# IrisRainbowNeko/HCP-Diffusion

Measured on AMD Instinct MI355X. Metric: training images/sec (whole node), SD1.5 LoRA 512px bs=4/GPU, higher is better.
Workload: dtype bf16; 1 GPU; SD1.5 UNet LoRA rank=8 bf16, bs=4/GPU, 512x512 (64x64 latents), 77-token context, random-init weights, cached latents, grad-ckpt off; global_batch=4, parallelism=dp1, rccl_ranks=1, comm=none, hip_graph=True, gradient_checkpointing=False

## Files before the change

hcp_diffusion_amd/_lib.py:

```python
import ctypes
import os
from ctypes import c_int, c_long, c_float, c_void_p, c_size_t, c_char_p
from pathlib import Path

LIB_PATH = Path(__file__).resolve().parent / "libhcp_mi355x.so"

P, I, L, F = c_void_p, c_int, c_long, c_float

_PROTOTYPES = {
    "hcp_last_error": (c_char_p, []),
    "hcp_is_emulated": (I, []),
    "hcp_abi_version": (I, []),
    "hcp_selfcheck_atomics": (I, [P, P, I, I, I, P]),
    "hcp_gemm_bf16": (I, [P, I, P, I, P, I, I, I, I, P, I, P, I, I, P, P, I, I, P, I, P, P, P, F, I, P, c_size_t, P]),
    "hcp_gemm_lora_bf16": (I, [P, I, P, I, P, P, P, I, P, I, I, I, I, P, P, I, P, P, P, P, c_size_t, P]),
    "hcp_gemm_geglu_bwd_bf16": (I, [P, I, P, I, P, P, P, I, P, P, I, I, I, P, c_size_t, P]),
    "hcp_gemm_workspace_bytes": (c_size_t, [I, I]),
    "hcp_conv3x3_bf16": (I, [P, I, P, I, I, I, I, I, I, I, I, I, I, P, I, P, I, P, P, I, P, I, I, P, P, P, c_size_t, P]),
    "hcp_attention_fwd": (I, [P, P, P, P, P, I, I, I, I, I, L, I, L, I, L, I, L, I, F, P, L, I, P]),
    "hcp_attention_bwd": (I, [P, P, P, P, P, P, P, P, P, P, I, I, I, I, I, L, I, L, I, L, I, L, I, F, P, L, I, P, c_size_t, P]),
    "hcp_groupnorm_workspace_bytes": (c_size_t, [I, I, I, I]),
    "hcp_groupnorm_silu_fwd": (I, [P, P, P, P, P, P, I, I, I, I, F, I, P]),
    "hcp_groupnorm_silu_bwd": (I, [P, P, P, P, P, P, P, P, I, I, I, I, I, P]),
    "hcp_layernorm_fwd": (I, [P, P, P, P, P, P, I, I, F, P]),
    "hcp_layernorm_bwd": (I, [P, P, P, P, P, P, P, P, P, I, I, P]),
    "hcp_geglu_fwd": (I, [P, P, L, I, P]),
    "hcp_geglu_bwd": (I, [P, P, P, L, I, P]),
    "hcp_add_bf16": (I, [P, P, P, L, P]),
    "hcp_copy2d_bf16": (I, [P, I, P, I, L, I, P]),
    "hcp_concat2_bf16": (I, [P, I, P, I, P, L, I, P]),
    "hcp_silu_fwd": (I, [P, P, L, P]),
    "hcp_silu_bwd": (I, [P, P, P, L, P]),
    "hcp_nchw_to_nhwc_bf16": (I, [P, I, P, I, I, I, I, P]),
    "hcp_nhwc_to_nchw_f32": (I, [P, P, I, I, I, I, P]),
    "hcp_upsample2x_bwd": (I, [P, P, I, I, I, I, P]),
    "hcp_timestep_embedding": (I, [P, P, I, I, F, P]),
    "hcp_timestep_embedding_f32": (I, [P, P, I, I, F, P]),
    "hcp_wgrad_linear_bf16": (I, [P, I, P, I, P, I, I, I, I, P, c_size_t, P]),
    "hcp_wgrad_conv3x3_bf16": (I, [P, I, P, I, P, I, P, I, I, I, I, I, I, I, I, I, P, c_size_t, P]),
    "hcp_colsum_bf16": (I, [P, I, P, I, I, I, I, P]),
    "hcp_ema_update": (I, [P, P, L, P, F, F, F, P]),
    "hcp_cast_f32_bf16": (I, [P, P, L, F, I, P]),
    "hcp_cast_bf16_f32": (I, [P, P, L, P]),
    "hcp_pack_piece_bytes": (I, []),
    "hcp_pack_weights": (I, [P, I, I, P]),
    "hcp_groupnorm_affine_grad": (I, [P, P, P, P, P, P, P, I, I, I, I, I, P]),
    "hcp_layernorm_affine_grad": (I, [P, P, P, P, P, I, I, P]),
    "hcp_add_noise": (I, [P, P, P, P, P, I, L, P]),
    "hcp_cfg_ddim_step": (I, [P, P, P, L, I, F, F, F, P]),
    "hcp_snr_loss_weight": (I, [P, P, P, I, I, F, P]),
    "hcp_quick_gelu": (I, [P, P, P, L, P]),
    "hcp_embedding_bf16": (I, [P, P, P, P, P, L, I, I, P]),
    "hcp_embedding_pt_fwd_bf16": (I, [P, I, I, I, I, P, I, P, P, I, P, I, P, I, P, P, I, P]),
    "hcp_embedding_pt_bwd_f32": (I, [P, P, L, I, P, I, I, P]),
    "hcp_transpose_bf16": (I, [P, P, I, I, I, P]),
    "hcp_softmax_rows": (I, [P, L, P, L, I, I, F, P]),
    "hcp_vae_latent_sample": (I, [P, P, P, P, P, I, I, L, F, P]),
    "hcp_mse_masked_mean": (I, [P, P, P, I, P, P, P, I, I, I, F, P]),
    "hcp_lora_wgrad": (I, [P, I, I, P, I, P, I, I, I, I, F, I, P, c_size_t, P]),
    "hcp_lora_wgrad_pair": (I, [P, I, P, I, I, P, P, I, P, I, I, P, I, I, F, P, c_size_t, P]),
    "hcp_split_hi_lo_bf16": (I, [P, P, c_long, I, P]),
    "hcp_lora_wgrad_group_geometry": (I, [I, I, I, I, I, P, P, P, P]),
    "hcp_lora_wgrad_group_desc_bytes": (I, []),
    "hcp_lora_wgrad_grouped": (I, [P, I, I, I, c_long, P, c_size_t, P]),
    "hcp_lora_pack": (I, [P, I, P]),
    "hcp_lora_pack_desc_bytes": (I, []),
    "hcp_sumsq_f32": (I, [P, L, P, P]),
    "hcp_adamw_clip_fused": (I, [P, P, P, P, L, P, F, F, F, F, P, F, F, P, P]),
    "hcp_comm_unique_id": (I, [P]),
    "hcp_comm_init": (I, [I, I, P, ctypes.POINTER(P)]),
    "hcp_comm_destroy": (I, [P]),
    "hcp_comm_rank": (I, [P]),
    "hcp_comm_world": (I, [P]),
    "hcp_allreduce_flat": (I, [P, P, c_size_t, I, P]),
    "hcp_reduce_scatter_flat": (I, [P, P, P, c_size_t, I, P]),
    "hcp_allgather_flat": (I, [P, P, P, c_size_t, I, P]),
}

_TOOLS_PROTOTYPES = {
    "hcp_debug_set_gemm_config": (I, [I]),
    "hcp_debug_set_gemm_glds": (I, [I]),
    "hcp_debug_set_gemm_loaders": (I, [I]),
    "hcp_debug_set_gemm_epilogue": (I, [I]),
    "hcp_debug_set_conv_patch": (I, [I]),
    "hcp_debug_set_gn_target": (I, [I]),
    "hcp_debug_set_gemm_ablation": (I, [I]),
    "hcp_debug_set_attention_config": (I, [I]),
    "hcp_debug_set_wgrad_tile": (I, [I]),
    "hcp_debug_gemm_table_stats": (I, [P, P]),
}

EXPORTED_SYMBOLS = tuple(_PROTOTYPES)
TOOLS_SYMBOLS = tuple(_TOOLS_PROTOTYPES)
TOOLS_LIB_PATH = Path(__file__).resolve().parent / "libhcp_mi355x_tools.so"


ABI_VERSION = 4


class HcpError(RuntimeError):
    pass


def bind(cdll):
    cdll.hcp_abi_version.restype = I
    cdll.hcp_abi_version.argtypes = []
    got = cdll.hcp_abi_version()
    if got != ABI_VERSION:
        raise HcpError(f"{getattr(cdll, '_name', 'library')}: hcp_abi_version() = {got}, these bindings are for ABI {ABI_VERSION} "
                       "(rebuild with `python -m hcp_diffusion_amd.build`)")
    for name, (res, args) in _PROTOTYPES.items():
        fn = getattr(cdll, name)
        fn.restype = res
        fn.argtypes = args
    for name, (res, args) in _TOOLS_PROTOTYPES.items():
        fn = getattr(cdll, name, None)
        if fn is not None:
            fn.restype = res
            fn.argtypes = args
    return cdll


_tools = None


def load_tools():
    global _tools
    if _tools is None:
        import torch
        if not TOOLS_LIB_PATH.exists():
            raise HcpError(f"{TOOLS_LIB_PATH} not found: build it with `python -m hcp_diffusion_amd.build`")
        _tools = ctypes.CDLL(str(TOOLS_LIB_PATH))
        for name in _TOOLS_PROTOTYPES:
            getattr(_tools, name)
    return _tools


_lib = None


def load():
    global _lib
    if _lib is None:
        import torch
        if not LIB_PATH.exists():
            raise HcpError(
                f"{LIB_PATH} not found: build it with `python -m hcp_diffusion_amd.build` "
                "(hipcc, gfx950). hcp_diffusion_amd has no CPU/PyTorch fallback path.")
        _lib = bind(ctypes.CDLL(str(LIB_PATH)))
    return _lib


def check(rc, what=""):
    if rc != 0:
        msg = load().hcp_last_error() if _lib is not None else b""
        raise HcpError(f"{what} failed: {msg.decode() if msg else rc}")
```

hcp_diffusion_amd/csrc/gemm.hip:

```cpp
#include "hcp_common.h"
#include "gemm_params.h"

extern "C" int hcp_geglu_fwd(const void* h, void* y, long M, int F, hipStream_t stream);

namespace {

using namespace hcp_gemm;

HCP_DEVICE void epilogue_store(const GemmParams& p, int m, int n, hcp_f32x4 v) {
    if (p.geglu_hg) { epilogue_geglu_bwd(p, m, n, v); return; }
    v = v * p.alpha;
    if (p.bias) v += *(const hcp_f32x4*)(p.bias + n);
    if (p.rowbias) v += *(const hcp_f32x4*)(p.rowbias + (size_t)(m / p.rows_per_group) * p.rowbias_ld + n);
    if (p.residual) {
        hcp_bf16x4 r = *(const hcp_bf16x4*)(p.residual + (size_t)m * p.ldr + n);
#pragma unroll
        for (int q = 0; q < 4; ++q) v[q] += hcp_bf2f((unsigned short)r[q]);
        add_residual_lo(p, m, n, v);
    }
    if (p.out_f32) *(hcp_f32x4*)((float*)p.D + (size_t)m * p.ldd + n) = v;
    else store_hi_lo(p, m, n, v);
}


// ... 469 lines not shown
            } else
#endif
            {
#pragma unroll
                for (int i = 0; i < TM; ++i) fa[i] = *(const hcp_bf16x8*)(st + a_rd + i * 16 * BK);
#pragma unroll
                for (int j = 0; j < TN; ++j) fb[j] = *(const hcp_bf16x8*)(st + b_rd + j * 16 * BK);
            }
#if defined(HCP_TOOLS)
            if (p.dbg & 16) {
#pragma unroll
                for (int i = 0; i < TM; ++i) asm volatile("" ::"v"(fa[i]));
#pragma unroll
                for (int j = 0; j < TN; ++j) asm volatile("" ::"v"(fb[j]));
                continue;
            }
#endif
#pragma unroll
            for (int i = 0; i < TM; ++i)
#pragma unroll
                for (int j = 0; j < TN; ++j) acc[i][j] = hcp_mfma16(fb[j], fa[i], acc[i][j]);
            if (LORA) {
                const hcp_bf16x8 fl = *(const hcp_bf16x8*)(st + (l_rd0 ^ (ks * 32)));
#pragma unroll
                for (int i = 0; i < TM; ++i) tacc[i] = hcp_mfma16(fl, fa[i], tacc[i]);
            }
        }
    };

    constexpr bool EARLY = NLD > 0;
    constexpr int ES = EARLY ? 32 : 40;
    hcp_bf16* const le_early = lds + NST * BUF_ELEMS;
    hcp_f32x4 bias_v[TN];
    hcp_bf16x4 res_v[TM][TN];
    auto load_epilogue_operands = [&]() {
#pragma unroll
        for (int j = 0; j < TN; ++j) {
            const int nl = n0 + wn * WTN + j * 16 + 4 * fg, n = geglu_col(p, BN, nl);
            hcp_f32x4 z = {0.f, 0.f, 0.f, 0.f};
            bias_v[j] = (p.bias && nl < p.N) ? *(const hcp_f32x4*)(p.bias + n) : z;
        }
        if (p.residual && !p.epi_tile) {
#pragma unroll
            for (int i = 0; i < TM; ++i) {
                const int m = m0 + wm * WTM + i * 16 + fr;
#pragma unroll
                for (int j = 0; j < TN; ++j) {
                    const int n = n0 + wn * WTN + j * 16 + 4 * fg;
                    hcp_bf16x4 z = {0, 0, 0, 0};
                    res_v[i][j] = (m < p.M && n < p.N) ? *(const hcp_bf16x4*)(p.residual + (size_t)m * p.ldr + n) : z;
                }
            }
        }
    };
    if (EARLY && !is_loader && p.nsplit == 1) load_epilogue_operands();

    if (NLD > 0 && is_loader) {
        if (LORA) {
            const hcp_rsrc re = hcp_make_rsrc(p.E);
            for (int g = wave; g < BN / 16; g += NLD) {
                const int nl = n0 + g * 16 + (lane >> 2), n = geglu_col(p, BN, nl);
                hcp_buf_glds16(re, nl < p.N ? (unsigned)(((size_t)n * 32 + (lane & 3) * 8) * 2) : HCP_BUF_OOB, le_early + g * 16 * 32);
            }
        }
        static_assert(NLD == 0 || (BM % RPP == 0 && BN % RPP == 0), "loader waves: whole row groups");
        constexpr int IPT = A_IT + B_IT + (LORA ? 1 : 0);
        int issued = 0, wbuf = 0;
        auto issue_next = [&]() {
            if (issued < nprim) issue(wbuf); else issue_ext(wbuf);
            ++issued; wbuf = wbuf + 1 == NST ? 0 : wbuf + 1;
        };
        auto wait_newer = [&](int newer) {
            if (NST > 3 && newer >= 2) hcp_wait_vmcnt_c<2 * IPT>();
            else if (NST > 2 && newer >= 1) hcp_wait_vmcnt_c<IPT>();
            else hcp_wait_vmcnt_c<0>();
        };
        for (int i = 0; i < NST - 1 && issued < nk; ++i) issue_next();
        wait_newer(issued - 1);
        hcp_barrier_keep_dma();
        for (int t = 0; t < nk; ++t) {
#if defined(HCP_TOOLS)
            if (p.dbg & 8) issued = nk;
#endif
            if (issued < nk) issue_next();
            wait_newer(issued - (t + 2));
            hcp_barrier_keep_dma();
        }
        if (LORA) HCP_SYNC();
        if ((p.geglu_hg || p.geglu_out || p.epi_tile) && p.nsplit == 1) { if (LORA) HCP_SYNC(); HCP_SYNC(); }
        return;
    }
    if (NLD == 0) { if (nprim > 0) issue(0); else if (has_ext) issue_ext(0); }
    HCP_SYNC();
    for (int t = 0, cur = 0; t < nk; ++t) {
        if (NLD == 0) {
            if (t + 1 < nprim) issue(cur ^ 1);
            else if (t + 1 == nprim && has_ext) issue_ext(cur ^ 1);
        }
        compute(cur);
        HCP_SYNC();
        cur = cur + 1 == NST ? 0 : cur + 1;
    }

    if (LORA) {
        constexpr int TS2 = 40;
        hcp_bf16* lt = lds;
        hcp_bf16* le = EARLY ? le_early : lds + BM * TS2;
        hcp_bf16* lt2 = lds + BM * TS2 + (EARLY ? 0 : BN * TS2);
        const bool split = p.ldt == 64;
        const int ldt = split ? 64 : 32;
#pragma unroll
        for (int i = 0; i < TM; ++i) {
            hcp_bf16x4 o, o2;
            lora_t_split(tacc[i], o, o2);
            const int ml = wm * WTM + i * 16 + fr;
            *(hcp_bf16x4*)(lt + ml * TS2 + wn * 16 + 4 * fg) = o;
            if (split) *(hcp_bf16x4*)(lt2 + ml * TS2 + wn * 16 + 4 * fg) = o2;
            if (tile_n == 0 && p.Tout && m0 + ml < p.M) {
                *(hcp_bf16x4*)(p.Tout + (size_t)(m0 + ml) * ldt + wn * 16 + 4 * fg) = o;
                if (split) *(hcp_bf16x4*)(p.Tout + (size_t)(m0 + ml) * ldt + 32 + wn * 16 + 4 * fg) = o2;
            }
        }
        if (!EARLY) {
            for (int c = tid_all; c < BN * 4; c += NTC) {
                const int r = c >> 2, q = c & 3;
                hcp_bf16x8 v = hcp_zero8();
                if (n0 + r < p.N) v = *(const hcp_bf16x8*)(p.E + (size_t)geglu_col(p, BN, n0 + r) * 32 + q * 8);
                *(hcp_bf16x8*)(le + r * TS2 + q * 8) = v;
            }
        }
        HCP_SYNC();
        hcp_bf16x8 ft[TM], fe[TN];
#pragma unroll
        for (int i = 0; i < TM; ++i) ft[i] = *(const hcp_bf16x8*)(lt + (wm * WTM + i * 16 + fr) * TS2 + fg * 8);
#pragma unroll
        for (int j = 0; j < TN; ++j) fe[j] = *(const hcp_bf16x8*)(le + (wn * WTN + j * 16 + fr) * ES + fg * 8);
#pragma unroll
        for (int i = 0; i < TM; ++i)
#pragma unroll
            for (int j = 0; j < TN; ++j) acc[i][j] = hcp_mfma16(fe[j], ft[i], acc[i][j]);
        if (split) {
#pragma unroll
            for (int i = 0; i < TM; ++i) ft[i] = *(const hcp_bf16x8*)(lt2 + (wm * WTM + i * 16 + fr) * TS2 + fg * 8);
#pragma unroll
            for (int i = 0; i < TM; ++i)
#pragma unroll
                for (int j = 0; j < TN; ++j) acc[i][j] = hcp_mfma16(fe[j], ft[i], acc[i][j]);
        }
    }

    if (p.nsplit > 1) {
#pragma unroll
        for (int i = 0; i < TM; ++i) {
            const int m = m0 + wm * WTM + i * 16 + fr;
            if (m >= p.M) continue;
#pragma unroll
            for (int j = 0; j < TN; ++j) {
                const int n = n0 + wn * WTN + j * 16 + 4 * fg;
                if (n < p.N) *(hcp_f32x4*)(p.slabs + ((size_t)split * p.M + m) * p.N + n) = acc[i][j];
            }
        }
        return;
    }
    if (p.geglu_hg) {
        static_assert((size_t)BM * geglu_tile_ld(BN) <= (size_t)2 * BUF_ELEMS, "the product tile fits the ring");
        if (LORA) HCP_SYNC();
#pragma unroll
        for (int i = 0; i < TM; ++i)
#pragma unroll
            for (int j = 0; j < TN; ++j) geglu_tile_put(lds, geglu_tile_ld(BN), wm * WTM + i * 16 + fr, wn * WTN + j * 16 + 4 * fg, acc[i][j], p.alpha);
        HCP_SYNC();
        geglu_tile_apply<BM, BN, NTC>(p, lds, m0, n0, tid_all);
        return;
    }
    if (p.geglu_out) {
        static_assert((size_t)BM * BN * 2 <= (size_t)2 * BUF_ELEMS * sizeof(hcp_bf16), "the gelu(g) tile fits the ring");
        if (!EARLY) load_epilogue_operands();
        if (LORA) HCP_SYNC();
        hcp_f32x4 v[TM][TN];
        int rows[TM], cols[TN];
        constexpr int HW = WGN / 2;
        const bool is_g = wn >= HW;
#pragma unroll
        for (int j = 0; j < TN; ++j) cols[j] = tile_n * (BN / 2) + (wn - (is_g ? HW : 0)) * WTN + j * 16 + 4 * fg;
#pragma unroll
        for (int i = 0; i < TM; ++i) {
            const int m = m0 + wm * WTM + i * 16 + fr;
            rows[i] = m;
#pragma unroll
            for (int j = 0; j < TN; ++j) {
                v[i][j] = acc[i][j] * p.alpha + bias_v[j];
                if (m < p.M) store_hi_lo(p, m, cols[j] + (is_g ? (p.N >> 1) : 0), v[i][j]);
            }
        }
        geglu_fwd_pair<TM, TN>(v, is_g, wm * HW + (wn - (is_g ? HW : 0)), lane, (hcp_f32x4*)lds, [] { HCP_SYNC(); }, p.geglu_out, p.N >> 1, rows, p.M, cols);
        return;
    }
    if (p.epi_tile) {
        if (!EARLY) load_epilogue_operands();
        if (LORA) HCP_SYNC();
        float* const tile = (float*)lds;
#pragma unroll
        for (int i = 0; i < TM; ++i) {
            const int ml = wm * WTM + i * 16 + fr, m = m0 + ml;
            const float* rbp = (p.rowbias && m < p.M) ? p.rowbias + (size_t)(m / p.rows_per_group) * p.rowbias_ld : nullptr;
#pragma unroll
            for (int j = 0; j < TN; ++j) {
                const int nl = wn * WTN + j * 16 + 4 * fg;
                hcp_f32x4 v = acc[i][j] * p.alpha + bias_v[j];
                if (rbp && n0 + nl < p.N) v += *(const hcp_f32x4*)(rbp + n0 + nl);
                *(hcp_f32x4*)(tile + ml * epi_tile_ld(BN) + nl) = v;
            }
        }
        HCP_SYNC();
        epi_tile_store<BM, BN, NTC>(p, tile, m0, n0, tid_all);
        return;
    }
    if (!EARLY) load_epilogue_operands();
#pragma unroll
    for (int i = 0; i < TM; ++i) {
        const int m = m0 + wm * WTM + i * 16 + fr;
        if (m >= p.M) continue;
        hcp_f32x4 rb_v[TN];
        if (p.rowbias) {
            const float* rbp = p.rowbias + (size_t)(m / p.rows_per_group) * p.rowbias_ld;
#pragma unroll
            for (int j = 0; j < TN; ++j) {
                const int n = n0 + wn * WTN + j * 16 + 4 * fg;
                hcp_f32x4 z = {0.f, 0.f, 0.f, 0.f};
                rb_v[j] = n < p.N ? *(const hcp_f32x4*)(rbp + n) : z;
            }
        }
#pragma unroll
        for (int j = 0; j < TN; ++j) {
            const int n = n0 + wn * WTN + j * 16 + 4 * fg;
            if (n >= p.N) continue;
            hcp_f32x4 v = acc[i][j] * p.alpha + bias_v[j];
            if (p.rowbias) v += rb_v[j];
            if (p.residual) {
#pragma unroll
                for (int q = 0; q < 4; ++q) v[q] += hcp_bf2f((unsigned short)res_v[i][j][q]);
                add_residual_lo(p, m, n, v);
            }
#if defined(HCP_TOOLS)
            if ((p.dbg & 64) && v[0] != 12345.678f) continue;
#endif
            if (p.out_f32) *(hcp_f32x4*)((float*)p.D + (size_t)m * p.ldd + n) = v;
            else store_hi_lo(p, m, n, v);
        }
    }
}

HCP_KERNEL(256) splitk_reduce_kernel(GemmParams p) {
    const unsigned nv = (unsigned)p.N / 4;
    const unsigned total = (unsigned)p.M * nv;
    const size_t slab = (size_t)p.M * p.N;
    const int ns = p.nsplit;
    const bool plain = !p.geglu_hg;
    for (unsigned i = blockIdx.x * 256u + threadIdx.x; i < total; i += gridDim.x * 256u) {
        const int m = (int)(i / nv), n = (int)(i - (unsigned)m * nv) * 4;
        const float* src = p.slabs + (size_t)i * 4;
        hcp_f32x4 v = *(const hcp_f32x4*)src;
        const void* const zp = g_zero_page;
        const hcp_f32x4 bias = *(const hcp_f32x4*)(plain && p.bias ? (const void*)(p.bias + n) : zp);
        const hcp_f32x4 rowb = *(const hcp_f32x4*)(plain && p.rowbias ? (const void*)(p.rowbias + (size_t)(m / p.rows_per_group) * p.rowbias_ld + n) : zp);
        const hcp_bf16x4 res = *(const hcp_bf16x4*)(plain && p.residual ? (const void*)(p.residual + (size_t)m * p.ldr + n) : zp);
        const hcp_bf16x4 res_lo = *(const hcp_bf16x4*)(plain && p.residual && p.residual_lo ? (const void*)(p.residual_lo + (size_t)m * p.ldr + n) : zp);
        int s = 1;
        for (; s + 4 <= ns; s += 4) {
            const hcp_f32x4 a = *(const hcp_f32x4*)(src + (size_t)s * slab), b = *(const hcp_f32x4*)(src + (size_t)(s + 1) * slab);
            const hcp_f32x4 c = *(const hcp_f32x4*)(src + (size_t)(s + 2) * slab), d = *(const hcp_f32x4*)(src + (size_t)(s + 3) * slab);
            v += a; v += b; v += c; v += d;
        }
        if (s + 2 <= ns) {
            const hcp_f32x4 a = *(const hcp_f32x4*)(src + (size_t)s * slab), b = *(const hcp_f32x4*)(src + (size_t)(s + 1) * slab);
            v += a; v += b;
            s += 2;
        }
        if (s < ns) v += *(const hcp_f32x4*)(src + (size_t)s * slab);
        if (!plain) { epilogue_geglu_bwd(p, m, n, v); continue; }
        v = v * p.alpha;
        if (p.bias) v += bias;
        if (p.rowbias) v += rowb;
        if (p.residual) {
#pragma unroll
            for (int q = 0; q < 4; ++q) v[q] += hcp_bf2f((unsigned short)res[q]);
            if (p.residual_lo) {
#pragma unroll
                for (int q = 0; q < 4; ++q) v[q] += hcp_bf2f((unsigned short)res_lo[q]);
            }
        }
        if (p.out_f32) *(hcp_f32x4*)((float*)p.D + (size_t)m * p.ldd + n) = v;
        else store_hi_lo(p, m, n, v);
    }
}

HCP_TUNABLE(int, g_force_cfg, -1);
inline int forced_id(int v) { return v >= 1024 ? (v - 1024) % 64 : v % 16; }
inline int forced_split(int v) { const int s = v >= 1024 ? (v - 1024) / 64 : v / 16; return s > 0 ? s : 1; }
HCP_TUNABLE(int, g_dbg_ablate, 0);
HCP_TUNABLE(int, g_use_v2, 1);

HCP_TUNABLE(int, g_conv_patch, 1);
HCP_TUNABLE(int, g_epi_tile, -1);
HCP_TUNABLE(int, g_force_loaders, -1);

bool want_epi_tile(const GemmParams& p, int mode) {
    if (p.nsplit != 1 || p.out_f32 || p.geglu_hg || p.geglu_out || p.N % 8 || p.ldd % 8 || (p.residual && p.ldr % 8)) return false;
    if ((((size_t)p.D) | ((size_t)p.D_lo) | ((size_t)p.residual) | ((size_t)p.residual_lo)) & 15) return false;
    if (g_epi_tile >= 0) return g_epi_tile == 1;
    return mode == 0 && p.residual != nullptr;
}

int launch_splitk_reduce(const GemmParams& p, hipStream_t stream, const char* name = "splitk_reduce_kernel") {
    if (p.nsplit > 1) {
        const long nv = (long)p.M * (p.N / 4);
        int g = (int)((nv + 255) / 256); if (g > 2048) g = 2048;
        HCP_LAUNCH(splitk_reduce_kernel, dim3(g), dim3(256), 0, stream, p);
    }
    HCP_LAUNCH_CHECK(name);
}
bool buffer_loops_take(const GemmParams& p) {
    return g_use_v2 && !(g_dbg_ablate & 7) && p.K % BK == 0 && (p.K2 == 0 || p.K2 == 32) &&
           (size_t)p.M * p.lda * 2 < (1ul << 31) && (size_t)p.N * p.ldb * 2 < (1ul << 31);
}
void pair_geglu_or_clear(GemmParams& p, int mode, int bn, int wgn) {
    if (p.geglu_out && mode == 0 && wgn % 2 == 0 && p.nsplit == 1 && (p.N / 2) % (bn / 2) == 0) p.geglu_fused = 1;
    else p.geglu_out = nullptr;
}
template <int BM, int BN, int WGM, int WGN, int MODE, bool FAST, bool LORA = false, int NSTAGE = 2, int NLD = 0>
int launch_cfg(GemmParams& p, hipStream_t stream) {
    p.tiles_m = hcp_cdiv(p.M, BM);
    const int tiles_n = hcp_cdiv(p.N, BN);
    p.dbg = g_dbg_ablate;
    constexpr size_t tail = (size_t)(2 * BM + BN) * 40 * sizeof(hcp_bf16);
    if constexpr (NSTAGE == 2 && (MODE == 0 || FAST)) {
        if (buffer_loops_take(p)) {
            constexpr size_t stage = (size_t)(BM + BN + (LORA ? 32 : 0)) * BK * sizeof(hcp_bf16);
            constexpr size_t eimg = (LORA && NLD > 0) ? (size_t)BN * 32 * sizeof(hcp_bf16) : 0;
            pair_geglu_or_clear(p, MODE, BN, WGN);
            constexpr size_t tile_bytes = (size_t)BM * epi_tile_ld(BN) * sizeof(float);
            p.epi_tile = want_epi_tile(p, MODE) && tile_bytes <= 160 * 1024 - eimg ? 1 : 0;
            size_t smem = 2 * stage;
            if (LORA && smem < tail) smem = tail;
            if (p.epi_tile && smem < tile_bytes) smem = tile_bytes;
            [[maybe_unused]] const dim3 grid(p.tiles_m * tiles_n, p.nsplit);
            if constexpr (NLD > 0) {
                const size_t tb = p.epi_tile ? tile_bytes : 0;
                if (p.loaders == 4 && 4 * stage + eimg <= 160 * 1024) {
                    HCP_LAUNCH((gemm_v2_kernel<BM, BN, WGM, WGN, MODE, LORA, NLD, (4 * stage + eimg <= 160 * 1024 ? 4 : 2)>), grid, dim3(64 * (WGM * WGN + NLD)), (4 * stage > tb ? 4 * stage : tb) + eimg, stream, p);
                } else if (p.loaders >= 3 && 3 * stage + eimg <= 160 * 1024) {
                    HCP_LAUNCH((gemm_v2_kernel<BM, BN, WGM, WGN, MODE, LORA, NLD, (3 * stage + eimg <= 160 * 1024 ? 3 : 2)>), grid, dim3(64 * (WGM * WGN + NLD)), (3 * stage > tb ? 3 * stage : tb) + eimg, stream, p);
                } else if (p.loaders) {
                    HCP_LAUNCH((gemm_v2_kernel<BM, BN, WGM, WGN, MODE, LORA, NLD>), grid, dim3(64 * (WGM * WGN + NLD)), smem + eimg, stream, p);
                } else {
                    HCP_LAUNCH((gemm_v2_kernel<BM, BN, WGM, WGN, MODE, LORA>), grid, dim3(64 * WGM * WGN), smem, stream, p);
                }
            } else {
                HCP_LAUNCH((gemm_v2_kernel<BM, BN, WGM, WGN, MODE, LORA>), dim3(p.tiles_m * tiles_n, p.nsplit), dim3(64 * WGM * WGN), smem, stream, p);
            }
            return launch_splitk_reduce(p, stream, "gemm_v2_kernel");
        }
    }
    {
        p.epi_tile = 0;
        p.geglu_out = nullptr;
        size_t smem = (size_t)NSTAGE * (BM + BN + (LORA ? 32 : 0)) * BK * sizeof(hcp_bf16);
        if (LORA && smem < tail) smem = tail;
        HCP_LAUNCH((gemm_glds_kernel<BM, BN, WGM, WGN, MODE, FAST, LORA, NSTAGE>), dim3(p.tiles_m * tiles_n, p.nsplit),
                   dim3(64 * WGM * WGN), smem, stream, p);
    }
    return launch_splitk_reduce(p, stream, "gemm_kernel");
}

struct TileCfg { int bm, bn; };
constexpr TileCfg kCfgs[] = {{128, 128}, {128, 64}, {64, 64}, {128, 160}, {64, 160}, {256, 128}, {256, 160}, {128, 320},
                             {128, 160}, {128, 160}, {256, 160},
                             {128, 320}, {256, 160}, {128, 160}, {64, 160}, {128, 128},
                             {32, 160}};
constexpr int kNumCfgs = sizeof(kCfgs) / sizeof(kCfgs[0]);

int try_pp(int id, int mode, bool fast_or_plain, bool lora, GemmParams& p, hipStream_t stream) {
    if (p.loaders < 8 || !fast_or_plain || !buffer_loops_take(p)) return -2;
    const int bm = kCfgs[id].bm, bn = kCfgs[id].bn;
    p.tiles_m = hcp_cdiv(p.M, bm);
    p.dbg = g_dbg_ablate;
    p.epi_tile = want_epi_tile(p, mode) ? 1 : 0;
    hcp_bf16* const gout = p.geglu_out;
    pair_geglu_or_clear(p, mode, bn, 2);
    int r = -2;
    if (mode != 0 && !lora && (g_conv_patch == 2 || (g_conv_patch == 1 && (mode == 2 || p.nsplit > 1))))
        r = conv_patch_launch(p, bm, bn, mode, p.loaders - 8, stream);
    if (r == -2) r = gemm_pp_launch(p, bm, bn, mode, lora, p.loaders - 8, stream);
    if (r == -2) { p.geglu_out = gout; p.geglu_fused = 0; }
    if (r != 0 || p.nsplit <= 1) return r;
    return launch_splitk_reduce(p, stream);
}

template <int MODE, bool FAST>
int launch_by_id(int id, GemmParams& p, hipStream_t stream) {
    if (id >= 0 && id < kNumCfgs) { const int r = try_pp(id, MODE, MODE == 0 || FAST, false, p, stream); if (r != -2) return r; }
    switch (id) {
        case 0: return launch_cfg<128, 128, 2, 2, MODE, FAST>(p, stream);
        case 1: return launch_cfg<128, 64, 2, 2, MODE, FAST>(p, stream);
        case 2: return launch_cfg<64, 64, 2, 2, MODE, FAST>(p, stream);
        case 3: return launch_cfg<128, 160, 2, 2, MODE, FAST>(p, stream);
        case 4: return launch_cfg<64, 160, 2, 2, MODE, FAST>(p, stream);
        case 5: return launch_cfg<256, 128, 4, 2, MODE, FAST>(p, stream);
        case 6: return launch_cfg<256, 160, 4, 2, MODE, FAST>(p, stream);
        case 8: return launch_cfg<128, 160, 4, 2, MODE, FAST, false, 3>(p, stream);
        case 9: return launch_cfg<128, 160, 2, 2, MODE, FAST, false, 3>(p, stream);
        case 10: return launch_cfg<256, 160, 4, 2, MODE, FAST, false, 3>(p, stream);
        case 11: return launch_cfg<128, 320, 4, 4, MODE, FAST>(p, stream);
        case 12: return launch_cfg<256, 160, 8, 2, MODE, FAST>(p, stream);
        case 13: return launch_cfg<128, 160, 4, 2, MODE, FAST, false, 2, 4>(p, stream);
        case 14: return launch_cfg<64, 160, 4, 2, MODE, FAST, false, 2, 4>(p, stream);
        case 15: return launch_cfg<128, 128, 4, 2, MODE, FAST, false, 2, 4>(p, stream);
        case 16: return launch_cfg<64, 160, 4, 2, MODE, FAST, false, 2, 4>(p, stream);
        default: return launch_cfg<128, 320, 2, 4, MODE, FAST>(p, stream);
    }
}

int launch_lora_by_id(int id, GemmParams& p, hipStream_t stream) {
    if (id >= 0 && id < kNumCfgs) { const int r = try_pp(id, 0, true, true, p, stream); if (r != -2) return r; }
    switch (id) {
        case 0: return launch_cfg<128, 128, 2, 2, 0, false, true>(p, stream);
        case 1: return launch_cfg<128, 64, 2, 2, 0, false, true>(p, stream);
        case 2: return launch_cfg<64, 64, 2, 2, 0, false, true>(p, stream);
        case 3: return launch_cfg<128, 160, 2, 2, 0, false, true>(p, stream);
        case 5: return launch_cfg<256, 128, 4, 2, 0, false, true>(p, stream);
        case 6: return launch_cfg<256, 160, 4, 2, 0, false, true>(p, stream);
        case 8: return launch_cfg<128, 160, 4, 2, 0, false, true, 3>(p, stream);
        case 9: return launch_cfg<128, 160, 2, 2, 0, false, true, 3>(p, stream);
        case 12: return launch_cfg<256, 160, 8, 2, 0, false, true>(p, stream);
        case 13: return launch_cfg<128, 160, 4, 2, 0, false, true, 2, 4>(p, stream);
        case 14: return launch_cfg<64, 160, 4, 2, 0, false, true, 2, 4>(p, stream);
        case 15: return launch_cfg<128, 128, 4, 2, 0, false, true, 2, 4>(p, stream);
        case 16: return launch_cfg<64, 160, 4, 2, 0, false, true, 2, 4>(p, stream);
        default: return launch_cfg<64, 160, 2, 2, 0, false, true>(p, stream);
    }
}

int choose_cfg(const GemmParams& p, int* nsplit_out) {
    const int nk1 = hcp_cdiv(p.K, BK);
    int id;
    if (p.N <= 64) id = 2;
    else if (p.N % 160 == 0) id = ((long)p.M * p.N >= (long)4096 * 2560) ? 6 : 4;
    else id = ((long)p.M * p.N >= (long)4096 * 2048) ? 0 : 2;
    const long tiles = (long)hcp_cdiv(p.M, kCfgs[id].bm) * hcp_cdiv(p.N, kCfgs[id].bn);
    int s = 1;
    while (s < 16 && tiles * s < 1024 && nk1 / (s * 2) >= 4) s *= 2;
    *nsplit_out = s;
    return id;
}

struct TunedEntry { int mode, M, N, K, has_k2, stride, up, cfg, split, loaders; };
const TunedEntry kTuned[] = {
#include "gemm_tuned_loaders.inc"
#include "gemm_tuned.inc"
};

#if defined(HCP_TOOLS)
long g_table_hits = 0, g_table_misses = 0;
#endif

bool lookup_tuned(const GemmParams& p, int mode, int* cfg, int* split, int* loaders = nullptr) {
    bool hit = false;
    for (const TunedEntry& e : kTuned) {
        if (g_force_loaders == 0 && e.loaders) continue;
        if (e.mode == mode && e.M == p.M && e.N == p.N && e.K == p.K && e.has_k2 == (p.K2 > 0) &&
            (mode == 0 || mode == 3 || (e.stride == p.cv.stride && e.up == p.cv.up))) {
            *cfg = e.cfg; *split = e.split; if (loaders) *loaders = e.loaders; hit = true; break;
        }
    }
#if defined(HCP_TOOLS)
    (hit ? g_table_hits : g_table_misses) += 1;
#endif
    return hit;
}

inline int deepest_ring(int ld) { return ld == 3 ? 4 : ld; }

template <int MODE, bool FAST>
int dispatch_gemm(GemmParams& p, float* ws, size_t ws_bytes, hipStream_t stream) {
    int nsplit = 1;
    int id = 0, ld = 0;
    if (!lookup_tuned(p, MODE, &id, &nsplit, &ld)) id = choose_cfg(p, &nsplit);
    if (g_force_cfg >= 0) { id = forced_id(g_force_cfg); nsplit = forced_split(g_force_cfg); }
    p.loaders = g_force_loaders >= 0 ? g_force_loaders : deepest_ring(ld);
    if (nsplit > 1 && (size_t)nsplit * p.M * p.N * sizeof(float) > ws_bytes) nsplit = 1;
    if (p.geglu_out) nsplit = 1;
    const int nk1 = hcp_cdiv(p.K, BK);
    p.nsplit = nsplit;
    p.kt_per_split = hcp_cdiv(nk1, nsplit);
    p.nsplit = hcp_cdiv(nk1, p.kt_per_split);
    p.slabs = ws;
    return launch_by_id<MODE, FAST>(id, p, stream);
}

int check_common(const GemmParams& p) {
    HCP_REQUIRE(p.M > 0 && p.N > 0 && p.K > 0, "gemm: empty problem M=%d N=%d K=%d", p.M, p.N, p.K);
    HCP_REQUIRE(p.K % 8 == 0 && p.K2 % 8 == 0, "gemm: K (%d) and K2 (%d) must be multiples of 8", p.K, p.K2);
    HCP_REQUIRE(p.N % 4 == 0 && p.ldd % 4 == 0, "gemm: N (%d) and ldd (%d) must be multiples of 4", p.N, p.ldd);
    HCP_REQUIRE(p.ldb % 8 == 0, "gemm: ldb (%d) must be a multiple of 8", p.ldb);
    HCP_REQUIRE(p.K2 == 0 || (p.A2 && p.B2 && p.lda2 % 8 == 0 && p.ldb2 % 8 == 0), "gemm: bad K-extension operands");
    HCP_REQUIRE(!p.residual || p.ldr % 4 == 0, "gemm: ldr must be a multiple of 4");
    HCP_REQUIRE(!p.rowbias || p.rows_per_group > 0, "gemm: rows_per_group must be > 0");
    return 0;
}

int check_gact(GemmParams& p, void* gact, const char* who) {
    if (!gact) return 0;
    HCP_REQUIRE(!p.out_f32 && !p.residual && !p.rowbias && !p.D_lo && p.alpha == 1.0f && p.N % 16 == 0 && p.ldd == p.N,
                "%s: the GEGLU output needs a contiguous bf16 (h | g) [M, N] (N %% 16 == 0) with no residual / row bias / alpha", who);
    p.geglu_out = (hcp_bf16*)gact; p.geglu_fused = 0;
    return 0;
}
int finish_gact(const GemmParams& p, void* gact, hipStream_t stream) {
    if (!gact || p.geglu_fused) return 0;
    return hcp_geglu_fwd(p.D, gact, p.M, p.N / 2, stream);
}

int launch_lora_dispatched(GemmParams& p, void* workspace, size_t workspace_bytes, hipStream_t stream) {
    int id = 4, nsplit = 1, ld = 0;
    GemmParams q = p; q.K2 = 32;
    if (!lookup_tuned(q, 3, &id, &nsplit, &ld)) {
        if (p.K >= 4096 && p.M <= 4096) id = -1;
        else if ((long)p.M * p.N >= (long)4096 * 2560 && p.N % 160 == 0) id = 6;
        else if (p.N % 160 == 0 && (long)p.M * p.N >= (long)4096 * 640) id = 4;
        else id = 2;
    }
    if (g_force_cfg >= 0) id = forced_id(g_force_cfg);
    p.loaders = g_force_loaders >= 0 ? g_force_loaders : deepest_ring(ld);
    if (id == 7 || id == 10 || id == 11) id = 6;
    if (id < 0) {
        HCP_REQUIRE(p.Tout, "hcp_gemm_lora_bf16: this shape runs as two launches and needs the T buffer");
        const int ldt = p.ldt == 64 ? 64 : 32;
        if (ldt == 64 && hcp_memset_async(p.Tout, 0, (size_t)p.M * 64 * sizeof(hcp_bf16), stream)) return hcp_set_error("hcp_gemm_lora_bf16: memset failed");
        GemmParams t = {};
        t.A = p.A; t.lda = p.lda; t.B = p.L; t.ldb = p.K; t.M = p.M; t.N = 32; t.K = p.K; t.D = p.Tout; t.ldd = ldt; t.alpha = 1.0f;
        if (int e2 = dispatch_gemm<0, false>(t, (float*)workspace, workspace ? workspace_bytes : 0, stream)) return e2;
        p.A2 = (const hcp_bf16*)p.Tout; p.lda2 = ldt; p.B2 = p.E; p.ldb2 = 32; p.K2 = 32;
        p.L = nullptr; p.E = nullptr; p.Tout = nullptr; p.ldt = 0;
        return dispatch_gemm<0, false>(p, (float*)workspace, workspace ? workspace_bytes : 0, stream);
    }
    p.nsplit = 1; p.kt_per_split = hcp_cdiv(p.K, BK); p.slabs = nullptr;
    return launch_lora_by_id(id, p, stream);
}

}

#if defined(HCP_TOOLS)
HCP_API int hcp_debug_gemm_table_stats(long* hits, long* misses) {
    if (hits) *hits = g_table_hits;
    if (misses) *misses = g_table_misses;
    g_table_hits = 0; g_table_misses = 0;
    return 0;
}
HCP_API int hcp_debug_set_gemm_config(int cfg) { g_force_cfg = cfg; return 0; }
HCP_API int hcp_debug_set_gemm_glds(int on) { g_use_v2 = on == 1; return 0; }
HCP_API int hcp_debug_set_gemm_ablation(int flags) { g_dbg_ablate = flags; return 0; }
HCP_API int hcp_debug_set_gemm_loaders(int mode) { g_force_loaders = mode; return 0; }
HCP_API int hcp_debug_set_gemm_epilogue(int mode) { g_epi_tile = mode; return 0; }
HCP_API int hcp_debug_set_conv_patch(int on) { g_conv_patch = on; return 0; }
#endif

HCP_API size_t hcp_gemm_workspace_bytes(int M, int N) { return (size_t)16 * M * N * sizeof(float); }

HCP_API int hcp_gemm_bf16(const void* A, int lda, const void* B, int ldb, void* D, int ldd, int M, int N, int K,
                          const void* A2, int lda2, const void* B2, int ldb2, int K2, const float* bias,
                          const float* rowbias, int rowbias_ld, int rows_per_group, const void* residual, int ldr,
                          const void* residual_lo, void* D_lo, void* gact, float alpha, int out_f32, void* workspace,
                          size_t workspace_bytes, hipStream_t stream) {
    GemmParams p = {};
    p.A = (const hcp_bf16*)A; p.lda = lda; p.B = (const hcp_bf16*)B; p.ldb = ldb;
    p.A2 = (const hcp_bf16*)A2; p.lda2 = lda2; p.B2 = (const hcp_bf16*)B2; p.ldb2 = ldb2; p.K2 = K2;
    p.M = M; p.N = N; p.K = K; p.D = D; p.ldd = ldd; p.out_f32 = out_f32;
    p.bias = bias; p.rowbias = rowbias; p.rowbias_ld = rowbias_ld; p.rows_per_group = rows_per_group;
    p.residual = (const hcp_bf16*)residual; p.ldr = ldr; p.alpha = alpha;
    p.residual_lo = (const hcp_bf16*)residual_lo; p.D_lo = (hcp_bf16*)D_lo;
    HCP_REQUIRE(A && B && D, "hcp_gemm_bf16: null operand");
    HCP_REQUIRE((!residual_lo || residual) && (!D_lo || !out_f32), "hcp_gemm_bf16: residual_lo needs residual; D_lo needs a bf16 output");
    HCP_REQUIRE(lda % 8 == 0, "hcp_gemm_bf16: lda (%d) must be a multiple of 8", lda);
    if (int e = check_common(p)) return e;
    if (int e = check_gact(p, gact, "hcp_gemm_bf16")) return e;
    if (int e = dispatch_gemm<0, false>(p, (float*)workspace, workspace ? workspace_bytes : 0, stream)) return e;
    return finish_gact(p, gact, stream);
}

HCP_API int hcp_conv3x3_bf16(const void* X1, int C1, const void* X2, int C2, int Bn, int Hs, int Ws, int Ho, int Wo,
                             int mode, int stride, int upsample, int pad, const void* Wp, int Cout, void* D, int ldd,
                             const float* bias, const float* rowbias, int rowbias_ld, const void* residual, int ldr,
                             int out_f32, const void* A2, const void* B2, void* workspace, size_t workspace_bytes,
                             hipStream_t stream) {
    GemmParams p = {};
    HCP_REQUIRE(X1 && Wp && D, "hcp_conv3x3_bf16: null operand");
    HCP_REQUIRE((A2 == nullptr) == (B2 == nullptr), "hcp_conv3x3_bf16: the rank-32 K-extension needs both A2 and B2");
    if (A2) { p.A2 = (const hcp_bf16*)A2; p.lda2 = 32; p.B2 = (const hcp_bf16*)B2; p.ldb2 = 32; p.K2 = 32; }
    HCP_REQUIRE(C1 % 8 == 0 && C2 % 8 == 0 && (C2 == 0 || X2), "hcp_conv3x3_bf16: channels must be multiples of 8");
    HCP_REQUIRE(stride == 1 || stride == 2, "hcp_conv3x3_bf16: stride must be 1 or 2");
    HCP_REQUIRE(mode == 0 || (mode == 1 && upsample == 0 && C2 == 0), "hcp_conv3x3_bf16: bad mode/options");
    HCP_REQUIRE(pad == 1 || (pad == 0 && mode == 0 && !upsample), "hcp_conv3x3_bf16: pad must be 1 (or 0 for a forward conv without upsampling)");
    HCP_REQUIRE(Ho <= 1024 && Wo <= 1024 && Bn < 2048, "hcp_conv3x3_bf16: dims too large for packed pixel ids (10 bits per output axis)");
    HCP_REQUIRE((long)Bn * Hs * Ws * (C1 > C2 ? C1 : C2) < (1L << 31), "hcp_conv3x3_bf16: source tensor too large for 32-bit offsets");
    p.cv.X1 = (const hcp_bf16*)X1; p.cv.C1 = C1; p.cv.X2 = (const hcp_bf16*)X2; p.cv.C2 = C2;
    p.cv.Hs = Hs; p.cv.Ws = Ws; p.cv.Ho = Ho; p.cv.Wo = Wo; p.cv.stride = stride; p.cv.up = upsample ? 1 : 0; p.cv.pad = pad;
    p.M = Bn * Ho * Wo; p.N = Cout; p.K = 9 * (C1 + C2);
    p.B = (const hcp_bf16*)Wp; p.ldb = p.K;
    p.D = D; p.ldd = ldd; p.out_f32 = out_f32; p.bias = bias;
    p.rowbias = rowbias; p.rowbias_ld = rowbias_ld; p.rows_per_group = Ho * Wo;
    p.residual = (const hcp_bf16*)residual; p.ldr = ldr; p.alpha = 1.0f;
    if (int e = check_common(p)) return e;
    float* ws = (float*)workspace; size_t wb = workspace ? workspace_bytes : 0;
    const bool fast = (C1 % 64 == 0) && (C2 % 64 == 0) && !upsample && !(mode == 1 && stride == 2);
    if (mode == 0) return fast ? dispatch_gemm<1, true>(p, ws, wb, stream) : dispatch_gemm<1, false>(p, ws, wb, stream);
    return fast ? dispatch_gemm<2, true>(p, ws, wb, stream) : dispatch_gemm<2, false>(p, ws, wb, stream);
}

HCP_API int hcp_gemm_geglu_bwd_bf16(const void* A, int lda, const void* B, int ldb, const void* L, const void* E, void* Tout, int ldt,
                                    const void* HG, void* DHG, int M, int F, int K, void* workspace, size_t workspace_bytes,
                                    hipStream_t stream) {
    GemmParams p = {};
    p.A = (const hcp_bf16*)A; p.lda = lda; p.B = (const hcp_bf16*)B; p.ldb = ldb;
    p.M = M; p.N = F; p.K = K; p.D = DHG; p.ldd = 2 * F; p.out_f32 = 0; p.alpha = 1.0f;
    p.geglu_hg = (const hcp_bf16*)HG; p.geglu_ld = 2 * F;
    HCP_REQUIRE(A && B && HG && DHG, "hcp_gemm_geglu_bwd_bf16: null operand");
    HCP_REQUIRE((L == nullptr) == (E == nullptr), "hcp_gemm_geglu_bwd_bf16: L and E come together");
    HCP_REQUIRE(lda % 8 == 0 && F % 8 == 0, "hcp_gemm_geglu_bwd_bf16: lda (%d) and F (%d) must be multiples of 8", lda, F);
    if (int e = check_common(p)) return e;
    if (!L) return dispatch_gemm<0, false>(p, (float*)workspace, workspace ? workspace_bytes : 0, stream);
    HCP_REQUIRE(ldt == 32 || ldt == 64, "hcp_gemm_geglu_bwd_bf16: ldt (%d) is 32 (bf16 U) or 64 (split U: hi | lo)", ldt);
    p.L = (const hcp_bf16*)L; p.E = (const hcp_bf16*)E; p.Tout = (hcp_bf16*)Tout; p.ldt = ldt;
    return launch_lora_dispatched(p, workspace, workspace_bytes, stream);
}

HCP_API int hcp_gemm_lora_bf16(const void* A, int lda, const void* B, int ldb, const void* L, const void* E, void* Tout, int ldt, void* D,
                               int ldd, int M, int N, int K, const float* bias, const void* residual, int ldr, const void* residual_lo,
                               void* D_lo, void* gact, void* workspace, size_t workspace_bytes, hipStream_t stream) {
    GemmParams p = {};
    p.A = (const hcp_bf16*)A; p.lda = lda; p.B = (const hcp_bf16*)B; p.ldb = ldb;
    p.M = M; p.N = N; p.K = K; p.D = D; p.ldd = ldd; p.out_f32 = 0;
    p.bias = bias; p.residual = (const hcp_bf16*)residual; p.ldr = ldr; p.alpha = 1.0f;
    p.L = (const hcp_bf16*)L; p.E = (const hcp_bf16*)E; p.Tout = (hcp_bf16*)Tout; p.ldt = ldt;
    p.residual_lo = (const hcp_bf16*)residual_lo; p.D_lo = (hcp_bf16*)D_lo;
    HCP_REQUIRE(A && B && D && L && E, "hcp_gemm_lora_bf16: null operand");
    HCP_REQUIRE(!residual_lo || residual, "hcp_gemm_lora_bf16: residual_lo needs residual");
    HCP_REQUIRE(ldt == 32 || ldt == 64, "hcp_gemm_lora_bf16: ldt (%d) is 32 (bf16 T) or 64 (split T: hi | lo)", ldt);
    HCP_REQUIRE(lda % 8 == 0, "hcp_gemm_lora_bf16: lda (%d) must be a multiple of 8", lda);
    if (int e = check_common(p)) return e;
    if (int e = check_gact(p, gact, "hcp_gemm_lora_bf16")) return e;
    if (int e = launch_lora_dispatched(p, workspace, workspace_bytes, stream)) return e;
    return finish_gact(p, gact, stream);
}
```

hcp_diffusion_amd/csrc/gemm_params.h:

```cpp
#pragma once
#include "hcp_common.h"

namespace hcp_gemm {

struct ConvDesc {
    const hcp_bf16* X1; int C1;
    const hcp_bf16* X2; int C2;
    int Hs, Ws;
    int Ho, Wo;
    int stride;
    int up;
    int pad;
};

struct GemmParams {
    const hcp_bf16* A; int lda;
    const hcp_bf16* A2; int lda2; int K2;
    const hcp_bf16* B; int ldb;
    const hcp_bf16* B2; int ldb2;
    int M, N, K;
    void* D; int ldd; int out_f32;
    const float* bias;
    const float* rowbias; int rowbias_ld; int rows_per_group;
    const hcp_bf16* residual; int ldr;
    const hcp_bf16* residual_lo; hcp_bf16* D_lo;
    float alpha;
    int tiles_m;
    int nsplit; int kt_per_split;
    float* slabs;
    const hcp_bf16* L; const hcp_bf16* E; hcp_bf16* Tout; int ldt;
    const hcp_bf16* geglu_hg; int geglu_ld;
    hcp_bf16* geglu_out; int geglu_fused;
    int epi_tile;
    int loaders;
    int dbg;
    ConvDesc cv;
};

constexpr int BK = 64;

HCP_DEVICE void lora_t_split(const hcp_f32x4& t, hcp_bf16x4& hi, hcp_bf16x4& lo) {
#pragma unroll
    for (int q = 0; q < 4; ++q) {
        const unsigned short h = hcp_f2bf(t[q]);
        hi[q] = (short)h;
        lo[q] = (short)hcp_f2bf(t[q] - hcp_bf2f(h));
    }
}

HCP_DEVICE void store_hi_lo(const GemmParams& p, int m, int n, const hcp_f32x4& v) {
    hcp_bf16x4 o;
#pragma unroll
    for (int q = 0; q < 4; ++q) o[q] = (short)hcp_f2bf(v[q]);
    *(hcp_bf16x4*)((hcp_bf16*)p.D + (size_t)m * p.ldd + n) = o;
    if (p.D_lo) {
        hcp_bf16x4 l;
#pragma unroll
        for (int q = 0; q < 4; ++q) l[q] = (short)hcp_f2bf(v[q] - hcp_bf2f((unsigned short)o[q]));
        *(hcp_bf16x4*)(p.D_lo + (size_t)m * p.ldd + n) = l;
    }
}
HCP_DEVICE void add_residual_lo(const GemmParams& p, int m, int n, hcp_f32x4& v) {
    if (!p.residual_lo) return;
    const hcp_bf16x4 r = *(const hcp_bf16x4*)(p.residual_lo + (size_t)m * p.ldr + n);
#pragma unroll
    for (int q = 0; q < 4; ++q) v[q] += hcp_bf2f((unsigned short)r[q]);
}

constexpr int epi_tile_ld(int BN) { return BN + 4; }
template <int BM, int BN, int NTHREADS>
HCP_DEVICE void epi_tile_store(const GemmParams& p, const float* tile, int m0, int n0, int tid) {
    constexpr int LD = epi_tile_ld(BN), PIECES = BN / 8;
    for (int idx = tid; idx < BM * PIECES; idx += NTHREADS) {
        const int row = idx / PIECES, c8 = (idx - row * PIECES) * 8;
        const int m = m0 + row, n = n0 + c8;
        if (m >= p.M || n >= p.N) continue;
        const hcp_f32x4 a = *(const hcp_f32x4*)(tile + row * LD + c8), b = *(const hcp_f32x4*)(tile + row * LD + c8 + 4);
        float v[8] = {a[0], a[1], a[2], a[3], b[0], b[1], b[2], b[3]};
        if (p.residual) {
            const hcp_bf16x8 r = *(const hcp_bf16x8*)(p.residual + (size_t)m * p.ldr + n);
#pragma unroll
            for (int q = 0; q < 8; ++q) v[q] += hcp_bf2f((unsigned short)r[q]);
            if (p.residual_lo) {
                const hcp_bf16x8 rl = *(const hcp_bf16x8*)(p.residual_lo + (size_t)m * p.ldr + n);
#pragma unroll
                for (int q = 0; q < 8; ++q) v[q] += hcp_bf2f((unsigned short)rl[q]);
            }
        }
        hcp_bf16x8 o;
#pragma unroll
        for (int q = 0; q < 8; ++q) o[q] = (short)hcp_f2bf(v[q]);
        *(hcp_bf16x8*)((hcp_bf16*)p.D + (size_t)m * p.ldd + n) = o;
        if (p.D_lo) {
            hcp_bf16x8 l;
#pragma unroll
            for (int q = 0; q < 8; ++q) l[q] = (short)hcp_f2bf(v[q] - hcp_bf2f((unsigned short)o[q]));
            *(hcp_bf16x8*)(p.D_lo + (size_t)m * p.ldd + n) = l;
        }
    }
}

HCP_DEVICE int geglu_col(const GemmParams& p, int BN, int nl) {
    if (!p.geglu_out) return nl;
    const int half = BN >> 1, j = nl / BN, c = nl - j * BN;
    return c < half ? j * half + c : (p.N >> 1) + j * half + (c - half);
}
template <int TI, int TJ, typename SYNC>
HCP_DEVICE void geglu_fwd_pair(hcp_f32x4 (&v)[TI][TJ], bool is_g, int slot, int lane, hcp_f32x4* xg, SYNC&& sync,
                               hcp_bf16* out, int F, const int (&rows)[TI], int M, const int (&cols)[TJ]) {
    hcp_f32x4* mine = xg + (size_t)slot * TI * TJ * 64 + lane;
    if (is_g) {
#pragma unroll
        for (int i = 0; i < TI; ++i)
#pragma unroll
            for (int j = 0; j < TJ; ++j) {
                hcp_f32x4 ge;
#pragma unroll
                for (int q = 0; q < 4; ++q) ge[q] = hcp_gelu_erf(v[i][j][q]);
                mine[(i * TJ + j) * 64] = ge;
            }
    }
    sync();
    if (!is_g) {
#pragma unroll
        for (int i = 0; i < TI; ++i) {
            if (rows[i] >= M) continue;
#pragma unroll
            for (int j = 0; j < TJ; ++j) {
                const hcp_f32x4 ge = mine[(i * TJ + j) * 64];
                hcp_bf16x4 o;
#pragma unroll
                for (int q = 0; q < 4; ++q) o[q] = (short)hcp_f2bf(v[i][j][q] * ge[q]);
                *(hcp_bf16x4*)(out + (size_t)rows[i] * F + cols[j]) = o;
            }
        }
    }
}

HCP_DEVICE void epilogue_geglu_bwd(const GemmParams& p, int m, int n, hcp_f32x4 v) {
    const hcp_bf16* hp = p.geglu_hg + (size_t)m * p.geglu_ld + n;
    const hcp_bf16x4 h = *(const hcp_bf16x4*)hp, g = *(const hcp_bf16x4*)(hp + p.N);
    hcp_bf16x4 dh, dg;
#pragma unroll
    for (int q = 0; q < 4; ++q) {
        const float hf = hcp_bf2f((unsigned short)h[q]), gf = hcp_bf2f((unsigned short)g[q]);
        const float d = hcp_bf2f(hcp_f2bf(v[q] * p.alpha));
        dh[q] = (short)hcp_f2bf(d * hcp_gelu_erf(gf));
        dg[q] = (short)hcp_f2bf(d * hf * hcp_gelu_erf_grad(gf));
    }
    hcp_bf16* dp = (hcp_bf16*)p.D + (size_t)m * p.ldd + n;
    *(hcp_bf16x4*)dp = dh;
    *(hcp_bf16x4*)(dp + p.N) = dg;
}

constexpr int geglu_tile_ld(int BN) { return BN + 8; }
HCP_DEVICE void geglu_tile_put(hcp_bf16* tile, int ld, int row, int col, hcp_f32x4 v, float alpha) {
    hcp_bf16x4 o;
#pragma unroll
    for (int q = 0; q < 4; ++q) o[q] = (short)hcp_f2bf(v[q] * alpha);
    *(hcp_bf16x4*)(tile + row * ld + col) = o;
}
template <int BM, int BN, int NTHREADS>
HCP_DEVICE void geglu_tile_apply(const GemmParams& p, const hcp_bf16* tile, int m0, int n0, int tid) {
    constexpr int LD = geglu_tile_ld(BN), PIECES = BN / 8;
    for (int idx = tid; idx < BM * PIECES; idx += NTHREADS) {
        const int row = idx / PIECES, c8 = (idx - row * PIECES) * 8;
        const int m = m0 + row, n = n0 + c8;
        if (m >= p.M || n >= p.N) continue;
        const hcp_bf16x8 d = *(const hcp_bf16x8*)(tile + row * LD + c8);
        const hcp_bf16* hp = p.geglu_hg + (size_t)m * p.geglu_ld + n;
        const hcp_bf16x8 h = *(const hcp_bf16x8*)hp, g = *(const hcp_bf16x8*)(hp + p.N);
        hcp_bf16x8 dh, dg;
#pragma unroll
        for (int q = 0; q < 8; ++q) {
            const float df = hcp_bf2f((unsigned short)d[q]), hf = hcp_bf2f((unsigned short)h[q]), gf = hcp_bf2f((unsigned short)g[q]);
            dh[q] = (short)hcp_f2bf(df * hcp_gelu_erf(gf));
            dg[q] = (short)hcp_f2bf(df * hf * hcp_gelu_erf_grad(gf));
        }
        hcp_bf16* dp = (hcp_bf16*)p.D + (size_t)m * p.ldd + n;
        *(hcp_bf16x8*)dp = dh;
        *(hcp_bf16x8*)(dp + p.N) = dg;
    }
}

int gemm_pp_launch(GemmParams& p, int bm, int bn, int mode, bool lora, int ring, hipStream_t stream);
int conv_patch_launch(GemmParams& p, int bm, int bn, int mode, int ring, hipStream_t stream);

}
```

hcp_diffusion_amd/csrc/gemm_pp.hip:

```cpp
#include "gemm_params.h"
#include <type_traits>

namespace hcp_gemm {
namespace {

template <int BM, int BN, int MODE, bool LORA, int NST>
HCP_KERNEL(768) gemm_pp_kernel(GemmParams p) {
    constexpr int NC = 8, NLD = 4;
    constexpr int NTC = 64 * NC, NTL = 64 * NLD;
    constexpr int WTM = BM / 2, WTN = BN / 2;
    constexpr int TM = WTM / 16, TN = WTN / 16;
    constexpr int UPT = 1;
    constexpr bool FIN_N = TM == 1;
    constexpr int TMF = FIN_N ? 1 : TM / 2;
    constexpr int TNF0 = FIN_N ? (TN + 1) / 2 : TN, TNF1 = FIN_N ? TN / 2 : TN;
    constexpr int TNF = TNF0;
    constexpr int RPP = NTL / 8;
    constexpr int A_IT = BM / RPP, B_IT = BN / RPP;
    static_assert(WTM % 16 == 0 && WTN % 16 == 0 && BM % RPP == 0 && BN % RPP == 0 && (TM % 2 == 0 || FIN_N), "tile shape");
    static_assert(NST >= 2 && NST <= 4, "ring depth");
    constexpr int A_ELEMS = BM * BK, B_ELEMS = BN * BK, L_ELEMS = LORA ? 32 * BK : 0, BUF_ELEMS = A_ELEMS + B_ELEMS + L_ELEMS;
    constexpr int E_ELEMS = LORA ? BN * 32 : 0;
    HCP_DYN_SMEM(smem);
    hcp_bf16* const lds_e = (hcp_bf16*)smem;
    hcp_bf16* const ring = lds_e + E_ELEMS;

    const int tid_all = threadIdx.x;
    const int lane = tid_all & 63;
    const int wave_all = hcp_uniform(tid_all >> 6);
    const int tile_m = blockIdx.x % p.tiles_m, tile_n = blockIdx.x / p.tiles_m;
    const int m0 = tile_m * BM, n0 = tile_n * BN;
    const int split = blockIdx.y;

    const int nk1 = p.K / BK;
    const int kt_begin = split * p.kt_per_split;
    int kt_end = kt_begin + p.kt_per_split; if (kt_end > nk1) kt_end = nk1;
    const int nprim = kt_end - kt_begin;
    const bool has_ext = (split == p.nsplit - 1) && p.K2 > 0;
    const int nk = nprim + (has_ext ? 1 : 0);

    if (wave_all >= NC) {
        const int wave = wave_all - NC, tid = tid_all - NTC;
        const int kc = tid & 7, lrow = tid >> 3;
#if defined(HCP_TOOLS)
        if (p.dbg & 0x2000) hcp_setprio<3>();
#endif
        const int Ctot = p.cv.C1 + p.cv.C2;
        unsigned va[A_IT], vb[B_IT];
        unsigned a_msk[(A_IT + 2) / 3];
#pragma unroll
        for (int i = 0; i < (A_IT + 2) / 3; ++i) a_msk[i] = 0;
        const unsigned a_chunk = (unsigned)(((kc ^ ((lrow >> 1) & 7)) << 3) * 2);
#pragma unroll
        for (int i = 0; i < B_IT; ++i) {
            const int r = lrow + RPP * i, nl = n0 + r, n = geglu_col(p, BN, nl);
            vb[i] = nl < p.N ? (unsigned)(((size_t)n * p.ldb + ((kc ^ ((r >> 1) & 7)) << 3)) * 2) : HCP_BUF_OOB;
        }
#pragma unroll
        for (int i = 0; i < A_IT; ++i) {
            const int r = lrow + RPP * i, m = m0 + r;
            va[i] = HCP_BUF_OOB;
            if (m < p.M) {
                if (MODE == 0) {
                    va[i] = (unsigned)(((size_t)m * p.lda + ((kc ^ ((r >> 1) & 7)) << 3)) * 2);
                } else {
                    const int hw = p.cv.Ho * p.cv.Wo;
                    const int b = m / hw; const int rem = m - b * hw;
                    const int py = rem / p.cv.Wo, px = rem - py * p.cv.Wo;
                    const int s = MODE == 1 ? p.cv.stride : 1;
                    va[i] = (unsigned)((b * p.cv.Hs + py * s) * p.cv.Ws + px * s);
                    unsigned msk = 0;
#pragma unroll
                    for (int ky = 0; ky < 3; ++ky)
#pragma unroll
                        for (int kx = 0; kx < 3; ++kx) {
                            const int sy = MODE == 1 ? py * s + ky - p.cv.pad : py + 1 - ky;
                            const int sx = MODE == 1 ? px * s + kx - p.cv.pad : px + 1 - kx;
                            if (sy >= 0 && sy < p.cv.Hs && sx >= 0 && sx < p.cv.Ws) msk |= 1u << (ky * 3 + kx);
                        }
                    a_msk[i / 3] |= msk << (9 * (i % 3));
                }
            }
        }
        int tap = 0, cb = 0;
        if (MODE != 0) { const int k0 = kt_begin * BK; tap = k0 / Ctot; cb = k0 - tap * Ctot; }
        unsigned vo1[MODE != 0 ? A_IT : 1], vo2[MODE != 0 ? A_IT : 1], a_nmsk[(A_IT + 2) / 3];
        if (MODE != 0) {
#pragma unroll
            for (int i = 0; i < A_IT; ++i) {
                const bool live = va[i] != HCP_BUF_OOB;
                vo1[i] = live ? va[i] * (unsigned)(2 * p.cv.C1) + a_chunk : HCP_BUF_OOB;
                vo2[i] = live ? va[i] * (unsigned)(2 * p.cv.C2) + a_chunk : HCP_BUF_OOB;
            }
#pragma unroll
            for (int i = 0; i < (A_IT + 2) / 3; ++i) a_nmsk[i] = ~a_msk[i];
        }
        const hcp_bf16* Ab = p.A + (size_t)kt_begin * BK;
        const hcp_bf16* Bb = p.B + (size_t)kt_begin * BK;
        const hcp_bf16* Lb = LORA ? p.L + (size_t)kt_begin * BK : nullptr;
        const unsigned vl = (unsigned)(((size_t)lrow * p.K + ((kc ^ ((lrow >> 1) & 7)) << 3)) * 2);

        constexpr int IPT = A_IT + B_IT + (LORA ? 1 : 0);
        static_assert(IPT * (NST - 1) < 64, "vmcnt immediate");
        auto issue_part = [&](auto Q0, auto Q1, int buf, bool ext) {
            constexpr int q0 = decltype(Q0)::value, q1 = decltype(Q1)::value;
            hcp_bf16* la = ring + buf * BUF_ELEMS;
            hcp_bf16* lb = la + A_ELEMS;
            if (!ext) {
                const hcp_rsrc rb = hcp_make_rsrc(Bb);
#pragma unroll
                for (int i = 0; i < B_IT; ++i)
                    if (i >= q0 && i < q1) hcp_buf_glds16(rb, vb[i], lb + (wave * 8 + RPP * i) * BK);
                if (LORA && B_IT >= q0 && B_IT < q1) {
                    const hcp_rsrc rl = hcp_make_rsrc(Lb);
                    hcp_buf_glds16(rl, vl, lb + B_ELEMS + (wave * 8) * BK);
                }
                constexpr int qa = B_IT + (LORA ? 1 : 0);
                if (qa + A_IT > q0 && qa < q1) {
                    if (MODE == 0) {
                        const hcp_rsrc ra = hcp_make_rsrc(Ab);
#pragma unroll
                        for (int i = 0; i < A_IT; ++i)
                            if (qa + i >= q0 && qa + i < q1) hcp_buf_glds16(ra, va[i], la + (wave * 8 + RPP * i) * BK);
                    } else {
                        const int ky = tap / 3, kx = tap - ky * 3;
                        const int doff = MODE == 1 ? (ky - p.cv.pad) * p.cv.Ws + (kx - p.cv.pad) : (1 - ky) * p.cv.Ws + (1 - kx);
                        const bool first = cb < p.cv.C1;
                        const hcp_bf16* base = first ? p.cv.X1 + (long)doff * p.cv.C1 + cb : p.cv.X2 + (long)doff * p.cv.C2 + (cb - p.cv.C1);
                        const hcp_rsrc ra = hcp_make_rsrc(base);
                        if (first) {
#pragma unroll
                            for (int i = 0; i < A_IT; ++i)
                                if (qa + i >= q0 && qa + i < q1)
                                    hcp_buf_glds16(ra, vo1[i] | (((a_nmsk[i / 3] >> (9 * (i % 3) + tap)) & 1u) << 31), la + (wave * 8 + RPP * i) * BK);
                        } else {
#pragma unroll
                            for (int i = 0; i < A_IT; ++i)
                                if (qa + i >= q0 && qa + i < q1)
                                    hcp_buf_glds16(ra, vo2[i] | (((a_nmsk[i / 3] >> (9 * (i % 3) + tap)) & 1u) << 31), la + (wave * 8 + RPP * i) * BK);
                        }
                    }
                }
            } else {
                const hcp_rsrc rb = hcp_make_rsrc(p.B2), ra = hcp_make_rsrc(p.A2);
#pragma unroll
                for (int i = 0; i < B_IT; ++i)
                    if (i >= q0 && i < q1) {
                        const int r = lrow + RPP * i, nl = n0 + r, n = geglu_col(p, BN, nl), k = (kc ^ ((r >> 1) & 7)) << 3;
                        hcp_buf_glds16(rb, (nl < p.N && k < p.K2) ? (unsigned)(((size_t)n * p.ldb2 + k) * 2) : HCP_BUF_OOB, lb + (wave * 8 + RPP * i) * BK);
                    }
                if (LORA && B_IT >= q0 && B_IT < q1) hcp_buf_glds16(rb, HCP_BUF_OOB, lb + B_ELEMS + (wave * 8) * BK);
                constexpr int qa = B_IT + (LORA ? 1 : 0);
#pragma unroll
                for (int i = 0; i < A_IT; ++i)
                    if (qa + i >= q0 && qa + i < q1) {
                        const int r = lrow + RPP * i, m = m0 + r, k = (kc ^ ((r >> 1) & 7)) << 3;
                        hcp_buf_glds16(ra, (m < p.M && k < p.K2) ? (unsigned)(((size_t)m * p.lda2 + k) * 2) : HCP_BUF_OOB, la + (wave * 8 + RPP * i) * BK);
                    }
            }
        };
        int issued = 0, wbuf = 0;
        auto tile_done = [&]() {
            if (issued < nprim) {
                Bb += BK;
                if (LORA) Lb += BK;
                if (MODE == 0) Ab += BK;
                else { cb += BK; if (cb >= Ctot) { cb -= Ctot; ++tap; } }
            }
            ++issued; wbuf = wbuf + 1 == NST ? 0 : wbuf + 1;
        };
        using I0 = std::integral_constant<int, 0>;
        using IALL = std::integral_constant<int, IPT>;
        if (LORA) {
            const hcp_rsrc re = hcp_make_rsrc(p.E);
            for (int gq = wave; gq < BN / 16; gq += NLD) {
                const int nl = n0 + gq * 16 + (lane >> 2), n = geglu_col(p, BN, nl);
                hcp_buf_glds16(re, nl < p.N ? (unsigned)(((size_t)n * 32 + (lane & 3) * 8) * 2) : HCP_BUF_OOB, lds_e + gq * 16 * 32);
            }
        }
        auto wait_tiles = [&](int rem) {
            if (NST >= 4 && rem >= 3) hcp_wait_vmcnt_c<(NST >= 4 ? 3 : 0) * IPT>();
            else if (NST >= 4 && rem == 2) hcp_wait_vmcnt_c<(NST >= 4 ? 2 : 0) * IPT>();
            else if (NST >= 3 && rem >= 1) hcp_wait_vmcnt_c<(NST >= 3 ? 1 : 0) * IPT>();
            else hcp_wait_vmcnt_c<0>();
        };
        auto quiet_iter = [&](int t) {
            hcp_barrier_only();
#pragma unroll
            for (int e = 0; e < 2 * UPT - 2; ++e) hcp_barrier_only();
            wait_tiles(issued - (t + 2));
            hcp_barrier_only();
        };
        for (int i = 0; i < NST && issued < nk; ++i) { issue_part(I0{}, IALL{}, wbuf, issued >= nprim); tile_done(); }
        wait_tiles(issued - 1);
        hcp_barrier_only();
        quiet_iter(0);
        int t = 1;
        constexpr int NPART = NST >= 3 ? 2 * UPT : 1;
        constexpr int LASTQ = IPT * (NPART - 1) / NPART;
        for (; t + NST - 1 < nk; ++t) {
            const bool ext = issued >= nprim;
            hcp_barrier_only();
#if defined(HCP_TOOLS)
            if (p.dbg & 0x300) {
                const hcp_rsrc rz = hcp_make_rsrc(p.B);
                hcp_bf16* la = ring + wbuf * BUF_ELEMS;
                if (!(p.dbg & 0x100)) for (int i = 0; i < A_IT; ++i) hcp_buf_glds16(rz, MODE == 0 ? (va[i] & 0xfffff) : (unsigned)(lane * 16 + i * 1024 + wave * 8192), la + (wave * 8 + RPP * i) * BK);
                if (!(p.dbg & 0x200)) for (int i = 0; i < B_IT; ++i) hcp_buf_glds16(rz, vb[i], la + A_ELEMS + (wave * 8 + RPP * i) * BK);
                ++issued; wbuf = wbuf + 1 == NST ? 0 : wbuf + 1;
                for (int e = 0; e < 2 * UPT - 2; ++e) hcp_barrier_only();
                hcp_wait_vmcnt_c<0>();
                hcp_barrier_only();
                continue;
            }
#endif
            if constexpr (NPART == 1) {
                issue_part(I0{}, IALL{}, wbuf, ext); tile_done();
#pragma unroll
                for (int e = 0; e < 2 * UPT - 2; ++e) hcp_barrier_only();
                hcp_wait_vmcnt_c<0>();
                hcp_barrier_only();
            } else {
                if constexpr (NPART == 2) {
                    issue_part(I0{}, std::integral_constant<int, LASTQ>{}, wbuf, ext);
                } else {
                    issue_part(I0{}, std::integral_constant<int, IPT / 4>{}, wbuf, ext);
                    hcp_barrier_only();
                    issue_part(std::integral_constant<int, IPT / 4>{}, std::integral_constant<int, IPT / 2>{}, wbuf, ext);
                    hcp_barrier_only();
                    issue_part(std::integral_constant<int, IPT / 2>{}, std::integral_constant<int, LASTQ>{}, wbuf, ext);
                }
                hcp_wait_vmcnt_c<(NST - 3) * IPT + LASTQ>();
                hcp_barrier_only();
                issue_part(std::integral_constant<int, LASTQ>{}, IALL{}, wbuf, ext); tile_done();
            }
        }
        for (; t < nk; ++t) quiet_iter(t);
        hcp_barrier_only();
        hcp_barrier_only(); hcp_barrier_only();
        if (LORA) HCP_SYNC();
        if ((p.geglu_hg || p.geglu_out || p.epi_tile) && p.nsplit == 1) { if (LORA) HCP_SYNC(); HCP_SYNC(); }
        return;
    }

    const int g = wave_all >> 2, gm = (wave_all >> 1) & 1, gn = wave_all & 1;
    const int fr = lane & 15, fg = lane >> 4;
    const int row0 = gm * WTM;
    const int frow0 = FIN_N ? row0 : gm * WTM + g * (WTM / 2);
    const int col0 = gn * WTN;
    const int fcol0 = col0 + (FIN_N ? g * TNF0 * 16 : 0);
    const int nfin = FIN_N && g == 1 ? TNF1 : TNF0;
    const int sw0 = ((fg ^ ((fr >> 1) & 7)) << 3) ^ (g * 32);
    const int a_rd0 = (row0 + fr) * BK + sw0;
    const int b_rd0 = A_ELEMS + (col0 + fr) * BK + sw0;
    const int l_rd0 = A_ELEMS + B_ELEMS + (gn * 16 + fr) * BK + sw0;

    hcp_f32x4 acc[TM][TN];
    hcp_f32x4 tacc[LORA ? TM : 1];
#pragma unroll
    for (int i = 0; i < TM; ++i)
#pragma unroll
        for (int j = 0; j < TN; ++j) { hcp_f32x4 z = {0.f, 0.f, 0.f, 0.f}; acc[i][j] = z; }
#pragma unroll
    for (int i = 0; i < (LORA ? TM : 1); ++i) { hcp_f32x4 z = {0.f, 0.f, 0.f, 0.f}; tacc[i] = z; }

    constexpr bool EARLY = !(LORA && TM * TN >= 20);
    hcp_f32x4 bias_v[TNF];
    hcp_bf16x4 res_v[TMF][TNF];
    auto load_bias = [&]() {
        const hcp_rsrc rbias = hcp_make_rsrc_n(p.bias, p.bias ? (unsigned)p.N * 4u : 0u);
#pragma unroll
        for (int j = 0; j < TNF; ++j) bias_v[j] = hcp_buf_load16f(rbias, (unsigned)geglu_col(p, BN, n0 + fcol0 + j * 16 + 4 * fg) * 4u);
    };
    auto load_residual = [&]() {
        const hcp_rsrc rres = hcp_make_rsrc_n(p.residual, p.residual ? (unsigned)(((size_t)(p.M - 1) * p.ldr + p.N) * 2) : 0u);
#pragma unroll
        for (int i = 0; i < TMF; ++i) {
            const int m = m0 + frow0 + i * 16 + fr;
#pragma unroll
            for (int j = 0; j < TNF; ++j)
                res_v[i][j] = hcp_buf_load8(rres, ((unsigned)m * (unsigned)p.ldr + (unsigned)(n0 + fcol0 + j * 16 + 4 * fg)) * 2u);
        }
    };

    if (EARLY && p.nsplit == 1 && !p.epi_tile) load_residual();
    hcp_barrier_only();
    if (g == 1) hcp_barrier_only();
    for (int t = 0, st = 0; t < nk; ++t) {
        const hcp_bf16* sp = ring + st * BUF_ELEMS;
#pragma unroll
        for (int u = 0; u < UPT; ++u) {
#if defined(HCP_TOOLS)
            if (p.dbg & 0x800) { hcp_barrier_only(); hcp_barrier_only(); continue; }
#endif
            hcp_bf16x8 fa[TM], fb[TN], fl;
#pragma unroll
            for (int i = 0; i < TM; ++i) fa[i] = *(const hcp_bf16x8*)(sp + a_rd0 + i * 16 * BK);
#pragma unroll
            for (int j = 0; j < TN; ++j) fb[j] = *(const hcp_bf16x8*)(sp + b_rd0 + j * 16 * BK);
            if (LORA) fl = *(const hcp_bf16x8*)(sp + l_rd0);
            hcp_barrier_only();
#if defined(HCP_TOOLS)
            if (p.dbg & 0x400) {
#pragma unroll
                for (int i = 0; i < TM; ++i) asm volatile("" ::"v"(fa[i]));
#pragma unroll
                for (int j = 0; j < TN; ++j) asm volatile("" ::"v"(fb[j]));
                hcp_barrier_only();
                continue;
            }
#endif
#if defined(HCP_TOOLS)
            if (!(p.dbg & 0x1000))
#endif
            hcp_setprio<1>();
#pragma unroll
            for (int i = 0; i < TM; ++i)
#pragma unroll
                for (int j = 0; j < TN; ++j) acc[i][j] = hcp_mfma16(fb[j], fa[i], acc[i][j]);
            if (LORA) {
#pragma unroll
                for (int i = 0; i < TM; ++i) tacc[i] = hcp_mfma16(fl, fa[i], tacc[i]);
            }
            hcp_setprio<0>();
            hcp_barrier_only();
        }
        st = st + 1 == NST ? 0 : st + 1;
    }
    if (g == 0) hcp_barrier_only();

    hcp_f32x4* const xb = (hcp_f32x4*)ring;
    hcp_f32x4* const xt = xb + NC * TMF * (FIN_N ? TNF0 : TN) * 64;
    const int pw = wave_all ^ 4;
    if constexpr (FIN_N) {
        if (g == 1) {
            hcp_f32x4 tmp[TN];
#pragma unroll
            for (int j = 0; j < TN; ++j) tmp[j] = acc[0][j];
#pragma unroll
            for (int j = 0; j < TN; ++j) acc[0][j] = tmp[(j + TNF0) % TN];
        }
        if (g == 0) {
#pragma unroll
            for (int k = 0; k < TNF1; ++k) xb[(wave_all * TNF0 + k) * 64 + lane] = acc[0][TNF0 + k];
        } else {
#pragma unroll
            for (int k = 0; k < TNF0; ++k) xb[(wave_all * TNF0 + k) * 64 + lane] = acc[0][TNF1 + k];
            if (LORA) xt[wave_all * 64 + lane] = tacc[0];
        }
        if (p.nsplit == 1) load_bias();
        hcp_barrier_keep_dma();
        if (g == 0) {
#pragma unroll
            for (int k = 0; k < TNF0; ++k) acc[0][k] += xb[(pw * TNF0 + k) * 64 + lane];
            if (LORA) tacc[0] += xt[pw * 64 + lane];
        } else {
#pragma unroll
            for (int k = 0; k < TNF1; ++k) acc[0][k] += xb[(pw * TNF0 + k) * 64 + lane];
        }
    } else {
        if (g == 1) {
#pragma unroll
            for (int i = 0; i < TMF; ++i) {
#pragma unroll
                for (int j = 0; j < TN; ++j) { const hcp_f32x4 tmp = acc[i][j]; acc[i][j] = acc[TMF + i][j]; acc[TMF + i][j] = tmp; }
                if (LORA) { const hcp_f32x4 tmp = tacc[i]; tacc[i] = tacc[TMF + i]; tacc[TMF + i] = tmp; }
            }
        }
#pragma unroll
        for (int i = 0; i < TMF; ++i) {
#pragma unroll
            for (int j = 0; j < TN; ++j) xb[((wave_all * TMF + i) * TN + j) * 64 + lane] = acc[TMF + i][j];
            if (LORA) xt[(wave_all * TMF + i) * 64 + lane] = tacc[TMF + i];
        }
        if (p.nsplit == 1) load_bias();
        hcp_barrier_keep_dma();
#pragma unroll
        for (int i = 0; i < TMF; ++i) {
#pragma unroll
            for (int j = 0; j < TN; ++j) acc[i][j] += xb[((pw * TMF + i) * TN + j) * 64 + lane];
            if (LORA) tacc[i] += xt[(pw * TMF + i) * 64 + lane];
        }
    }
    hcp_barrier_keep_dma();

    if (LORA) {
        constexpr int TS2 = 40;
        hcp_bf16* lt = ring;
        hcp_bf16* lt2 = ring + BM * TS2;
        const bool split = p.ldt == 64;
        const int ldt = split ? 64 : 32;
#pragma unroll
        for (int i = 0; i < TMF; ++i) {
            if (FIN_N && g == 1) break;
            hcp_bf16x4 o, o2;
            lora_t_split(tacc[i], o, o2);
            const int ml = frow0 + i * 16 + fr;
            *(hcp_bf16x4*)(lt + ml * TS2 + gn * 16 + 4 * fg) = o;
            if (split) *(hcp_bf16x4*)(lt2 + ml * TS2 + gn * 16 + 4 * fg) = o2;
            if (tile_n == 0 && p.Tout && m0 + ml < p.M) {
                *(hcp_bf16x4*)(p.Tout + (size_t)(m0 + ml) * ldt + gn * 16 + 4 * fg) = o;
                if (split) *(hcp_bf16x4*)(p.Tout + (size_t)(m0 + ml) * ldt + 32 + gn * 16 + 4 * fg) = o2;
            }
        }
        if (!EARLY && p.nsplit == 1 && !p.epi_tile) load_residual();
        HCP_SYNC();
        hcp_bf16x8 ft[TMF], fe[TNF];
#pragma unroll
        for (int i = 0; i < TMF; ++i) ft[i] = *(const hcp_bf16x8*)(lt + (frow0 + i * 16 + fr) * TS2 + fg * 8);
#pragma unroll
        for (int j = 0; j < TNF; ++j) fe[j] = *(const hcp_bf16x8*)(lds_e + (fcol0 + j * 16 + fr) * 32 + fg * 8);
#pragma unroll
        for (int i = 0; i < TMF; ++i)
#pragma unroll
            for (int j = 0; j < TNF; ++j) acc[i][j] = hcp_mfma16(fe[j], ft[i], acc[i][j]);
        if (split) {
#pragma unroll
            for (int i = 0; i < TMF; ++i) ft[i] = *(const hcp_bf16x8*)(lt2 + (frow0 + i * 16 + fr) * TS2 + fg * 8);
#pragma unroll
            for (int i = 0; i < TMF; ++i)
#pragma unroll
                for (int j = 0; j < TNF; ++j) acc[i][j] = hcp_mfma16(fe[j], ft[i], acc[i][j]);
        }
    }

    if (p.nsplit > 1) {
#pragma unroll
        for (int i = 0; i < TMF; ++i) {
            const int m = m0 + frow0 + i * 16 + fr;
            if (m >= p.M) continue;
#pragma unroll
            for (int j = 0; j < TNF; ++j) {
                const int n = n0 + fcol0 + j * 16 + 4 * fg;
                if (j < nfin && n < p.N) *(hcp_f32x4*)(p.slabs + ((size_t)split * p.M + m) * p.N + n) = acc[i][j];
            }
        }
        return;
    }
    if (p.geglu_hg) {
        if (LORA) HCP_SYNC();
#pragma unroll
        for (int i = 0; i < TMF; ++i)
#pragma unroll
            for (int j = 0; j < TNF; ++j)
                if (j < nfin) geglu_tile_put(ring, geglu_tile_ld(BN), frow0 + i * 16 + fr, fcol0 + j * 16 + 4 * fg, acc[i][j], p.alpha);
        HCP_SYNC();
        geglu_tile_apply<BM, BN, NTC>(p, ring, m0, n0, tid_all);
        return;
    }
    if constexpr (!FIN_N) if (p.geglu_out) {
        static_assert((size_t)BM * BN * 2 <= (size_t)NST * BUF_ELEMS * sizeof(hcp_bf16), "the gelu(g) tile fits the ring");
        if (LORA) HCP_SYNC();
        hcp_f32x4 v[TMF][TN];
        int rows[TMF], cols[TN];
        const bool is_g = gn == 1;
#pragma unroll
        for (int j = 0; j < TN; ++j) cols[j] = tile_n * (BN / 2) + j * 16 + 4 * fg;
#pragma unroll
        for (int i = 0; i < TMF; ++i) {
            const int m = m0 + frow0 + i * 16 + fr;
            rows[i] = m;
#pragma unroll
            for (int j = 0; j < TN; ++j) {
                v[i][j] = acc[i][j] * p.alpha + bias_v[j];
                if (m < p.M) store_hi_lo(p, m, cols[j] + (is_g ? (p.N >> 1) : 0), v[i][j]);
            }
        }
        geglu_fwd_pair<TMF, TN>(v, is_g, wave_all >> 1, lane, (hcp_f32x4*)ring, [] { HCP_SYNC(); }, p.geglu_out, p.N >> 1, rows, p.M, cols);
        return;
    }
    if (p.epi_tile) {
        if (LORA) HCP_SYNC();
        float* const tile = (float*)ring;
#pragma unroll
        for (int i = 0; i < TMF; ++i) {
            const int ml = frow0 + i * 16 + fr, m = m0 + ml;
            const float* rbp = (p.rowbias && m < p.M) ? p.rowbias + (size_t)(m / p.rows_per_group) * p.rowbias_ld : nullptr;
#pragma unroll
            for (int j = 0; j < TNF; ++j) {
                if (j >= nfin) continue;
                const int nl = fcol0 + j * 16 + 4 * fg;
                hcp_f32x4 v = acc[i][j] * p.alpha + bias_v[j];
                if (rbp && n0 + nl < p.N) v += *(const hcp_f32x4*)(rbp + n0 + nl);
                *(hcp_f32x4*)(tile + ml * epi_tile_ld(BN) + nl) = v;
            }
        }
        HCP_SYNC();
        epi_tile_store<BM, BN, NTC>(p, tile, m0, n0, tid_all);
        return;
    }
#pragma unroll
    for (int i = 0; i < TMF; ++i) {
        const int m = m0 + frow0 + i * 16 + fr;
        if (m >= p.M) continue;
        hcp_f32x4 rb_v[TNF];
        if (p.rowbias) {
            const float* rbp = p.rowbias + (size_t)(m / p.rows_per_group) * p.rowbias_ld;
#pragma unroll
            for (int j = 0; j < TNF; ++j) {
                const int n = n0 + fcol0 + j * 16 + 4 * fg;
                hcp_f32x4 z = {0.f, 0.f, 0.f, 0.f};
                rb_v[j] = n < p.N ? *(const hcp_f32x4*)(rbp + n) : z;
            }
        }
#pragma unroll
        for (int j = 0; j < TNF; ++j) {
            const int n = n0 + fcol0 + j * 16 + 4 * fg;
            if (j >= nfin || n >= p.N) continue;
            hcp_f32x4 v = acc[i][j] * p.alpha + bias_v[j];
            if (p.rowbias) v += rb_v[j];
            if (p.residual) {
#pragma unroll
                for (int q = 0; q < 4; ++q) v[q] += hcp_bf2f((unsigned short)res_v[i][j][q]);
                add_residual_lo(p, m, n, v);
            }
            if (p.out_f32) *(hcp_f32x4*)((float*)p.D + (size_t)m * p.ldd + n) = v;
            else store_hi_lo(p, m, n, v);
        }
    }
}

template <int BM, int BN, int MODE, bool LORA>
int launch_pp(GemmParams& p, int ring, hipStream_t stream) {
    constexpr size_t stage = (size_t)(BM + BN + (LORA ? 32 : 0)) * BK * sizeof(hcp_bf16);
    constexpr size_t eimg = LORA ? (size_t)BN * 32 * sizeof(hcp_bf16) : 0;
    constexpr int TM = BM / 32, TN = BN / 32;
    constexpr int TMF = TM == 1 ? 1 : TM / 2, TNX = TM == 1 ? (TN + 1) / 2 : TN;
    constexpr size_t xchg = (size_t)8 * TMF * TNX * 64 * 16 + (LORA ? (size_t)8 * TMF * 64 * 16 : 0);
    constexpr size_t tail = LORA ? (size_t)2 * BM * 40 * sizeof(hcp_bf16) : 0;
    constexpr size_t tile_bytes = (size_t)BM * epi_tile_ld(BN) * sizeof(float);
    if (p.epi_tile && tile_bytes + eimg > 160 * 1024) p.epi_tile = 0;
    const size_t floor_ = (xchg > tail ? xchg : tail) > (p.epi_tile ? tile_bytes : 0) ? (xchg > tail ? xchg : tail) : tile_bytes;
    constexpr size_t cap = 160 * 1024;
    const dim3 grid(p.tiles_m * hcp_cdiv(p.N, BN), p.nsplit);
    if (ring >= 4 && 4 * stage + eimg <= cap) {
        constexpr int R = 4 * stage + eimg <= cap ? 4 : 2;
        const size_t sm = (R * stage > floor_ ? R * stage : floor_) + eimg;
        HCP_LAUNCH((gemm_pp_kernel<BM, BN, MODE, LORA, R>), grid, dim3(768), sm, stream, p);
    } else if (ring >= 3 && 3 * stage + eimg <= cap) {
        constexpr int R = 3 * stage + eimg <= cap ? 3 : 2;
        const size_t sm = (R * stage > floor_ ? R * stage : floor_) + eimg;
        HCP_LAUNCH((gemm_pp_kernel<BM, BN, MODE, LORA, R>), grid, dim3(768), sm, stream, p);
    } else {
        const size_t sm = (2 * stage > floor_ ? 2 * stage : floor_) + eimg;
        HCP_LAUNCH((gemm_pp_kernel<BM, BN, MODE, LORA, 2>), grid, dim3(768), sm, stream, p);
    }
    HCP_LAUNCH_CHECK("gemm_pp_kernel");
}

template <int BM, int BN>
int launch_pp_mode(GemmParams& p, int mode, bool lora, int ring, hipStream_t stream) {
    if (lora) return launch_pp<BM, BN, 0, true>(p, ring, stream);
    if (mode == 0) return launch_pp<BM, BN, 0, false>(p, ring, stream);
    if (mode == 1) return launch_pp<BM, BN, 1, false>(p, ring, stream);
    return launch_pp<BM, BN, 2, false>(p, ring, stream);
}

}

int gemm_pp_launch(GemmParams& p, int bm, int bn, int mode, bool lora, int ring, hipStream_t stream) {
    if (p.residual && (size_t)p.M * p.ldr * 2 >= (1ul << 31)) return -2;
    if (bm == 128 && bn == 160) return launch_pp_mode<128, 160>(p, mode, lora, ring, stream);
    if (bm == 64 && bn == 160) return launch_pp_mode<64, 160>(p, mode, lora, ring, stream);
    if (bm == 32 && bn == 160) {
        if (mode != 0 || p.geglu_out) return -2;
        return lora ? launch_pp<32, 160, 0, true>(p, ring, stream) : launch_pp<32, 160, 0, false>(p, ring, stream);
    }
    if (bm == 128 && bn == 128) return launch_pp_mode<128, 128>(p, mode, lora, ring, stream);
    return -2;
}

}
```

hcp_diffusion_amd/csrc/pack.hip:

```cpp
#include "hcp_common.h"

namespace {

struct PackPiece {
    const float* src;
    hcp_bf16* dst_rm;
    hcp_bf16* dst_tr;
    int rows, cols, src_ld, rm_ld, tr_ld;
    int tile0;
    int tiles_c;
    float scale;
};
static_assert(sizeof(PackPiece) == 56, "descriptor layout is part of the ABI");

HCP_KERNEL(256) pack_weights_kernel(const PackPiece* pieces, int count) {
    HCP_DYN_SMEM(smem);
    hcp_bf16* tile = (hcp_bf16*)smem;
    constexpr int TS = 66;
    int lo = 0, hi = count - 1;
    const int b = blockIdx.x;
    while (lo < hi) {
        const int mid = (lo + hi + 1) >> 1;
        if (pieces[mid].tile0 <= b) lo = mid; else hi = mid - 1;
    }
    const PackPiece pc = pieces[lo];
    const int t = b - pc.tile0;
    const int r0 = (t / pc.tiles_c) * 64, c0 = (t % pc.tiles_c) * 64;
    const int tid = threadIdx.x;
    const int cc = tid & 63, rg = tid >> 6;
#pragma unroll 4
    for (int i = 0; i < 16; ++i) {
        const int rr = rg + 4 * i;
        const int r = r0 + rr, c = c0 + cc;
        hcp_bf16 v = 0;
        if (r < pc.rows && c < pc.cols) {
            v = hcp_f2bf(pc.src[(size_t)r * pc.src_ld + c] * pc.scale);
            if (pc.dst_rm) pc.dst_rm[(size_t)r * pc.rm_ld + c] = v;
        }
        tile[rr * TS + cc] = v;
    }
    if (!pc.dst_tr) return;
    HCP_SYNC();
#pragma unroll 4
    for (int i = 0; i < 16; ++i) {
        const int ci = rg + 4 * i;
        const int c = c0 + ci, r = r0 + cc;
        if (c < pc.cols && r < pc.rows) pc.dst_tr[(size_t)c * pc.tr_ld + r] = tile[cc * TS + ci];
    }
}

}

HCP_API int hcp_pack_piece_bytes(void) { return (int)sizeof(PackPiece); }

HCP_API int hcp_pack_weights(const void* pieces, int count, int total_tiles, hipStream_t stream) {
    HCP_REQUIRE(pieces && count > 0 && total_tiles > 0, "hcp_pack_weights: bad arguments");
    HCP_LAUNCH(pack_weights_kernel, dim3(total_tiles), dim3(256), 64 * 66 * sizeof(hcp_bf16), stream, (const PackPiece*)pieces, count);
    HCP_LAUNCH_CHECK("pack_weights");
}
```

hcp_diffusion_amd/csrc/runtime.hip:

```cpp
#include "hcp_common.h"

static thread_local char g_err[512] = "";

extern "C" int hcp_set_error(const char* fmt, ...) {
    va_list ap;
    va_start(ap, fmt);
    vsnprintf(g_err, sizeof(g_err), fmt, ap);
    va_end(ap);
    return -1;
}

HCP_API const char* hcp_last_error(void) { return g_err; }

HCP_API int hcp_is_emulated(void) { return HCP_IS_EMULATED; }

HCP_API int hcp_abi_version(void) { return 4; }

namespace {
HCP_KERNEL(256) atomics_selfcheck_kernel(float* line, float* bucket, int nb, int stride) {
    const int tid = threadIdx.x;
    const float v = (float)((tid & 3) + 1);
    hcp_atomic_add(line + (tid & 15), v);
    const int idx = (int)(((long)blockIdx.x * 37 + (long)tid * 101) % nb);
    hcp_atomic_add(bucket + (size_t)idx * stride, v);
}
}

HCP_API int hcp_selfcheck_atomics(float* line, float* bucket, int nb, int stride, int workgroups, hipStream_t stream) {
    HCP_REQUIRE(line && bucket && nb > 0 && stride > 0 && workgroups > 0 && workgroups <= 4096, "hcp_selfcheck_atomics: bad arguments");
    if (hcp_memset_async(line, 0, 16 * sizeof(float), stream) != 0 || hcp_memset_async(bucket, 0, (size_t)nb * stride * sizeof(float), stream) != 0)
        return hcp_set_error("hcp_selfcheck_atomics: clearing the targets failed");
    HCP_LAUNCH(atomics_selfcheck_kernel, dim3(workgroups), dim3(256), 0, stream, line, bucket, nb, stride);
    HCP_LAUNCH_CHECK("atomics_selfcheck");
}
```

hcp_diffusion_amd/kernels.py:

```python
import ctypes
import math
import os
import torch

from . import _lib

_backend = None


def lib():
    global _backend
    if _backend is None:
        _backend = _lib.load()
    return _backend


def _set_backend_for_tests(cdll):
    global _backend
    _backend = _lib.bind(cdll) if cdll is not None else None


def _chk(rc, name):
    if rc != 0:
        raise _lib.HcpError(f"{name}: {lib().hcp_last_error().decode()}")


def _p(t):
    return None if t is None else t.data_ptr()


def _stream(t):
    if t.is_cuda:
        return torch.cuda.current_stream(t.device).cuda_stream
    if not lib().hcp_is_emulated():
        raise _lib.HcpError("hcp_diffusion_amd kernels need tensors on the HIP device (no CPU path)")
    return None


def _bf16_2d(t, name):
    assert t.dtype == torch.bfloat16 and t.dim() == 2 and t.stride(1) == 1, f"{name}: need 2-D bf16, unit inner stride"
    return t


BF16 = torch.bfloat16

_WS = {}
_WGTAB = {}
_WS_BYTES = 256 << 20
WGRAD_GRID_BLOCKS = 16384


def _workspace(t):
    key = (t.device.type, t.device.index)
    ws = _WS.get(key)
    if ws is None:
        ws = torch.empty(_WS_BYTES if t.is_cuda else (16 << 20), dtype=torch.uint8, device=t.device)
        _WS[key] = ws
    return ws


def atomics_selfcheck(device, workgroups=2048, nb=4099, stride=37):
    dev = torch.device(device)
    line = torch.empty(16, dtype=torch.float32, device=dev)
    bucket = torch.empty(nb * stride, dtype=torch.float32, device=dev)
    _chk(lib().hcp_selfcheck_atomics(_p(line), _p(bucket), nb, stride, workgroups, _stream(line)), "hcp_selfcheck_atomics")
    w = torch.arange(workgroups, dtype=torch.int64).view(-1, 1)
    t = torch.arange(256, dtype=torch.int64).view(1, -1)
    want_b = torch.zeros(nb, dtype=torch.int64).index_add_(0, ((37 * w + 101 * t) % nb).flatten(), ((t & 3) + 1).expand(workgroups, 256).flatten())
    want_l = workgroups * 16 * ((torch.arange(16) & 3) + 1)
    got_l, got_b = line.cpu().double(), bucket.cpu()[::stride].double()
    bad_l = int((got_l != want_l.double()).sum()); bad_b = int((got_b != want_b.double()).sum())
    if bad_l or bad_b:
        worst = float(((got_b - want_b.double()).abs() / want_b.double().clamp(min=1)).max())
        raise _lib.HcpError(f"fp32 atomics self-check FAILED on {dev}: {bad_l}/16 words of the shared line and {bad_b}/{nb} strided words differ "
                            f"from the exact integer sums (worst relative error {worst:.3g}); no result of this device can be trusted")
    return True


TRACE = None
LAUNCHES = None


def _launch(kind, **d):
    d["kind"] = kind
    LAUNCHES.append(d)


def _lo_pair(residual, residual_lo, want_lo, M, N, dev):
    if residual_lo is not None:
        assert residual is not None and residual_lo.dtype == BF16 and residual_lo.shape == (M, N) and residual_lo.stride() == residual.stride()
    return torch.empty((M, N), dtype=BF16, device=dev) if want_lo else None


def gemm(a, b, *, a2=None, b2=None, bias=None, rowbias=None, rows_per_group=1, residual=None, alpha=1.0,
         out_f32=False, out=None, residual_lo=None, want_lo=False, want_gact=False):
    _bf16_2d(a, "a"); _bf16_2d(b, "b")
    M, K = a.shape
    N = b.shape[0]
    assert b.shape[1] == K
    K2 = 0
    if a2 is not None:
        _bf16_2d(a2, "a2"); _bf16_2d(b2, "b2")
        K2 = a2.shape[1]
        assert a2.shape[0] == M and b2.shape == (N, K2)
    if TRACE is not None:
        TRACE.append(("gemm", M, N, K, 1 if K2 else 0))
    if out is None:
        out = torch.empty((M, N), dtype=torch.float32 if out_f32 else BF16, device=a.device)
    assert out.stride(1) == 1
    if LAUNCHES is not None:
        _launch("gemm", M=M, N=N, K=K, K2=K2, lda=a.stride(0), ldb=b.stride(0), ldd=out.stride(0),
                lda2=a2.stride(0) if K2 else 0, ldb2=b2.stride(0) if K2 else 0, ldr=residual.stride(0) if residual is not None else 0,
                bias=bias is not None, rowbias=rowbias is not None, rows_per_group=rows_per_group if rowbias is not None else 0,
                residual=residual is not None, residual_lo=residual_lo is not None, want_lo=bool(want_lo), gact=bool(want_gact),
                alpha=float(alpha), out_f32=out.dtype == torch.float32)
    if bias is not None:
        assert bias.dtype == torch.float32 and bias.numel() == N and bias.is_contiguous()
    if rowbias is not None:
        assert rowbias.dtype == torch.float32 and rowbias.shape[1] == N and rowbias.stride(1) == 1
    if residual is not None:
        _bf16_2d(residual, "residual"); assert residual.shape == (M, N)
    ws = _workspace(a)
    assert not want_lo or (out.dtype == BF16 and out.is_contiguous())
    out_lo = _lo_pair(residual, residual_lo, want_lo, M, N, a.device)
    gact = torch.empty((M, N // 2), dtype=BF16, device=a.device) if want_gact else None
    _chk(lib().hcp_gemm_bf16(_p(a), a.stride(0), _p(b), b.stride(0), _p(out), out.stride(0), M, N, K,
                             _p(a2), a2.stride(0) if a2 is not None else 0, _p(b2), b2.stride(0) if b2 is not None else 0,
                             K2, _p(bias), _p(rowbias), rowbias.stride(0) if rowbias is not None else 0, rows_per_group,
                             _p(residual), residual.stride(0) if residual is not None else 0, _p(residual_lo), _p(out_lo), _p(gact), float(alpha),
                             1 if out.dtype == torch.float32 else 0, _p(ws), ws.numel(), _stream(a)), "hcp_gemm_bf16")
    if want_gact:
        return out, gact
    return (out, out_lo) if want_lo else out


T_SPLIT = os.environ.get("HCP_T_SPLIT") == "1"


def t_lo(t):
    return 32 if (t is not None and T_SPLIT and t.shape[1] == 64 and t.stride(0) == 64) else 0


def gemm_lora(a, b, l, e, *, bias=None, residual=None, want_t=True, residual_lo=None, want_lo=False, want_gact=False):
    _bf16_2d(a, "a"); _bf16_2d(b, "b"); _bf16_2d(l, "l"); _bf16_2d(e, "e")
    M, Kd = a.shape
    N = b.shape[0]
    assert b.shape[1] == Kd and l.shape == (32, Kd) and e.shape == (N, 32) and l.is_contiguous() and e.is_contiguous()
    if TRACE is not None:
        TRACE.append(("lora", M, N, Kd))
    out = torch.empty((M, N), dtype=BF16, device=a.device)
    ldt = 64 if T_SPLIT else 32
    if LAUNCHES is not None:
        _launch("gemm_lora", M=M, N=N, K=Kd, lda=a.stride(0), ldb=b.stride(0), ldd=N, ldt=ldt, want_t=bool(want_t),
                ldr=residual.stride(0) if residual is not None else 0, bias=bias is not None, residual=residual is not None,
                residual_lo=residual_lo is not None, want_lo=bool(want_lo), gact=bool(want_gact))
    t = torch.empty((M, ldt), dtype=BF16, device=a.device) if want_t else None
    if bias is not None:
        assert bias.dtype == torch.float32 and bias.numel() == N and bias.is_contiguous()
    if residual is not None:
        _bf16_2d(residual, "residual"); assert residual.shape == (M, N)
    ws = _workspace(a)
    out_lo = _lo_pair(residual, residual_lo, want_lo, M, N, a.device)
    gact = torch.empty((M, N // 2), dtype=BF16, device=a.device) if want_gact else None
    _chk(lib().hcp_gemm_lora_bf16(_p(a), a.stride(0), _p(b), b.stride(0), _p(l), _p(e), _p(t), ldt, _p(out), N, M, N, Kd, _p(bias),
                                  _p(residual), residual.stride(0) if residual is not None else 0, _p(residual_lo), _p(out_lo), _p(gact),
                                  _p(ws), ws.numel(), _stream(a)),
         "hcp_gemm_lora_bf16")
    if want_gact:
        return (out, gact), t
    return ((out, out_lo) if want_lo else out), t


def gemm_geglu_bwd(dy, wt, hg, *, l=None, e=None, want_t=True):
    _bf16_2d(dy, "dy"); _bf16_2d(wt, "wt"); _bf16_2d(hg, "hg")
    M, C = dy.shape
    Fd = wt.shape[0]
    assert wt.shape[1] == C and hg.shape == (M, 2 * Fd) and hg.is_contiguous()
    if TRACE is not None:
        TRACE.append(("lora", M, Fd, C) if l is not None else ("gemm", M, Fd, C, 0))
    if LAUNCHES is not None:
        _launch("gemm_geglu_bwd", M=M, N=Fd, K=C, lda=dy.stride(0), ldb=wt.stride(0), ldd=2 * Fd, lora=l is not None,
                ldt=(64 if T_SPLIT else 32) if l is not None else 0, want_t=bool(want_t) and l is not None)
    dhg = torch.empty((M, 2 * Fd), dtype=BF16, device=dy.device)
    u = None
    if l is not None:
        _bf16_2d(l, "l"); _bf16_2d(e, "e")
        assert l.shape == (32, C) and e.shape == (Fd, 32) and l.is_contiguous() and e.is_contiguous()
        u = torch.empty((M, 64 if T_SPLIT else 32), dtype=BF16, device=dy.device) if want_t else None
    ws = _workspace(dy)
    _chk(lib().hcp_gemm_geglu_bwd_bf16(_p(dy), dy.stride(0), _p(wt), wt.stride(0), _p(l), _p(e), _p(u), 64 if T_SPLIT else 32, _p(hg), _p(dhg), M, Fd, C,
                                       _p(ws), ws.numel(), _stream(dy)), "hcp_gemm_geglu_bwd_bf16")
    return dhg, u


def conv3x3(x1, wp, cout, *, x2=None, stride=1, upsample=False, mode=0, out_hw=None, bias=None, rowbias=None,
            residual=None, out_f32=False, a2=None, b2=None, pad=1, out=None):
    assert x1.dtype == BF16 and x1.dim() == 4 and x1.is_contiguous()
    B, Hs, Ws, C1 = x1.shape
    C2 = 0
    if x2 is not None:
        assert x2.dtype == BF16 and x2.is_contiguous() and x2.shape[:3] == x1.shape[:3]
        C2 = x2.shape[3]
    assert wp.dtype == BF16 and wp.is_contiguous() and wp.numel() == cout * 9 * (C1 + C2)
    if mode == 0:
        up = 2 if upsample else 1
        Ho = (Hs * up + (2 if pad else 1) - 3) // stride + 1
        Wo = (Ws * up + (2 if pad else 1) - 3) // stride + 1
    else:
        Ho, Wo = out_hw
    if TRACE is not None:
        TRACE.append(("conv", mode, B, Hs, Ws, C1, C2, cout, stride, 1 if upsample else 0, Ho, Wo, 1 if a2 is not None else 0))
    if LAUNCHES is not None:
        _launch("conv3x3", M=B * Ho * Wo, N=cout, K=9 * (C1 + C2), K2=32 if a2 is not None else 0, mode=mode, B=B, Hs=Hs, Ws=Ws, C1=C1, C2=C2,
                Cout=cout, stride=stride, upsample=1 if upsample else 0, pad=pad, Ho=Ho, Wo=Wo, ldd=cout, ldr=cout if residual is not None else 0,
                bias=bias is not None, rowbias=rowbias is not None, rows_per_group=Ho * Wo if rowbias is not None else 0,
                residual=residual is not None, out_f32=bool(out_f32))
    if out is None:
        out = torch.empty((B, Ho, Wo, cout), dtype=torch.float32 if out_f32 else BF16, device=x1.device)
    assert out.dtype == (torch.float32 if out_f32 else BF16) and out.is_contiguous() and tuple(out.shape) == (B, Ho, Wo, cout)
    if residual is not None:
        assert residual.dtype == BF16 and residual.is_contiguous() and residual.numel() == out.numel()
    if rowbias is not None:
        assert rowbias.dtype == torch.float32 and rowbias.shape == (B, cout) and rowbias.stride(1) == 1
    if bias is not None:
        assert bias.dtype == torch.float32 and bias.numel() == cout and bias.is_contiguous()
    if a2 is not None:
        assert a2.dtype == BF16 and b2.dtype == BF16 and a2.is_contiguous() and b2.is_contiguous()
        assert a2.numel() == B * Ho * Wo * 32 and tuple(b2.shape) == (cout, 32)
    ws = _workspace(x1)
    _chk(lib().hcp_conv3x3_bf16(_p(x1), C1, _p(x2), C2, B, Hs, Ws, Ho, Wo, mode, stride, 1 if upsample else 0, pad, _p(wp),
                                cout, _p(out), cout, _p(bias), _p(rowbias), rowbias.stride(0) if rowbias is not None else 0,
                                _p(residual), cout, 1 if out_f32 else 0, _p(a2), _p(b2), _p(ws), ws.numel(), _stream(x1)),
         "hcp_conv3x3_bf16")
    return out


def wgrad_linear(dy, x, dw):
    assert dy.dtype == BF16 and x.dtype == BF16 and dw.dtype == torch.float32 and dy.dim() == 2 and x.dim() == 2
    assert dy.stride(1) == 1 and x.stride(1) == 1 and dw.stride(1) == 1 and dy.shape[0] == x.shape[0]
    M, N = dy.shape
    K = x.shape[1]
    assert tuple(dw.shape) == (N, K)
    if LAUNCHES is not None:
        _launch("wgrad_linear", M=M, N=N, K=K, ldy=dy.stride(0), ldx=x.stride(0), ldw=dw.stride(0))
    ws = _workspace(x)
    _chk(lib().hcp_wgrad_linear_bf16(_p(dy), dy.stride(0), _p(x), x.stride(0), _p(dw), dw.stride(0), M, N, K, _p(ws), ws.numel(),
                                     _stream(x)), "hcp_wgrad_linear_bf16")


def wgrad_conv3x3(dy, x1, dw, *, x2=None, stride=1, upsample=False, cout=None, col0=0):
    assert dy.dtype == BF16 and x1.dtype == BF16 and dw.dtype == torch.float32 and dy.is_contiguous() and x1.is_contiguous()
    B, Hs, Ws, C1 = x1.shape
    C2 = 0
    if x2 is not None:
        assert x2.dtype == BF16 and x2.is_contiguous() and x2.shape[:3] == x1.shape[:3]
        C2 = x2.shape[3]
    _, Ho, Wo, ldy = dy.shape
    cout = cout or ldy
    cw = dw.numel() // (cout * 9)
    assert dw.numel() == cout * 9 * cw and cw <= C1 + C2
    ws = _workspace(x1)
    assert col0 % 8 == 0 and col0 + (cout + 7) // 8 * 8 <= ldy
    if LAUNCHES is not None:
        _launch("wgrad_conv3x3", M=B * Ho * Wo, N=cout, K=9 * (C1 + C2), B=B, Hs=Hs, Ws=Ws, C1=C1, C2=C2, Cout=cout, Cw=cw, stride=stride,
                upsample=1 if upsample else 0, Ho=Ho, Wo=Wo, ldy=ldy, col0=col0)
    dyp = ctypes.c_void_p(dy.data_ptr() + 2 * col0)
    _chk(lib().hcp_wgrad_conv3x3_bf16(dyp, ldy, _p(x1), C1, _p(x2), C2, _p(dw), cw, B, Hs, Ws, Ho, Wo, cout, stride,
                                      1 if upsample else 0, _p(ws), ws.numel(), _stream(x1)), "hcp_wgrad_conv3x3_bf16")


def colsum(y, out, rows_per_group=None):
    assert y.dtype == BF16 and y.dim() == 2 and y.stride(1) == 1 and out.dtype == torch.float32
    M, N = y.shape
    rpg = rows_per_group or M
    ldo = out.stride(0) if out.dim() == 2 else N
    _chk(lib().hcp_colsum_bf16(_p(y), y.stride(0), _p(out), ldo, M, N, rpg, _stream(y)), "hcp_colsum_bf16")


def _attn_strides(t):
    assert t.dtype == BF16 and t.dim() == 3 and t.stride(2) == 1
    return t.stride(0), t.stride(1)


def _key_bias(key_bias, B, Nk):
    if key_bias is None:
        return None, 0
    assert key_bias.dtype == torch.float32 and tuple(key_bias.shape) == (B, Nk) and key_bias.stride(1) == 1
    return key_bias, key_bias.stride(0)


def _attn_desc(q, k, v, B, H, Nq, Nk, D, scale, kbt, kbs, causal, pre):
    C = H * D
    e = q.element_size()
    kv = k.stride() == v.stride() and v.data_ptr() - k.data_ptr() == C * e and k.stride(1) >= 2 * C
    qkv = kv and q.stride() == k.stride() and k.data_ptr() - q.data_ptr() == C * e and q.stride(1) >= 3 * C
    return dict(B=B, H=H, Nq=Nq, Nk=Nk, D=D, q_bs=q.stride(0), q_rs=q.stride(1), k_bs=k.stride(0), k_rs=k.stride(1), v_bs=v.stride(0),
                v_rs=v.stride(1), layout="qkv" if qkv else "q+kv" if kv else "separate", key_bias=kbt is not None, kb_bs=kbs,
                causal=bool(causal), prescaled=bool(pre), scale=0.0 if abs(scale * math.sqrt(D) - 1.0) < 1e-6 else float(scale))


def attention_fwd(q, k, v, heads, scale=None, key_bias=None, causal=False, q_prescaled=False):
    B, Nq, C = q.shape
    Nk = k.shape[1]
    D = C // heads
    scale = scale if scale is not None else 1.0 / math.sqrt(D)
    o = torch.empty((B, Nq, C), dtype=BF16, device=q.device)
    lse = torch.empty((B, heads, Nq), dtype=torch.float32, device=q.device)
    qb, qr = _attn_strides(q); kb, kr = _attn_strides(k); vb, vr = _attn_strides(v); ob, orr = _attn_strides(o)
    kbt, kbs = _key_bias(key_bias, B, Nk)
    if LAUNCHES is not None:
        _launch("attn_fwd", **_attn_desc(q, k, v, B, heads, Nq, Nk, D, scale, kbt, kbs, causal, q_prescaled))
    _chk(lib().hcp_attention_fwd(_p(q), _p(k), _p(v), _p(o), _p(lse), B, heads, Nq, Nk, D, qb, qr, kb, kr, vb, vr, ob, orr,
                                 float(scale), _p(kbt), kbs, (1 if causal else 0) | (2 if q_prescaled else 0), _stream(q)), "hcp_attention_fwd")
    return o, lse


def attention_bwd(q, k, v, o, do, lse, heads, scale=None, out=None, key_bias=None, causal=False, q_prescaled=False):
    B, Nq, C = q.shape
    Nk = k.shape[1]
    D = C // heads
    scale = scale if scale is not None else 1.0 / math.sqrt(D)
    assert o.is_contiguous() and do.is_contiguous()
    if out is None:
        assert q.is_contiguous() and k.is_contiguous() and v.is_contiguous(), "strided q/k/v need matching `out` buffers"
        dq = torch.empty_like(q); dk = torch.empty_like(k); dv = torch.empty_like(v)
    else:
        dq, dk, dv = out
        assert dq.stride() == q.stride() and dk.stride() == k.stride() and dv.stride() == v.stride()
    delta = torch.empty((B, heads, Nq), dtype=torch.float32, device=q.device)
    qb, qr = _attn_strides(q); kb, kr = _attn_strides(k); vb, vr = _attn_strides(v); ob, orr = _attn_strides(o)
    ws = _workspace(q)
    kbt, kbs = _key_bias(key_bias, B, Nk)
    if LAUNCHES is not None:
        _launch("attn_bwd", **_attn_desc(q, k, v, B, heads, Nq, Nk, D, scale, kbt, kbs, causal, q_prescaled))
    _chk(lib().hcp_attention_bwd(_p(q), _p(k), _p(v), _p(o), _p(do), _p(lse), _p(delta), _p(dq), _p(dk), _p(dv), B, heads,
                                 Nq, Nk, D, qb, qr, kb, kr, vb, vr, ob, orr, float(scale), _p(kbt), kbs,
                                 (1 if causal else 0) | (2 if q_prescaled else 0), _p(ws),
                                 ws.numel(), _stream(q)), "hcp_attention_bwd")
    return dq, dk, dv


def _gn_ws(x, B, HW, C, G):
    n = lib().hcp_groupnorm_workspace_bytes(B, HW, C, G)
    return torch.empty((max(n, 4) // 4,), dtype=torch.float32, device=x.device)


def groupnorm_fwd(x, gamma, beta, groups, eps, silu):
    assert x.dtype == BF16 and x.is_contiguous()
    B, C = x.shape[0], x.shape[-1]
    HW = x.numel() // (B * C)
    y = torch.empty_like(x)
    stats = torch.empty((B, groups, 2), dtype=torch.float32, device=x.device)
    ws = _gn_ws(x, B, HW, C, groups)
    _chk(lib().hcp_groupnorm_silu_fwd(_p(x), _p(gamma), _p(beta), _p(y), _p(stats), _p(ws), B, HW, C, groups, float(eps),
                                      1 if silu else 0, _stream(x)), "hcp_groupnorm_silu_fwd")
    return y, stats


def groupnorm_bwd(x, dy, gamma, beta, stats, groups, silu, addend=None):
    assert x.dtype == BF16 and x.is_contiguous() and dy.dtype == BF16 and dy.is_contiguous()
    assert addend is None or (addend.dtype == BF16 and addend.is_contiguous() and addend.numel() == x.numel())
    B, C = x.shape[0], x.shape[-1]
    HW = x.numel() // (B * C)
    dx = torch.empty_like(x)
    ws = _gn_ws(x, B, HW, C, groups)
    _chk(lib().hcp_groupnorm_silu_bwd(_p(x), _p(dy), _p(gamma), _p(beta), _p(stats), _p(addend), _p(dx), _p(ws), B, HW, C, groups,
                                      1 if silu else 0, _stream(x)), "hcp_groupnorm_silu_bwd")
    return dx


def groupnorm_affine_grad(x, dy, gamma, beta, stats, groups, silu, dgamma, dbeta):
    B, C = x.shape[0], x.shape[-1]
    HW = x.numel() // (B * C)
    assert x.is_contiguous() and dy.is_contiguous() and dgamma.dtype == torch.float32 and dbeta.dtype == torch.float32
    _chk(lib().hcp_groupnorm_affine_grad(_p(x), _p(dy), _p(gamma), _p(beta), _p(stats), _p(dgamma), _p(dbeta), B, HW, C, groups,
                                         1 if silu else 0, _stream(x)), "hcp_groupnorm_affine_grad")


def layernorm_affine_grad(x, dy, stats, dgamma, dbeta):
    C = x.shape[-1]
    M = x.numel() // C
    assert x.is_contiguous() and dy.is_contiguous() and dgamma.dtype == torch.float32 and dbeta.dtype == torch.float32
    _chk(lib().hcp_layernorm_affine_grad(_p(x), _p(dy), _p(stats), _p(dgamma), _p(dbeta), M, C, _stream(x)),
         "hcp_layernorm_affine_grad")


def _lo_like(t, ref):
    assert t is None or (t.dtype == BF16 and t.is_contiguous() and t.numel() == ref.numel())
    return t


def layernorm_fwd(x, gamma, beta, eps, x_lo=None):
    assert x.dtype == BF16 and x.is_contiguous()
    C = x.shape[-1]; M = x.numel() // C
    y = torch.empty_like(x)
    stats = torch.empty((M, 2), dtype=torch.float32, device=x.device)
    _chk(lib().hcp_layernorm_fwd(_p(x), _p(_lo_like(x_lo, x)), _p(gamma), _p(beta), _p(y), _p(stats), M, C, float(eps), _stream(x)), "hcp_layernorm_fwd")
    return y, stats


def layernorm_bwd(x, dy, gamma, stats, addend=None, x_lo=None, addend_lo=None, want_lo=False):
    assert x.is_contiguous() and dy.is_contiguous() and dy.dtype == BF16
    assert addend is None or (addend.dtype == BF16 and addend.is_contiguous() and addend.numel() == x.numel())
    C = x.shape[-1]; M = x.numel() // C
    dx = torch.empty_like(x)
    dx_lo = torch.empty_like(x) if want_lo else None
    _chk(lib().hcp_layernorm_bwd(_p(x), _p(_lo_like(x_lo, x)), _p(dy), _p(gamma), _p(stats), _p(addend), _p(_lo_like(addend_lo, x)), _p(dx),
                                 _p(dx_lo), M, C, _stream(x)), "hcp_layernorm_bwd")
    return (dx, dx_lo) if want_lo else dx


def geglu_fwd(h):
    assert h.dtype == BF16 and h.is_contiguous()
    F2 = h.shape[-1]; F = F2 // 2; M = h.numel() // F2
    y = torch.empty(h.shape[:-1] + (F,), dtype=BF16, device=h.device)
    _chk(lib().hcp_geglu_fwd(_p(h), _p(y), M, F, _stream(h)), "hcp_geglu_fwd")
    return y


def geglu_bwd(h, dy):
    assert h.is_contiguous() and dy.is_contiguous() and dy.dtype == BF16
    F2 = h.shape[-1]; F = F2 // 2; M = h.numel() // F2
    dh = torch.empty_like(h)
    _chk(lib().hcp_geglu_bwd(_p(h), _p(dy), _p(dh), M, F, _stream(h)), "hcp_geglu_bwd")
    return dh


def add(a, b):
    assert a.dtype == BF16 and b.dtype == BF16 and a.is_contiguous() and b.is_contiguous() and a.numel() == b.numel()
    o = torch.empty_like(a)
    _chk(lib().hcp_add_bf16(_p(a), _p(b), _p(o), a.numel(), _stream(a)), "hcp_add_bf16")
    return o


def concat_channels(a, b):
    assert a.dtype == BF16 and b.dtype == BF16 and a.is_contiguous() and b.is_contiguous() and a.shape[:-1] == b.shape[:-1]
    c1, c2 = a.shape[-1], b.shape[-1]
    M = a.numel() // c1
    out = torch.empty(a.shape[:-1] + (c1 + c2,), dtype=BF16, device=a.device)
    o2 = out.view(M, c1 + c2)
    _chk(lib().hcp_concat2_bf16(_p(a), c1, _p(b), c2, _p(o2), M, 0, _stream(a)), "hcp_concat2_bf16")
    return out


def split_channels(d, c1):
    assert d.dtype == BF16 and d.is_contiguous()
    c = d.shape[-1]; c2 = c - c1
    M = d.numel() // c
    d2 = d.view(M, c)
    a = torch.empty(d.shape[:-1] + (c1,), dtype=BF16, device=d.device)
    b = torch.empty(d.shape[:-1] + (c2,), dtype=BF16, device=d.device)
    _chk(lib().hcp_concat2_bf16(_p(a), c1, _p(b), c2, _p(d2), M, 1, _stream(d)), "hcp_concat2_bf16")
    return a, b


def silu_fwd(x):
    assert x.dtype == BF16 and x.is_contiguous()
    y = torch.empty_like(x)
    _chk(lib().hcp_silu_fwd(_p(x), _p(y), x.numel(), _stream(x)), "hcp_silu_fwd")
    return y


def silu_bwd(x, dy):
    dx = torch.empty_like(x)
    _chk(lib().hcp_silu_bwd(_p(x), _p(dy), _p(dx), x.numel(), _stream(x)), "hcp_silu_bwd")
    return dx


def nchw_to_nhwc(x, cpad=None):
    assert x.dim() == 4 and x.is_contiguous() and x.dtype in (torch.float32, BF16)
    B, C, H, W = x.shape
    cp = cpad or C
    y = torch.empty((B, H, W, cp), dtype=BF16, device=x.device)
    _chk(lib().hcp_nchw_to_nhwc_bf16(_p(x), 1 if x.dtype == torch.float32 else 0, _p(y), B, C, H * W, cp, _stream(x)),
         "hcp_nchw_to_nhwc_bf16")
    return y


def nhwc_to_nchw_f32(x, c):
    assert x.dim() == 4 and x.is_contiguous() and x.dtype == torch.float32
    B, H, W, Cs = x.shape
    y = torch.empty((B, c, H, W), dtype=torch.float32, device=x.device)
    _chk(lib().hcp_nhwc_to_nchw_f32(_p(x), _p(y), B, c, H * W, Cs, _stream(x)), "hcp_nhwc_to_nchw_f32")
    return y


def upsample2x_bwd(dup):
    assert dup.dtype == BF16 and dup.is_contiguous()
    B, H2, W2, C = dup.shape
    dx = torch.empty((B, H2 // 2, W2 // 2, C), dtype=BF16, device=dup.device)
    _chk(lib().hcp_upsample2x_bwd(_p(dup), _p(dx), B, H2 // 2, W2 // 2, C, _stream(dup)), "hcp_upsample2x_bwd")
    return dx


def timestep_embedding(t, dim, max_period=10000.0):
    assert t.dtype in (torch.int64, torch.float32) and t.is_contiguous()
    emb = torch.empty((t.numel(), dim), dtype=BF16, device=t.device)
    if t.dtype == torch.int64:
        _chk(lib().hcp_timestep_embedding(_p(t), _p(emb), t.numel(), dim, float(max_period), _stream(t)), "hcp_timestep_embedding")
    else:
        _chk(lib().hcp_timestep_embedding_f32(_p(t), _p(emb), t.numel(), dim, float(max_period), _stream(t)),
             "hcp_timestep_embedding_f32")
    return emb


def add_noise(x0, noise, t, alphas_cumprod):
    assert x0.dtype == torch.float32 and noise.dtype == torch.float32 and x0.is_contiguous() and noise.is_contiguous()
    assert t.dtype == torch.int64 and alphas_cumprod.dtype == torch.float32
    xt = torch.empty_like(x0)
    B = x0.shape[0]
    _chk(lib().hcp_add_noise(_p(x0), _p(noise), _p(t), _p(alphas_cumprod), _p(xt), B, x0.numel() // B, _stream(x0)), "hcp_add_noise")
    return xt


def cfg_ddim_step(x, eps2, a_t, a_prev, guidance_scale=1.0, out=None):
    assert x.dtype == torch.float32 and eps2.dtype == torch.float32 and x.is_contiguous() and eps2.is_contiguous()
    guided = eps2.numel() == 2 * x.numel()
    assert guided or eps2.numel() == x.numel()
    out = torch.empty_like(x) if out is None else out
    _chk(lib().hcp_cfg_ddim_step(_p(x), _p(eps2), _p(out), x.numel(), 1 if guided else 0, float(guidance_scale), float(a_t), float(a_prev),
                                 _stream(x)), "hcp_cfg_ddim_step")
    return out


def quick_gelu(x, dy=None):
    assert x.dtype == BF16 and x.is_contiguous() and (dy is None or (dy.dtype == BF16 and dy.is_contiguous() and dy.shape == x.shape))
    out = torch.empty_like(x)
    _chk(lib().hcp_quick_gelu(_p(x), _p(dy), _p(out), x.numel(), _stream(x)), "hcp_quick_gelu")
    return out


def embedding(token_table, ids, position_table, position_ids=None):
    assert token_table.dtype == torch.float32 and position_table.dtype == torch.float32 and token_table.is_contiguous() and position_table.is_contiguous()
    assert ids.dtype == torch.int64 and ids.is_contiguous() and (position_ids is None or (position_ids.dtype == torch.int64 and position_ids.shape == ids.shape))
    C, L = token_table.shape[1], ids.shape[-1]
    out = torch.empty(tuple(ids.shape) + (C,), dtype=BF16, device=ids.device)
    _chk(lib().hcp_embedding_bf16(_p(token_table), _p(ids), _p(position_table), _p(position_ids.contiguous() if position_ids is not None else None),
# ... 238 lines not shown
```

hcp_diffusion_amd/layers.py:

```python
import torch
from torch import nn

from . import ops

BF16 = torch.bfloat16


class _Packed:
    pass


def _key(*ts):
    return tuple((t._version, t.data_ptr(), t.device) if t is not None else None for t in ts)


def _same_storage(k_old, k_new):
    return len(k_old) == len(k_new) and all((a is None) == (b is None) and (a is None or a[1:] == b[1:]) for a, b in zip(k_old, k_new))


def _pad_last(t, mult):
    c = t.shape[-1]
    cp = (c + mult - 1) // mult * mult
    if cp == c:
        return t
    out = t.new_zeros(t.shape[:-1] + (cp,))
    out[..., :c] = t
    return out


class HipLinear(nn.Linear):
    supports_fused_residual = True
    _pk = None

    def packed(self):
        k = _key(self.weight, self.bias)
        if self._pk is None or self._pk.key != k:
            w = self.weight.detach()
            if self._pk is not None and _same_storage(self._pk.key, k):
                pk = self._pk
                pk.w.copy_(w); pk.wt.copy_(w.t())
                if pk.bias is not None and pk.bias.data_ptr() != self.bias.data_ptr():
                    pk.bias.copy_(self.bias.detach())
                pk.key = k
                return pk
            pk = _Packed(); pk.key = k
            pk.w = w.to(BF16).contiguous()
            pk.wt = w.t().to(BF16).contiguous()
            pk.bias = self.bias.detach().float().contiguous() if self.bias is not None else None
            self._pk = pk
        return self._pk

    def forward(self, x, residual=None, out_f32=False):
        return ops.linear(x, self, None, residual, out_f32)


class HipConv2d(nn.Conv2d):
    supports_fused_residual = True
    _pk = None

    def __init__(self, *args, **kwargs):
        super().__init__(*args, **kwargs)
        if self.kernel_size == (3, 3):
            self.weight.data = self.weight.data.contiguous(memory_format=torch.channels_last)

    def packed(self):
        k = _key(self.weight, self.bias)
        if self._pk is None or self._pk.key != k:
            w = self.weight.detach()
            if self._pk is not None and _same_storage(self._pk.key, k):
                pk = self._pk
                if self.kernel_size == (1, 1):
                    w2 = w.reshape(pk.cout, pk.cin)
                    pk.w.copy_(w2); pk.wt.copy_(w2.t())
                else:
                    pk.w[..., :pk.cin].copy_(w.permute(0, 2, 3, 1)); pk.wd[..., :pk.cout].copy_(w.permute(1, 2, 3, 0))
                if pk.bias is not None and pk.bias.data_ptr() != self.bias.data_ptr():
                    pk.bias.copy_(self.bias.detach())
                pk.key = k
                return pk
            pk = _Packed(); pk.key = k
            cout, cin = w.shape[0], w.shape[1]
            pk.cout, pk.cin = cout, cin
            pk.bias = self.bias.detach().float().contiguous() if self.bias is not None else None
            if self.kernel_size == (1, 1):
                w2 = w.reshape(cout, cin)
                pk.w = w2.to(BF16).contiguous(); pk.wt = w2.t().to(BF16).contiguous()
            else:
                assert self.kernel_size == (3, 3) and (self.padding == (1, 1) or (self.padding == (0, 0) and self.stride == (2, 2))), \
                    "only 3x3 (padding 1, or the VAE's padding-0 stride-2 downsample) and 1x1 convolutions exist in SD models"
                pk.cin_pad = (cin + 7) // 8 * 8
                pk.cout_pad = (cout + 7) // 8 * 8
                pk.w = _pad_last(w.permute(0, 2, 3, 1), 8).to(BF16).contiguous()
                pk.wd = _pad_last(w.permute(1, 2, 3, 0), 8).to(BF16).contiguous()
            self._pk = pk
        return self._pk

    def forward(self, x, residual=None, x2=None, rowbias=None, upsample=False):
        if self.kernel_size == (1, 1):
            assert x2 is None and rowbias is None and not upsample
            return ops.linear(x, self, None, residual)
        return ops.conv3x3(x, self, x2=x2, rowbias=rowbias, residual=residual, stride=self.stride[0], upsample=upsample)


class HipConvIn(HipConv2d):

    def forward(self, sample):
        return ops.conv_in(sample, self)


class HipConvOut(HipConv2d):

    def forward(self, x):
        return ops.conv_out(x, self)


class _F32Affine:
    _af = None

    def f32_params(self):
        k = _key(self.weight, self.bias)
        if self._af is None or self._af[0] != k:
            if self._af is not None and _same_storage(self._af[0], k):
                for dst, src in ((self._af[1], self.weight), (self._af[2], self.bias)):
                    if dst.data_ptr() != src.data_ptr():
                        dst.copy_(src.detach())
                self._af = (k, self._af[1], self._af[2])
            else:
                self._af = (k, self.weight.detach().float().contiguous(), self.bias.detach().float().contiguous())
        return self._af[1], self._af[2]


class HipGroupNorm(_F32Affine, nn.GroupNorm):
    def forward(self, x, silu=False, fork=False):
        return ops.groupnorm_fork(x, self, silu) if fork else ops.groupnorm(x, self, silu)


class HipLayerNorm(_F32Affine, nn.LayerNorm):
    def forward(self, x, fork=False):
        return ops.layernorm_fork(x, self) if fork else ops.layernorm(x, self)
```

hcp_diffusion_amd/ops.py:

```python
import os
import threading
from contextlib import contextmanager

import torch

from . import kernels as K

BF16 = torch.bfloat16



class WgradContext:
    def __init__(self, grouped=False, side_stream=False):
        self.grouped, self.side = bool(grouped), bool(side_stream)
        self.items, self.keep = [], []
        self.stream, self.side_keep = None, []

    def add(self, U, x2, gd, T, dy2, gu, rank, alpha, slot0=0, ulo=0, tlo=0):
        if self.grouped:
            self.items.append((U, x2, gd, T, dy2, gu, rank, alpha, slot0, ulo, tlo))
            return
        if slot0 != 0 or not dy2.is_contiguous() or (ulo != 0) != (U.shape[1] == 64) or (tlo != 0) != (T.shape[1] == 64):
            self.keep = [K.lora_wgrad_grouped([(U, x2, gd, T, dy2, gu, rank, alpha, slot0, ulo, tlo)])]
            return
        if not (self.side and x2.is_cuda):
            K.lora_wgrad_pair(U, x2, gd, T, dy2, gu, rank, alpha)
            return
        if self.stream is None:
            self.stream = torch.cuda.Stream(device=x2.device)
        ev = torch.cuda.Event()
        ev.record()
        self.stream.wait_event(ev)
        with torch.cuda.stream(self.stream):
            K.lora_wgrad_pair(U, x2, gd, T, dy2, gu, rank, alpha)
        self.side_keep.append((U, x2, T, dy2))

    def flush(self):
        if self.items:
            keep = K.lora_wgrad_grouped(self.items)
            self.keep = [keep, self.items]
            self.items = []

    def join(self):
        if self.stream is not None and self.side_keep:
            torch.cuda.current_stream().wait_stream(self.stream)
        self.side_keep.clear()


_IMMEDIATE = WgradContext()
_tls = threading.local()


def current_wgrad():
    return getattr(_tls, "ctx", None) or _IMMEDIATE


@contextmanager
def wgrad_context(ctx):
    prev = getattr(_tls, "ctx", None)
    _tls.ctx = ctx
    try:
        yield ctx
    finally:
        _tls.ctx = prev


def _tr(p):
    return p if (p is not None and p.requires_grad and torch.is_grad_enabled()) else None


def grad_buffer(p, conv3x3=False):
    g = p.grad
    if g is None:
        if conv3x3:
            g = torch.zeros((p.shape[0], 3, 3, p.shape[1]), dtype=torch.float32, device=p.device).permute(0, 3, 1, 2)
        else:
            g = torch.zeros(p.shape, dtype=torch.float32, device=p.device)
        p.grad = g
    if g.dtype != torch.float32:
        raise TypeError("hcp_diffusion_amd: host gradients accumulate in fp32 (fp32 master parameters expected)")
    if conv3x3:
        g = g.permute(0, 2, 3, 1)
    if not g.is_contiguous():
        raise RuntimeError("hcp_diffusion_amd: .grad of a trainable host parameter must be dense (3x3 conv weights: channels_last)")
    return g


class _LinearFn(torch.autograd.Function):

    @staticmethod
    def forward(ctx, x, residual, w_down, w_up, host, lora, out_f32=False, hw=None, hb=None, residual_lo=None, stream=False, geglu=False):
        shp = x.shape
        x2 = x.reshape(-1, shp[-1])
        res2 = residual.reshape(-1, residual.shape[-1]) if residual is not None else None
        lo2 = residual_lo.reshape(-1, residual_lo.shape[-1]) if residual_lo is not None else None
        pk = host.packed()
        T = None
        if lora is not None and getattr(lora, "wide", False):
            lp = lora.packed()
            T = K.gemm(x2, lp.ad)
            y = K.gemm(x2, pk.w, a2=T, b2=lp.bu, bias=pk.bias, residual=res2, residual_lo=lo2, want_lo=stream, want_gact=geglu)
        elif lora is not None:
            lp = lora.packed()
            y, T = K.gemm_lora(x2, pk.w, lp.ad, lp.bu, bias=pk.bias, residual=res2, residual_lo=lo2, want_lo=stream, want_gact=geglu)
        else:
            y = K.gemm(x2, pk.w, bias=pk.bias, residual=res2, out_f32=out_f32, residual_lo=lo2, want_lo=stream, want_gact=geglu)
        ctx.host, ctx.lora = host, lora
        ctx.wg = current_wgrad()
        ctx.train_w, ctx.train_b = hw is not None, hb is not None
        ctx.save_for_backward(x2 if (lora is not None or hw is not None) else None, T)
        ctx.xshape = shp
        ctx.has_res = residual is not None
        ctx.stream, ctx.has_lo = stream, residual_lo is not None
        if geglu:
            act = y[1].view(*shp[:-1], y[1].shape[-1])
            ctx.mark_non_differentiable(act)
            ctx.set_materialize_grads(False)
            return y[0].view(*shp[:-1], y[0].shape[-1]), act
        if stream:
            ctx.set_materialize_grads(False)
            return y[0].view(*shp[:-1], y[0].shape[-1]), y[1].view(*shp[:-1], y[1].shape[-1])
        return y.view(*shp[:-1], y.shape[-1])

    @staticmethod
    def backward(ctx, dy, dy_lo=None):
        if dy is None:
            assert dy_lo is None
            return (None,) * 12
        x2, T = ctx.saved_tensors
        host, lora = ctx.host, ctx.lora
        dy2 = dy.reshape(-1, dy.shape[-1])
        if not dy2.is_contiguous():
            dy2 = dy2.contiguous()
        pk = host.packed()
        dx = None
        if lora is not None and getattr(lora, "wide", False):
            lp = lora.packed()
            U = K.gemm(dy2, lp.but)
            if ctx.needs_input_grad[0]:
                dx = K.gemm(dy2, pk.wt, a2=U, b2=lp.wdt)
            for blk, s0 in lora.members():
                gd, gu = blk.grad_views()
                for j in range(0, blk.rank, 32):
                    pj = min(32, blk.rank - j)
                    K.lora_wgrad(U[:, s0 + j:s0 + j + 32], x2, gd[j:j + pj], pj, 1.0, False)
                    K.lora_wgrad(T[:, s0 + j:s0 + j + 32], dy2, gu, pj, blk.alpha_f, True, out_col0=j)
        elif lora is not None:
            lp = lora.packed()
            if ctx.needs_input_grad[0]:
                dx, U = K.gemm_lora(dy2, pk.wt, lp.but, lp.adt)
            else:
                U = K.gemm(dy2, lp.but)
            for blk, s0 in lora.members():
                gd, gu = blk.grad_views()
                ctx.wg.add(U, x2, gd, T, dy2, gu, blk.rank, blk.alpha_f, s0, K.t_lo(U), K.t_lo(T))
        elif ctx.needs_input_grad[0]:
            dx = K.gemm(dy2, pk.wt)
        if ctx.train_w:
            gw = grad_buffer(host.weight)
            K.wgrad_linear(dy2, x2, gw.view(gw.shape[0], -1))
        if ctx.train_b:
            K.colsum(dy2, grad_buffer(host.bias))
        if dx is not None:
            dx = dx.view(ctx.xshape)
        return dx, (dy if ctx.has_res else None), None, None, None, None, None, None, None, (dy_lo if ctx.has_lo else None), None, None


def linear_geglu(x, host, lora=None):
    wd = lora.layer.W_down if lora is not None else None
    wu = lora.layer.W_up if lora is not None else None
    return _LinearFn.apply(x, None, wd, wu, host, lora, False, _tr(host.weight), _tr(host.bias), None, False, True)


def linear(x, host, lora=None, residual=None, out_f32=False):
    wd = lora.layer.W_down if lora is not None else None
    wu = lora.layer.W_up if lora is not None else None
    hw, hb = _tr(host.weight), _tr(host.bias)
    if out_f32 and (lora is not None or x.requires_grad or hw is not None or hb is not None):
        raise NotImplementedError("hcp_diffusion_amd: fp32 linear output is only provided for the gradient-free time-embedding path")
    return _LinearFn.apply(x, residual, wd, wu, host, lora, out_f32, hw, hb)


def linear_stream(x, host, lora, hi, lo):
    wd = lora.layer.W_down if lora is not None else None
    wu = lora.layer.W_up if lora is not None else None
    return _LinearFn.apply(x, hi, wd, wu, host, lora, False, _tr(host.weight), _tr(host.bias), lo, True)


class _LinearGroupFn(torch.autograd.Function):

    @staticmethod
    def forward(ctx, x, group, *lora_params):
        shp = x.shape
        x2 = x.reshape(-1, shp[-1])
        w, _ = group.packed_host()
        T = None
        if group.has_lora:
            o = group.bucket.packed_group(group)
            y, T = K.gemm_lora(x2, w, o.ad, o.bu)
        else:
            y = K.gemm(x2, w)
        ctx.group = group
        ctx.wg = current_wgrad()
        ctx.save_for_backward(x2 if group.has_lora else None, T)
        ctx.xshape = shp
        return y.view(*shp[:-1], group.n_total)

    @staticmethod
    def backward(ctx, dy):
        x2, T = ctx.saved_tensors
        g = ctx.group
        dy2 = dy.reshape(-1, g.n_total)
        if not dy2.is_contiguous():
            dy2 = dy2.contiguous()
        _, wt = g.packed_host()
        dx = None
        if g.has_lora:
            o = g.bucket.packed_group(g)
            if ctx.needs_input_grad[0]:
                dx, U = K.gemm_lora(dy2, wt, o.but, o.adt)
            else:
                U = K.gemm(dy2, o.but)
            for blk, n0, s0, host, sc_ in zip(g.blocks, g.n_off, g.slot_off, g.hosts, g.out_scale):
                if blk is not None:
                    gd, gu = blk.grad_views()
                    ctx.wg.add(U, x2, gd, T, dy2[:, n0:n0 + host.weight.shape[0]], gu, blk.rank, blk.alpha_f * sc_, s0, K.t_lo(U), K.t_lo(T))
        elif ctx.needs_input_grad[0]:
            dx = K.gemm(dy2, wt)
        if dx is not None:
            dx = dx.view(ctx.xshape)
        return (dx, None) + (None,) * (len(ctx.needs_input_grad) - 2)


class _CtxKVFn(torch.autograd.Function):

    @staticmethod
    def forward(ctx, x, batch, *lora_params):
        shp = x.shape
        x2 = x.reshape(-1, shp[-1])
        ad_all, b_cat = batch.operands()
        T_all = None
        if ad_all is not None and batch.split:
            T_all = K.split_hi_lo(K.gemm(x2, ad_all, out_f32=True))
            y = K.gemm(K.concat_channels(x2, T_all), b_cat)
        elif ad_all is not None:
            T_all = K.gemm(x2, ad_all)
            y = K.gemm(K.concat_channels(x2, T_all), b_cat)
        else:
            y = K.gemm(x2, b_cat)
        ctx.batch, ctx.wg = batch, current_wgrad()
        ctx.dkv_all = torch.empty_like(y)
        ctx.save_for_backward(x2, T_all)
        y3 = y.view(*shp[:-1], batch.n_total)
        return tuple(y3[..., o:o + g.n_total] for g, o in zip(batch.groups, batch.n_off))

    @staticmethod
    def backward(ctx, *dkvs):
        x2, T_all = ctx.saved_tensors
        batch, dall = ctx.batch, ctx.dkv_all
        joint = T_all is not None and batch.all_have_lora() and all(d is not None for d in dkvs)
        for g, off, d in zip(batch.groups, batch.n_off, dkvs):
            if d is None or not g.has_lora:
                continue
            sl = dall[:, off:off + g.n_total]
            d2 = d.reshape(-1, g.n_total) if d.dim() != 2 else d
            if d2.data_ptr() != sl.data_ptr() or d2.stride() != sl.stride():
                sl.copy_(d2)
        U_all = None
        if joint:
            batch.operands()
            U_all = K.split_hi_lo(K.gemm(dall, batch.but_all, out_f32=True)) if batch.split else K.gemm(dall, batch.but_all)
        for gi, (g, off, d) in enumerate(zip(batch.groups, batch.n_off, dkvs)):
            if d is None or not g.has_lora:
                continue
            sl = dall[:, off:off + g.n_total]
            U = U_all[:, 32 * gi:32 * gi + 32] if joint else K.gemm(sl, g.bucket.packed_group(g).but)
            T = T_all[:, 32 * gi:32 * gi + 32]
            for blk, n0, s0, host, sc_ in zip(g.blocks, g.n_off, g.slot_off, g.hosts, g.out_scale):
                if blk is not None:
                    gd, gu = blk.grad_views()
                    ctx.wg.add(U, x2, gd, T, sl[:, n0:n0 + host.weight.shape[0]], gu, blk.rank, blk.alpha_f * sc_, s0,
                               batch.k2 if (joint and batch.split) else 0, batch.k2 if batch.split else 0)
        return (None, None) + (None,) * (len(ctx.needs_input_grad) - 2)


def ctx_kv(x, batch):
    assert not x.requires_grad
    params = [p for g in batch.groups for b in g.blocks if b is not None for p in (b.layer.W_down, b.layer.W_up)]
    outs = _CtxKVFn.apply(x, batch, *params)
    node = outs[0].grad_fn
    if node is not None:
        d3 = node.dkv_all.view(*x.shape[:-1], batch.n_total)
        for kv, g, o in zip(outs, batch.groups, batch.n_off):
            kv._hcp_grad_buf = d3[..., o:o + g.n_total]
    return outs


def linear_group(x, group):
    for h in group.hosts:
        assert _tr(h.weight) is None and _tr(h.bias) is None, "fused projection groups require frozen host weights"
    params = [p for b in group.blocks if b is not None for p in (b.layer.W_down, b.layer.W_up)]
    return _LinearGroupFn.apply(x, group, *params)


class _Conv3x3Fn(torch.autograd.Function):

    @staticmethod
    def forward(ctx, x1, x2, rowbias, residual, host, stride, upsample, hw=None, hb=None, lora=None, w_down=None, w_up=None):
        pk = host.packed()
        T = None
        if lora is not None and getattr(lora, "wide", False):
            lp = lora.packed()
            rp = lora.rank_pad
            T = K.conv3x3(x1, lp.ad, rp, x2=x2, stride=stride, upsample=upsample)
            y0 = K.conv3x3(x1, pk.w, pk.cout, x2=x2, stride=stride, upsample=upsample, bias=pk.bias, rowbias=rowbias, residual=residual)
            y = K.gemm(T.view(-1, rp), lp.bu, residual=y0.view(-1, pk.cout)).view_as(y0)
        elif lora is not None:
            lp = lora.packed()
            T = K.conv3x3(x1, lp.ad, 32, x2=x2, stride=stride, upsample=upsample)
            y = K.conv3x3(x1, pk.w, pk.cout, x2=x2, stride=stride, upsample=upsample, bias=pk.bias, rowbias=rowbias, residual=residual,
                          a2=T, b2=lp.bu)
        else:
            y = K.conv3x3(x1, pk.w, pk.cout, x2=x2, stride=stride, upsample=upsample, bias=pk.bias, rowbias=rowbias, residual=residual)
        ctx.host, ctx.stride, ctx.upsample, ctx.lora = host, stride, upsample, lora
        ctx.in_shape = x1.shape
        ctx.c2 = x2.shape[-1] if x2 is not None else 0
        ctx.has_res = residual is not None
        ctx.train_w, ctx.train_b = hw is not None, hb is not None
        keep_x = hw is not None or lora is not None
        ctx.save_for_backward(x1 if keep_x else None, x2 if keep_x else None, T)
        return y

    @staticmethod
    def backward(ctx, dy):
        pk = ctx.host.packed()
        dy = dy.contiguous()
        B, H, W, C1 = ctx.in_shape
        hw = (H * 2, W * 2) if ctx.upsample else (H, W)
        dx1 = dx2 = None
        x1, x2, T = ctx.saved_tensors
        lora = ctx.lora
        dl1 = dl2 = None
        if lora is not None:
            lp = lora.packed()
            rp = lp.but.shape[0]
            U = K.gemm(dy.view(-1, dy.shape[-1]), lp.but).view(*dy.shape[:-1], rp)
            T2 = T.view(-1, rp)
            for blk, s0 in lora.members():
                gd, gu = blk.grad_views()
                for j in range(0, blk.rank, 32):
                    K.lora_wgrad(T2[:, s0 + j:], dy.view(-1, dy.shape[-1]), gu, min(32, blk.rank - j), blk.alpha_f, True, out_col0=j)
                K.wgrad_conv3x3(U, x1, gd, x2=x2, stride=ctx.stride, upsample=ctx.upsample, cout=blk.rank, col0=s0)
            if ctx.needs_input_grad[0]:
                dl1 = K.conv3x3(U, lp.wdl[:C1], C1, mode=1, stride=ctx.stride, out_hw=hw)
            if ctx.c2 and ctx.needs_input_grad[1]:
                dl2 = K.conv3x3(U, lp.wdl[C1:], ctx.c2, mode=1, stride=ctx.stride, out_hw=hw)
        if ctx.needs_input_grad[0]:
            dx1 = K.conv3x3(dy, pk.wd[:C1], C1, mode=1, stride=ctx.stride, out_hw=hw, residual=dl1)
            if ctx.upsample:
                dx1 = K.upsample2x_bwd(dx1)
        if ctx.c2 and ctx.needs_input_grad[1]:
            dx2 = K.conv3x3(dy, pk.wd[C1:], ctx.c2, mode=1, stride=ctx.stride, out_hw=hw, residual=dl2)
        drb = None
        dy2 = dy.view(-1, dy.shape[-1])
        if ctx.needs_input_grad[2]:
            drb = torch.zeros((B, dy.shape[-1]), dtype=torch.float32, device=dy.device)
            K.colsum(dy2, drb, dy.shape[1] * dy.shape[2])
        if ctx.train_w:
            K.wgrad_conv3x3(dy, x1, grad_buffer(ctx.host.weight, True), x2=x2, stride=ctx.stride, upsample=ctx.upsample)
        if ctx.train_b:
            K.colsum(dy2, grad_buffer(ctx.host.bias))
        return dx1, dx2, drb, (dy if ctx.has_res else None), None, None, None, None, None, None, None, None


def conv3x3(x1, host, *, x2=None, rowbias=None, residual=None, stride=1, upsample=False, lora=None):
    wd = lora.layer.W_down if lora is not None else None
    wu = lora.layer.W_up if lora is not None else None
    return _Conv3x3Fn.apply(x1, x2, rowbias, residual, host, stride, upsample, _tr(host.weight), _tr(host.bias), lora, wd, wu)


def _gn_affine(ctx, x, dy, g, b, stats):
    if ctx.train:
        K.groupnorm_affine_grad(x, dy, g, b, stats, ctx.gn.num_groups, ctx.silu, grad_buffer(ctx.gn.weight), grad_buffer(ctx.gn.bias))


def _norm_tr(m):
    w, b = _tr(m.weight), _tr(m.bias)
    if (w is None) != (b is None):
        raise NotImplementedError("hcp_diffusion_amd: a norm layer's weight and bias must be trainable together")
    return w, b


class _GroupNormFn(torch.autograd.Function):
    @staticmethod
    def forward(ctx, x, gn, silu, hw=None, hb=None):
        g, b = gn.f32_params()
        y, stats = K.groupnorm_fwd(x, g, b, gn.num_groups, gn.eps, silu)
        ctx.save_for_backward(x, stats)
        ctx.gn, ctx.silu, ctx.train = gn, silu, hw is not None
        return y

    @staticmethod
    def backward(ctx, dy):
        x, stats = ctx.saved_tensors
        g, b = ctx.gn.f32_params()
        dy = dy.contiguous()
        _gn_affine(ctx, x, dy, g, b, stats)
        dx = K.groupnorm_bwd(x, dy, g, b, stats, ctx.gn.num_groups, ctx.silu) if ctx.needs_input_grad[0] else None
        return dx, None, None, None, None


def groupnorm(x, gn, silu):
    return _GroupNormFn.apply(x, gn, silu, *_norm_tr(gn))


class _GroupNormForkFn(torch.autograd.Function):

    @staticmethod
    def forward(ctx, x, gn, silu, hw=None, hb=None):
        g, b = gn.f32_params()
        y, stats = K.groupnorm_fwd(x, g, b, gn.num_groups, gn.eps, silu)
        ctx.save_for_backward(x, stats)
        ctx.gn, ctx.silu, ctx.train = gn, silu, hw is not None
        return y, x.view_as(x)

    @staticmethod
    def backward(ctx, dy, dskip):
        x, stats = ctx.saved_tensors
        g, b = ctx.gn.f32_params()
        if dy is None:
            return dskip, None, None, None, None
        dy = dy.contiguous()
        _gn_affine(ctx, x, dy, g, b, stats)
        return K.groupnorm_bwd(x, dy, g, b, stats, ctx.gn.num_groups, ctx.silu,
                               dskip.contiguous() if dskip is not None else None), None, None, None, None


def groupnorm_fork(x, gn, silu):
    return _GroupNormForkFn.apply(x, gn, silu, *_norm_tr(gn))


class _LayerNormFn(torch.autograd.Function):
    @staticmethod
    def forward(ctx, x, ln, hw=None, hb=None):
        g, b = ln.f32_params()
        y, stats = K.layernorm_fwd(x, g, b, ln.eps)
        ctx.save_for_backward(x, stats)
        ctx.ln, ctx.train = ln, hw is not None
        return y

    @staticmethod
    def backward(ctx, dy):
        x, stats = ctx.saved_tensors
        g, _ = ctx.ln.f32_params()
        dy = dy.contiguous()
        if ctx.train:
            K.layernorm_affine_grad(x, dy, stats, grad_buffer(ctx.ln.weight), grad_buffer(ctx.ln.bias))
        return (K.layernorm_bwd(x, dy, g, stats) if ctx.needs_input_grad[0] else None), None, None, None


def layernorm(x, ln):
    return _LayerNormFn.apply(x, ln, *_norm_tr(ln))


class _LayerNormForkFn(torch.autograd.Function):

    @staticmethod
    def forward(ctx, x, ln, hw=None, hb=None, x_lo=None, stream=False):
        g, b = ln.f32_params()
        y, stats = K.layernorm_fwd(x, g, b, ln.eps, x_lo=x_lo)
        ctx.save_for_backward(x, stats, x_lo)
        ctx.ln, ctx.train, ctx.stream = ln, hw is not None, stream
        if stream:
            ctx.set_materialize_grads(False)
            return y, x.view_as(x), (x_lo.view_as(x_lo) if x_lo is not None else None)
        return y, x.view_as(x)

    @staticmethod
    def backward(ctx, dy, dskip, dskip_lo=None):
        x, stats, x_lo = ctx.saved_tensors
        g, _ = ctx.ln.f32_params()
        if dy is None:
            return dskip, None, None, None, dskip_lo, None
        dy = dy.contiguous()
        if ctx.train:
            K.layernorm_affine_grad(x, dy, stats, grad_buffer(ctx.ln.weight), grad_buffer(ctx.ln.bias))
        if ctx.stream:
            want_lo = x_lo is not None
            r = K.layernorm_bwd(x, dy, g, stats, dskip.contiguous() if dskip is not None else None, x_lo=x_lo,
                                addend_lo=dskip_lo.contiguous() if (dskip_lo is not None and dskip is not None) else None, want_lo=want_lo)
            return (r[0], None, None, None, r[1], None) if want_lo else (r, None, None, None, None, None)
        return K.layernorm_bwd(x, dy, g, stats, dskip.contiguous() if dskip is not None else None), None, None, None, None, None


def layernorm_fork(x, ln):
    return _LayerNormForkFn.apply(x, ln, *_norm_tr(ln))


def layernorm_fork_stream(hi, lo, ln):
    return _LayerNormForkFn.apply(hi, ln, *_norm_tr(ln), lo, True)


class _GegluFn(torch.autograd.Function):
    @staticmethod
    def forward(ctx, h):
        ctx.save_for_backward(h)
        return K.geglu_fwd(h)

    @staticmethod
    def backward(ctx, dy):
        (h,) = ctx.saved_tensors
        return K.geglu_bwd(h, dy.contiguous())


geglu = _GegluFn.apply


class _GegluLinearFn(torch.autograd.Function):

    @staticmethod
    def forward(ctx, hg, residual, w_down, w_up, host, lora, hw=None, hb=None, residual_lo=None, stream=False, gact=None):
        shp = hg.shape
        hg2 = hg.reshape(-1, shp[-1])
        x2 = gact.reshape(-1, gact.shape[-1]) if gact is not None else K.geglu_fwd(hg2)
        res2 = residual.reshape(-1, residual.shape[-1]) if residual is not None else None
        lo2 = residual_lo.reshape(-1, residual_lo.shape[-1]) if residual_lo is not None else None
        pk = host.packed()
        T = None
        if lora is not None:
            lp = lora.packed()
            y, T = K.gemm_lora(x2, pk.w, lp.ad, lp.bu, bias=pk.bias, residual=res2, residual_lo=lo2, want_lo=stream)
        else:
            y = K.gemm(x2, pk.w, bias=pk.bias, residual=res2, residual_lo=lo2, want_lo=stream)
        ctx.host, ctx.lora = host, lora
        ctx.wg = current_wgrad()
        ctx.train_w, ctx.train_b = hw is not None, hb is not None
        ctx.save_for_backward(hg2, x2 if (lora is not None or hw is not None) else None, T)
        ctx.hshape = shp
        ctx.has_res = residual is not None
        ctx.has_lo = residual_lo is not None
        if stream:
            ctx.set_materialize_grads(False)
            return y[0].view(*shp[:-1], y[0].shape[-1]), y[1].view(*shp[:-1], y[1].shape[-1])
        return y.view(*shp[:-1], y.shape[-1])

    @staticmethod
    def backward(ctx, dy, dy_lo=None):
        if dy is None:
            assert dy_lo is None
            return (None,) * 11
        hg2, x2, T = ctx.saved_tensors
        host, lora = ctx.host, ctx.lora
        dy2 = dy.reshape(-1, dy.shape[-1])
        if not dy2.is_contiguous():
            dy2 = dy2.contiguous()
        pk = host.packed()
        dhg = None
        if lora is not None:
            lp = lora.packed()
            if ctx.needs_input_grad[0]:
                dhg, U = K.gemm_geglu_bwd(dy2, pk.wt, hg2, l=lp.but, e=lp.adt)
            else:
                U = K.gemm(dy2, lp.but)
            for blk, s0 in lora.members():
                gd, gu = blk.grad_views()
                ctx.wg.add(U, x2, gd, T, dy2, gu, blk.rank, blk.alpha_f, s0, K.t_lo(U), K.t_lo(T))
        elif ctx.needs_input_grad[0]:
            dhg, _ = K.gemm_geglu_bwd(dy2, pk.wt, hg2)
        if ctx.train_w:
            gw = grad_buffer(host.weight)
            K.wgrad_linear(dy2, x2, gw.view(gw.shape[0], -1))
        if ctx.train_b:
            K.colsum(dy2, grad_buffer(host.bias))
        if dhg is not None:
            dhg = dhg.view(ctx.hshape)
        return dhg, (dy if ctx.has_res else None), None, None, None, None, None, None, (dy_lo if ctx.has_lo else None), None, None


def geglu_linear(hg, host, lora=None, residual=None, gact=None):
    wd = lora.layer.W_down if lora is not None else None
    wu = lora.layer.W_up if lora is not None else None
    if isinstance(residual, tuple):
        return _GegluLinearFn.apply(hg, residual[0], wd, wu, host, lora, _tr(host.weight), _tr(host.bias), residual[1], True, gact)
    return _GegluLinearFn.apply(hg, residual, wd, wu, host, lora, _tr(host.weight), _tr(host.bias), None, False, gact)


class _AttentionFn(torch.autograd.Function):
    @staticmethod
    def forward(ctx, q, k, v, heads, key_bias=None, causal=False):
        o, lse = K.attention_fwd(q, k, v, heads, key_bias=key_bias, causal=causal)
        ctx.save_for_backward(q, k, v, o, lse, key_bias)
        ctx.heads, ctx.causal = heads, causal
        return o

    @staticmethod
    def backward(ctx, do):
        q, k, v, o, lse, key_bias = ctx.saved_tensors
        dq, dk, dv = K.attention_bwd(q.contiguous(), k.contiguous(), v.contiguous(), o, do.contiguous(), lse, ctx.heads,
                                     key_bias=key_bias, causal=ctx.causal)
        return dq, dk, dv, None, None, None


def attention(q, k, v, heads, key_bias=None, causal=False):
    return _AttentionFn.apply(q, k, v, heads, key_bias, causal)


class _QuickGeluFn(torch.autograd.Function):
    @staticmethod
    def forward(ctx, x):
        ctx.save_for_backward(x)
        return K.quick_gelu(x)

    @staticmethod
    def backward(ctx, dy):
        (x,) = ctx.saved_tensors
        return K.quick_gelu(x, dy.contiguous())


def quick_gelu(x):
    return _QuickGeluFn.apply(x)


class _AttentionPackedFn(torch.autograd.Function):

    @staticmethod
    def forward(ctx, a, kv, heads, key_bias=None, q_prescaled=False):
        if kv is None:
            C = a.shape[-1] // 3
            q, k, v = a[..., :C], a[..., C:2 * C], a[..., 2 * C:]
        else:
            C = a.shape[-1]
            q, k, v = a, kv[..., :C], kv[..., C:]
        o, lse = K.attention_fwd(q, k, v, heads, key_bias=key_bias, q_prescaled=q_prescaled)
        ctx.save_for_backward(a, kv, o, lse, key_bias)
        ctx.heads, ctx.C, ctx.pre = heads, C, q_prescaled
        ctx.dkv_buf = getattr(kv, "_hcp_grad_buf", None)
        return o

    @staticmethod
    def backward(ctx, do):
        a, kv, o, lse, key_bias = ctx.saved_tensors
        C = ctx.C
        if kv is None:
            da = torch.empty_like(a)
            q, k, v = a[..., :C], a[..., C:2 * C], a[..., 2 * C:]
            K.attention_bwd(q, k, v, o, do.contiguous(), lse, ctx.heads, out=(da[..., :C], da[..., C:2 * C], da[..., 2 * C:]),
                            key_bias=key_bias, q_prescaled=ctx.pre)
            return da, None, None, None, None
        da = torch.empty_like(a)
        dkv = ctx.dkv_buf if ctx.dkv_buf is not None else torch.empty_like(kv)
        if dkv.stride() != kv.stride():
            dkv = torch.empty_strided(kv.shape, kv.stride(), dtype=kv.dtype, device=kv.device)
        K.attention_bwd(a, kv[..., :C], kv[..., C:], o, do.contiguous(), lse, ctx.heads, out=(da, dkv[..., :C], dkv[..., C:]),
                        key_bias=key_bias, q_prescaled=ctx.pre)
        return da, dkv, None, None, None


def attention_packed(a, kv, heads, key_bias=None, q_prescaled=False):
    return _AttentionPackedFn.apply(a, kv, heads, key_bias, q_prescaled)

# ... 236 lines not shown
```

include/hcp_mi355x.h:

```cpp
#ifndef HCP_MI355X_H
#define HCP_MI355X_H
#include <stddef.h>

#ifdef __cplusplus
extern "C" {
#endif

typedef struct ihipStream_t* hcpStream_t;

const char* hcp_last_error(void);
int hcp_is_emulated(void);
#define HCP_ABI_VERSION 4
int hcp_abi_version(void);
int hcp_selfcheck_atomics(float* line, float* bucket, int nb, int stride, int workgroups, hcpStream_t stream);

int hcp_gemm_bf16(const void* A, int lda, const void* B, int ldb, void* D, int ldd, int M, int N, int K, const void* A2,
                  int lda2, const void* B2, int ldb2, int K2, const float* bias, const float* rowbias, int rowbias_ld,
                  int rows_per_group, const void* residual, int ldr, const void* residual_lo, void* D_lo, void* gact, float alpha,
                  int out_f32, void* workspace, size_t workspace_bytes, hcpStream_t stream);
int hcp_gemm_lora_bf16(const void* A, int lda, const void* B, int ldb, const void* L, const void* E, void* Tout, int ldt, void* D,
                       int ldd, int M, int N, int K, const float* bias, const void* residual, int ldr, const void* residual_lo, void* D_lo,
                       void* gact, void* workspace, size_t workspace_bytes, hcpStream_t stream);
int hcp_gemm_geglu_bwd_bf16(const void* A, int lda, const void* B, int ldb, const void* L, const void* E, void* Tout, int ldt,
                            const void* HG, void* DHG, int M, int F, int K, void* workspace, size_t workspace_bytes, hcpStream_t stream);
size_t hcp_gemm_workspace_bytes(int M, int N);

int hcp_conv3x3_bf16(const void* X1, int C1, const void* X2, int C2, int B, int Hs, int Ws, int Ho, int Wo, int mode,
                     int stride, int upsample, int pad, const void* Wp, int Cout, void* D, int ldd, const float* bias,
                     const float* rowbias, int rowbias_ld, const void* residual, int ldr, int out_f32, const void* A2,
                     const void* B2, void* workspace, size_t workspace_bytes, hcpStream_t stream);

int hcp_attention_fwd(const void* Q, const void* K, const void* V, void* O, float* lse, int B, int H, int Nq, int Nk, int D,
                      long q_bs, int q_rs, long k_bs, int k_rs, long v_bs, int v_rs, long o_bs, int o_rs, float scale,
                      const float* key_bias, long key_bias_bs, int causal, hcpStream_t stream);
int hcp_attention_bwd(const void* Q, const void* K, const void* V, const void* O, const void* dO, const float* lse,
                      float* delta_ws , void* dQ, void* dK, void* dV, int B, int H, int Nq, int Nk, int D,
                      long q_bs, int q_rs, long k_bs, int k_rs, long v_bs, int v_rs, long o_bs, int o_rs, float scale,
                      const float* key_bias, long key_bias_bs, int causal, void* workspace, size_t workspace_bytes,
                      hcpStream_t stream);


size_t hcp_groupnorm_workspace_bytes(int B, int HW, int C, int G);
int hcp_groupnorm_silu_fwd(const void* x, const float* gamma, const float* beta, void* y, float* stats, void* workspace,
                           int B, int HW, int C, int G, float eps, int silu, hcpStream_t stream);
int hcp_groupnorm_silu_bwd(const void* x, const void* dy, const float* gamma, const float* beta, const float* stats,
                           const void* addend , void* dx,
                           void* workspace, int B, int HW, int C, int G, int silu, hcpStream_t stream);

int hcp_layernorm_fwd(const void* x, const void* x_lo, const float* gamma, const float* beta, void* y, float* stats, int M, int C,
                      float eps, hcpStream_t stream);
int hcp_layernorm_bwd(const void* x, const void* x_lo, const void* dy, const float* gamma, const float* stats, const void* addend,
                      const void* addend_lo, void* dx, void* dx_lo, int M, int C, hcpStream_t stream);

int hcp_geglu_fwd(const void* h, void* y, long M, int F, hcpStream_t stream);
int hcp_geglu_bwd(const void* h, const void* dy, void* dh, long M, int F, hcpStream_t stream);

int hcp_add_bf16(const void* a, const void* b, void* out, long n, hcpStream_t stream);
int hcp_copy2d_bf16(const void* src, int sld, void* dst, int dld, long M, int C, hcpStream_t stream);
int hcp_concat2_bf16(void* a, int c1, void* b, int c2, void* joint, long M, int split, hcpStream_t stream);
int hcp_silu_fwd(const void* x, void* y, long n, hcpStream_t stream);
int hcp_silu_bwd(const void* x, const void* dy, void* dx, long n, hcpStream_t stream);
int hcp_nchw_to_nhwc_bf16(const void* src, int src_is_f32, void* dst, int B, int C, int HW, int Cpad, hcpStream_t stream);
int hcp_nhwc_to_nchw_f32(const float* src, float* dst, int B, int C, int HW, int Csrc, hcpStream_t stream);
int hcp_upsample2x_bwd(const void* dup, void* dx, int B, int H, int W, int C, hcpStream_t stream);

int hcp_wgrad_linear_bf16(const void* dY, int ldy, const void* X, int ldx, float* dW, int ldw, int M, int N, int K,
                          float* workspace, size_t workspace_bytes, hcpStream_t stream);
int hcp_wgrad_conv3x3_bf16(const void* dY, int ldy, const void* X1, int C1, const void* X2, int C2, float* dW, int Cw, int B,
                           int Hs, int Ws, int Ho, int Wo, int Cout, int stride, int upsample, float* workspace,
                           size_t workspace_bytes, hcpStream_t stream);
int hcp_colsum_bf16(const void* Y, int ldy, float* out, int ldo, int M, int N, int rows_per_group, hcpStream_t stream);
int hcp_pack_piece_bytes(void);
int hcp_pack_weights(const void* pieces, int count, int total_tiles, hcpStream_t stream);
int hcp_groupnorm_affine_grad(const void* x, const void* dy, const float* gamma, const float* beta, const float* stats,
                              float* dgamma, float* dbeta, int B, int HW, int C, int G, int silu, hcpStream_t stream);
int hcp_layernorm_affine_grad(const void* x, const void* dy, const float* stats, float* dgamma, float* dbeta, int M, int C,
                              hcpStream_t stream);

int hcp_timestep_embedding(const long long* timesteps, void* emb, int B, int dim, float max_period, hcpStream_t stream);
int hcp_timestep_embedding_f32(const float* values, void* emb, int B, int dim, float max_period, hcpStream_t stream);
int hcp_add_noise(const float* x0, const float* noise, const long long* timesteps, const float* alphas_cumprod, float* xt,
                  int B, long per_sample, hcpStream_t stream);
int hcp_transpose_bf16(const void* src, void* dst, int batch, int R, int C, hcpStream_t stream);
int hcp_softmax_rows(const float* S, long lds, void* P, long ldp, int M, int N, float scale, hcpStream_t stream);
int hcp_vae_latent_sample(const float* moments, const float* Wq, const float* bq, const float* noise, float* latents, int B, int L,
                          long hw, float scale, hcpStream_t stream);
int hcp_quick_gelu(const void* x, const void* dy, void* out, long n, hcpStream_t stream);
int hcp_embedding_bf16(const float* token_table, const long long* ids, const float* position_table, const long long* position_ids,
                       void* out, long n, int C, int L, hcpStream_t stream);
int hcp_embedding_pt_fwd_bf16(const long long* ids, int B, int R, int W, int n_word, const float* token_table, int vocab,
                              const float* position_table, const long long* position_ids, int n_pos, const float* custom_table,
                              int n_custom, const int* custom_map, int n_map, void* out, int* src_map, int C, hcpStream_t stream);
int hcp_embedding_pt_bwd_f32(const void* dX, const int* src_map, long M, int C, float* grad, int n_custom, int beta, hcpStream_t stream);
int hcp_snr_loss_weight(const long long* timesteps, const float* alphas_cumprod, float* w, int B, int kind, float gamma,
                        hcpStream_t stream);
int hcp_mse_masked_mean(const float* pred, const float* target, const float* mask, int mask_channels,
                        const float* sample_weight, float* loss, float* grad, int B, int C, int HW, float weight,
                        hcpStream_t stream);

int hcp_lora_wgrad(const void* L, int ldl, int l_lo, const void* R, int ldr, float* out, int ldo, int M, int P, int Q, float scale,
                   int transpose_out, void* workspace, size_t workspace_bytes, hcpStream_t stream);
int hcp_lora_wgrad_pair(const void* U, int ldu, const void* x, int ldx, int K, float* grad_down, const void* T, int ldt, const void* dY,
                        int ldy, int N, float* grad_up, int M, int r, float scale, void* workspace, size_t workspace_bytes,
                        hcpStream_t stream);
int hcp_split_hi_lo_bf16(const float* src, void* dst, long M, int C, hcpStream_t stream);
int hcp_lora_wgrad_group_geometry(int M, int K, int N, int P, int target_blocks, int* qt_down, int* qt_up, int* splits,
                                  int* rows_per_split);
int hcp_lora_wgrad_group_desc_bytes(void);
int hcp_lora_wgrad_grouped(const void* descs, int count, int total_blocks, int total_tiles, long slab_units, void* workspace,
                           size_t workspace_bytes, hcpStream_t stream);
int hcp_lora_pack(const void* descs, int count, hcpStream_t stream);
int hcp_lora_pack_desc_bytes(void);

int hcp_sumsq_f32(const float* g, long n, float* out, hcpStream_t stream);
int hcp_adamw_clip_fused(float* p, float* g, float* m, float* v, long n, const float* lr, float beta1, float beta2,
                         float eps, float weight_decay, const float* sumsq, float grad_scale, float max_norm, int* step,
                         hcpStream_t stream);
int hcp_ema_update(float* ema, const float* p, long n, const int* step, float inv_gamma, float power, float decay_max,
                   hcpStream_t stream);
int hcp_cast_f32_bf16(float* src, void* dst_bf16, long n, float scale, int zero_src, hcpStream_t stream);
int hcp_cast_bf16_f32(const void* src_bf16, float* dst, long n, hcpStream_t stream);

int hcp_cfg_ddim_step(const float* x, const float* eps2, float* out, long n, int guided, float guidance_scale,
                      float alpha_cumprod_t, float alpha_cumprod_prev, hcpStream_t stream);


#define HCP_COMM_UNIQUE_ID_BYTES 128
int hcp_comm_unique_id(void* out128);
int hcp_comm_init(int rank, int world, const void* unique_id128, void** comm_out);
int hcp_comm_destroy(void* comm);
int hcp_comm_rank(const void* comm);
int hcp_comm_world(const void* comm);
int hcp_allreduce_flat(void* comm, void* buf, size_t count, int dtype, hcpStream_t stream);
int hcp_reduce_scatter_flat(void* comm, const void* send, void* recv, size_t recv_count, int dtype, hcpStream_t stream);
int hcp_allgather_flat(void* comm, const void* send, void* recv, size_t send_count, int dtype, hcpStream_t stream);

#ifdef __cplusplus
}
#endif
#endif
```

include/hcp_mi355x_tools.h:

```cpp
#ifndef HCP_MI355X_TOOLS_H
#define HCP_MI355X_TOOLS_H
#include "hcp_mi355x.h"
#ifdef __cplusplus
extern "C" {
#endif
int hcp_debug_gemm_table_stats(long* hits, long* misses);
int hcp_debug_set_gemm_config(int cfg);
int hcp_debug_set_gemm_ablation(int flags);
int hcp_debug_set_gn_target(int workgroups);
int hcp_debug_set_gemm_epilogue(int mode);
int hcp_debug_set_conv_patch(int on);
int hcp_debug_set_gemm_loaders(int mode);
int hcp_debug_set_gemm_glds(int on);
int hcp_debug_set_attention_config(int cfg);
int hcp_debug_set_wgrad_tile(int wx);
#ifdef __cplusplus
}
#endif
#endif
```

Measured before the change: 211.2 images/sec.

## Fold nearest-upsample into 3x3 conv as four 2x2 sub-pixel convolutions

Upsample-then-conv3x3 layers in the UNet decoder (frozen weights, no LoRA) now use a folded kernel. The 3x3 weights are pre-summed into four 2x2 phase filters, so the convolution runs on the low-resolution input instead of the upsampled one. The data gradient uses a matching 4x4 stride-2 fold, which removes both the separate upsample backward pass and the 9-tap work at high resolution. This cuts the conv FLOPs for these layers (16 taps at low resolution versus 36 at high resolution). In exchange it adds weight-fold pack kernels, new GEMM modes with extra masking logic, and bf16 rounding of the summed weights.

Measured after the change: 216.6 images/sec (median of 6 runs). 1.03x the previous value.

```diff
diff --git a/hcp_diffusion_amd/_lib.py b/hcp_diffusion_amd/_lib.py
--- a/hcp_diffusion_amd/_lib.py
+++ b/hcp_diffusion_amd/_lib.py
@@ -17,6 +17,8 @@
     "hcp_gemm_geglu_bwd_bf16": (I, [P, I, P, I, P, P, P, I, P, P, I, I, I, P, c_size_t, P]),
     "hcp_gemm_workspace_bytes": (c_size_t, [I, I]),
     "hcp_conv3x3_bf16": (I, [P, I, P, I, I, I, I, I, I, I, I, I, I, P, I, P, I, P, P, I, P, I, I, P, P, P, c_size_t, P]),
+    "hcp_conv_fold_pack": (I, [P, P, P, I, I, P]),
+    "hcp_conv3x3_up_fold_bf16": (I, [P, I, I, I, I, I, I, P, P, P, P, c_size_t, P]),
     "hcp_attention_fwd": (I, [P, P, P, P, P, I, I, I, I, I, L, I, L, I, L, I, L, I, F, P, L, I, P]),
     "hcp_attention_bwd": (I, [P, P, P, P, P, P, P, P, P, P, I, I, I, I, I, L, I, L, I, L, I, L, I, F, P, L, I, P, c_size_t, P]),
     "hcp_groupnorm_workspace_bytes": (c_size_t, [I, I, I, I]),
@@ -83,6 +85,7 @@
     "hcp_debug_set_gemm_loaders": (I, [I]),
     "hcp_debug_set_gemm_epilogue": (I, [I]),
     "hcp_debug_set_conv_patch": (I, [I]),
+    "hcp_debug_set_conv_fold": (I, [I]),
     "hcp_debug_set_gn_target": (I, [I]),
     "hcp_debug_set_gemm_ablation": (I, [I]),
     "hcp_debug_set_attention_config": (I, [I]),
@@ -95,7 +98,7 @@
 TOOLS_LIB_PATH = Path(__file__).resolve().parent / "libhcp_mi355x_tools.so"
 
 
-ABI_VERSION = 4
+ABI_VERSION = 5
 
 
 class HcpError(RuntimeError):
diff --git a/hcp_diffusion_amd/csrc/gemm.hip b/hcp_diffusion_amd/csrc/gemm.hip
--- a/hcp_diffusion_amd/csrc/gemm.hip
+++ b/hcp_diffusion_amd/csrc/gemm.hip
@@ -795,6 +795,7 @@
 HCP_TUNABLE(int, g_use_v2, 1);
 
 HCP_TUNABLE(int, g_conv_patch, 1);
+HCP_TUNABLE(int, g_conv_fold, 1);
 HCP_TUNABLE(int, g_epi_tile, -1);
 HCP_TUNABLE(int, g_force_loaders, -1);
 
@@ -1041,9 +1042,42 @@
     return launch_lora_by_id(id, p, stream);
 }
 
+const TunedEntry kTunedFold[] = {
+    {-1, 0, 0, 0, 0, 0, 0, 0, 0, 0},
+#include "gemm_tuned_fold.inc"
+};
+int dispatch_fold(GemmParams& p, int mode, float* ws, size_t ws_bytes, hipStream_t stream) {
+    int id = (long)hcp_cdiv(p.M, 128) * hcp_cdiv(p.N, 160) >= 256 ? 3 : 4, nsplit = 1, ring = 4;
+    const int nk1 = p.K / BK;
+    if (mode == 5) {
+        const long tiles = (long)hcp_cdiv(p.M, kCfgs[id].bm) * hcp_cdiv(p.N, 160);
+        while (nsplit < 16 && tiles * nsplit < 256 && nk1 / (nsplit * 2) >= 16) nsplit *= 2;
+    }
+    for (const TunedEntry& e : kTunedFold)
+        if (e.mode == mode && e.M == p.M && e.N == p.N && e.K == p.K) { id = e.cfg; nsplit = e.split; ring = e.loaders - 8; break; }
+    if (g_force_cfg >= 0) { id = forced_id(g_force_cfg); nsplit = forced_split(g_force_cfg); }
+    if (g_force_loaders >= 8) ring = g_force_loaders - 8;
+    if (mode == 4 || (size_t)nsplit * p.M * p.N * sizeof(float) > ws_bytes) nsplit = 1;
+    HCP_REQUIRE(id >= 0 && id < kNumCfgs && kCfgs[id].bn == 160 && (kCfgs[id].bm == 128 || kCfgs[id].bm == 64), "hcp_conv3x3_up_fold_bf16: tile id %d has no folded kernel", id);
+    p.loaders = 8 + ring;
+    p.nsplit = nsplit;
+    p.kt_per_split = hcp_cdiv(nk1, nsplit);
+    p.nsplit = hcp_cdiv(nk1, p.kt_per_split);
+    p.slabs = ws;
+    p.tiles_m = hcp_cdiv(p.M, kCfgs[id].bm);
+    p.dbg = 0;
+    p.epi_tile = 0;
+    HCP_REQUIRE(buffer_loops_take(p), "hcp_conv3x3_up_fold_bf16: operands too large for 32-bit offsets");
+    const int r = gemm_pp_launch(p, kCfgs[id].bm, 160, mode, false, ring, stream);
+    HCP_REQUIRE(r != -2, "hcp_conv3x3_up_fold_bf16: no kernel for tile id %d", id);
+    if (r != 0 || p.nsplit <= 1) return r;
+    return launch_splitk_reduce(p, stream);
+}
+
 }
 
 #if defined(HCP_TOOLS)
+HCP_API int hcp_debug_set_conv_fold(int on) { g_conv_fold = on; return 0; }
 HCP_API int hcp_debug_gemm_table_stats(long* hits, long* misses) {
     if (hits) *hits = g_table_hits;
     if (misses) *misses = g_table_misses;
@@ -1110,6 +1144,28 @@
     return fast ? dispatch_gemm<2, true>(p, ws, wb, stream) : dispatch_gemm<2, false>(p, ws, wb, stream);
 }
 
+HCP_API int hcp_conv3x3_up_fold_bf16(const void* X, int Bn, int Hs, int Ws, int Cin, int Cout, int mode, const void* Wfold, void* D,
+                                     const float* bias, void* workspace, size_t workspace_bytes, hipStream_t stream) {
+    HCP_REQUIRE(X && Wfold && D, "hcp_conv3x3_up_fold_bf16: null operand");
+    HCP_REQUIRE(mode == 0 || (mode == 1 && !bias), "hcp_conv3x3_up_fold_bf16: mode is 0 (forward) or 1 (data gradient, no bias)");
+    HCP_REQUIRE(Bn > 0 && Hs > 0 && Ws > 0 && Cin > 0 && Cout > 0 && Cin % 64 == 0 && Cout % 160 == 0,
+                "hcp_conv3x3_up_fold_bf16: needs Cin %% 64 == 0 and Cout %% 160 == 0 (Cin %d, Cout %d)", Cin, Cout);
+    HCP_REQUIRE(Hs <= 512 && Ws <= 512 && Bn < 2048 && (long)Bn * Hs * Ws * 4 * (Cin > Cout ? Cin : Cout) * 2 < (1L << 31),
+                "hcp_conv3x3_up_fold_bf16: tensors too large for 32-bit offsets");
+    if (!g_conv_fold) return 1;
+    GemmParams p = {};
+    p.cv.C1 = mode == 0 ? Cin : Cout; p.cv.X1 = (const hcp_bf16*)X;
+    p.cv.Ho = Hs; p.cv.Wo = Ws; p.cv.stride = 1; p.cv.pad = 1;
+    p.cv.Hs = mode == 0 ? Hs : 2 * Hs; p.cv.Ws = mode == 0 ? Ws : 2 * Ws;
+    p.M = Bn * Hs * Ws;
+    if (mode == 0) { p.N = 4 * Cout; p.K = 4 * Cin; p.ldd = 2 * Cout; p.cv.fold_c = Cout; }
+    else { p.N = Cin; p.K = 16 * ((Cout + BK - 1) / BK * BK); p.ldd = Cin; }
+    p.B = (const hcp_bf16*)Wfold; p.ldb = p.K;
+    p.D = D; p.bias = bias; p.alpha = 1.0f; p.rows_per_group = Hs * Ws;
+    if (int e = check_common(p)) return e;
+    return dispatch_fold(p, mode == 0 ? 4 : 5, (float*)workspace, workspace ? workspace_bytes : 0, stream);
+}
+
 HCP_API int hcp_gemm_geglu_bwd_bf16(const void* A, int lda, const void* B, int ldb, const void* L, const void* E, void* Tout, int ldt,
                                     const void* HG, void* DHG, int M, int F, int K, void* workspace, size_t workspace_bytes,
                                     hipStream_t stream) {
diff --git a/hcp_diffusion_amd/csrc/gemm_params.h b/hcp_diffusion_amd/csrc/gemm_params.h
--- a/hcp_diffusion_amd/csrc/gemm_params.h
+++ b/hcp_diffusion_amd/csrc/gemm_params.h
@@ -11,6 +11,7 @@
     int stride;
     int up;
     int pad;
+    int fold_c;
 };
 
 struct GemmParams {
diff --git a/hcp_diffusion_amd/csrc/gemm_pp.hip b/hcp_diffusion_amd/csrc/gemm_pp.hip
--- a/hcp_diffusion_amd/csrc/gemm_pp.hip
+++ b/hcp_diffusion_amd/csrc/gemm_pp.hip
@@ -45,11 +45,16 @@
 #if defined(HCP_TOOLS)
         if (p.dbg & 0x2000) hcp_setprio<3>();
 #endif
-        const int Ctot = p.cv.C1 + p.cv.C2;
+        const int Ctot = MODE == 5 ? (p.cv.C1 + BK - 1) / BK * BK : p.cv.C1 + p.cv.C2;
         unsigned va[A_IT], vb[B_IT];
-        unsigned a_msk[(A_IT + 2) / 3];
-#pragma unroll
-        for (int i = 0; i < (A_IT + 2) / 3; ++i) a_msk[i] = 0;
+        constexpr int TB = MODE == 5 ? 16 : 9;
+        constexpr int RPW = 32 / TB;
+        constexpr int NMW = (A_IT + RPW - 1) / RPW;
+        unsigned a_msk[NMW];
+        const int fold_q = MODE == 4 ? n0 / p.cv.fold_c : 0;
+        const int fold_py = fold_q >> 1, fold_px = fold_q & 1;
+#pragma unroll
+        for (int i = 0; i < NMW; ++i) a_msk[i] = 0;
         const unsigned a_chunk = (unsigned)(((kc ^ ((lrow >> 1) & 7)) << 3) * 2);
 #pragma unroll
         for (int i = 0; i < B_IT; ++i) {
@@ -67,24 +72,38 @@
                     const int hw = p.cv.Ho * p.cv.Wo;
                     const int b = m / hw; const int rem = m - b * hw;
                     const int py = rem / p.cv.Wo, px = rem - py * p.cv.Wo;
-                    const int s = MODE == 1 ? p.cv.stride : 1;
+                    const int s = MODE == 1 ? p.cv.stride : (MODE == 5 ? 2 : 1);
                     va[i] = (unsigned)((b * p.cv.Hs + py * s) * p.cv.Ws + px * s);
                     unsigned msk = 0;
-#pragma unroll
-                    for (int ky = 0; ky < 3; ++ky)
-#pragma unroll
-                        for (int kx = 0; kx < 3; ++kx) {
-                            const int sy = MODE == 1 ? py * s + ky - p.cv.pad : py + 1 - ky;
-                            const int sx = MODE == 1 ? px * s + kx - p.cv.pad : px + 1 - kx;
-                            if (sy >= 0 && sy < p.cv.Hs && sx >= 0 && sx < p.cv.Ws) msk |= 1u << (ky * 3 + kx);
+                    if (MODE == 4) {
+#pragma unroll
+                        for (int t = 0; t < 4; ++t) {
+                            const int sy = py + (t >> 1) - 1 + fold_py, sx = px + (t & 1) - 1 + fold_px;
+                            if (sy >= 0 && sy < p.cv.Hs && sx >= 0 && sx < p.cv.Ws) msk |= 1u << t;
                         }
-                    a_msk[i / 3] |= msk << (9 * (i % 3));
+                    } else if (MODE == 5) {
+#pragma unroll
+                        for (int t = 0; t < 16; ++t) {
+                            const int sy = 2 * py + (t >> 2) - 1, sx = 2 * px + (t & 3) - 1;
+                            if (sy >= 0 && sy < p.cv.Hs && sx >= 0 && sx < p.cv.Ws) msk |= 1u << t;
+                        }
+                    } else {
+#pragma unroll
+                        for (int ky = 0; ky < 3; ++ky)
+#pragma unroll
+                            for (int kx = 0; kx < 3; ++kx) {
+                                const int sy = MODE == 1 ? py * s + ky - p.cv.pad : py + 1 - ky;
+                                const int sx = MODE == 1 ? px * s + kx - p.cv.pad : px + 1 - kx;
+                                if (sy >= 0 && sy < p.cv.Hs && sx >= 0 && sx < p.cv.Ws) msk |= 1u << (ky * 3 + kx);
+                            }
+                    }
+                    a_msk[i / RPW] |= msk << (TB * (i % RPW));
                 }
             }
         }
         int tap = 0, cb = 0;
         if (MODE != 0) { const int k0 = kt_begin * BK; tap = k0 / Ctot; cb = k0 - tap * Ctot; }
-        unsigned vo1[MODE != 0 ? A_IT : 1], vo2[MODE != 0 ? A_IT : 1], a_nmsk[(A_IT + 2) / 3];
+        unsigned vo1[MODE != 0 ? A_IT : 1], vo2[MODE != 0 ? A_IT : 1], a_nmsk[NMW];
         if (MODE != 0) {
 #pragma unroll
             for (int i = 0; i < A_IT; ++i) {
@@ -93,8 +112,9 @@
                 vo2[i] = live ? va[i] * (unsigned)(2 * p.cv.C2) + a_chunk : HCP_BUF_OOB;
             }
 #pragma unroll
-            for (int i = 0; i < (A_IT + 2) / 3; ++i) a_nmsk[i] = ~a_msk[i];
-        }
+            for (int i = 0; i < NMW; ++i) a_nmsk[i] = ~a_msk[i];
+        }
+        const unsigned tail_oob = (MODE == 5 && ((kc ^ ((lrow >> 1) & 7)) << 3) >= (p.cv.C1 & (BK - 1))) ? HCP_BUF_OOB : 0u;
         const hcp_bf16* Ab = p.A + (size_t)kt_begin * BK;
         const hcp_bf16* Bb = p.B + (size_t)kt_begin * BK;
         const hcp_bf16* Lb = LORA ? p.L + (size_t)kt_begin * BK : nullptr;
@@ -124,20 +144,27 @@
                             if (qa + i >= q0 && qa + i < q1) hcp_buf_glds16(ra, va[i], la + (wave * 8 + RPP * i) * BK);
                     } else {
                         const int ky = tap / 3, kx = tap - ky * 3;
-                        const int doff = MODE == 1 ? (ky - p.cv.pad) * p.cv.Ws + (kx - p.cv.pad) : (1 - ky) * p.cv.Ws + (1 - kx);
+                        const int doff = MODE == 4 ? ((tap >> 1) - 1 + fold_py) * p.cv.Ws + ((tap & 1) - 1 + fold_px)
+                                       : MODE == 5 ? ((tap >> 2) - 1) * p.cv.Ws + ((tap & 3) - 1)
+                                       : MODE == 1 ? (ky - p.cv.pad) * p.cv.Ws + (kx - p.cv.pad) : (1 - ky) * p.cv.Ws + (1 - kx);
                         const bool first = cb < p.cv.C1;
                         const hcp_bf16* base = first ? p.cv.X1 + (long)doff * p.cv.C1 + cb : p.cv.X2 + (long)doff * p.cv.C2 + (cb - p.cv.C1);
                         const hcp_rsrc ra = hcp_make_rsrc(base);
-                        if (first) {
+                        if (MODE == 5 && cb + BK > p.cv.C1) {
 #pragma unroll
                             for (int i = 0; i < A_IT; ++i)
                                 if (qa + i >= q0 && qa + i < q1)
-                                    hcp_buf_glds16(ra, vo1[i] | (((a_nmsk[i / 3] >> (9 * (i % 3) + tap)) & 1u) << 31), la + (wave * 8 + RPP * i) * BK);
-                        } else {
+                                    hcp_buf_glds16(ra, vo1[i] | tail_oob | (((a_nmsk[i / RPW] >> (TB * (i % RPW) + tap)) & 1u) << 31), la + (wave * 8 + RPP * i) * BK);
+                        } else if (first) {
 #pragma unroll
                             for (int i = 0; i < A_IT; ++i)
                                 if (qa + i >= q0 && qa + i < q1)
-                                    hcp_buf_glds16(ra, vo2[i] | (((a_nmsk[i / 3] >> (9 * (i % 3) + tap)) & 1u) << 31), la + (wave * 8 + RPP * i) * BK);
+                                    hcp_buf_glds16(ra, vo1[i] | (((a_nmsk[i / RPW] >> (TB * (i % RPW) + tap)) & 1u) << 31), la + (wave * 8 + RPP * i) * BK);
+                        } else {
+#pragma unroll
+                            for (int i = 0; i < A_IT; ++i)
+                                if (qa + i >= q0 && qa + i < q1)
+                                    hcp_buf_glds16(ra, vo2[i] | (((a_nmsk[i / RPW] >> (TB * (i % RPW) + tap)) & 1u) << 31), la + (wave * 8 + RPP * i) * BK);
                         }
                     }
                 }
@@ -267,10 +294,11 @@
     constexpr bool EARLY = !(LORA && TM * TN >= 20);
     hcp_f32x4 bias_v[TNF];
     hcp_bf16x4 res_v[TMF][TNF];
+    const int nc0 = MODE == 4 ? n0 % p.cv.fold_c : n0;
     auto load_bias = [&]() {
-        const hcp_rsrc rbias = hcp_make_rsrc_n(p.bias, p.bias ? (unsigned)p.N * 4u : 0u);
-#pragma unroll
-        for (int j = 0; j < TNF; ++j) bias_v[j] = hcp_buf_load16f(rbias, (unsigned)geglu_col(p, BN, n0 + fcol0 + j * 16 + 4 * fg) * 4u);
+        const hcp_rsrc rbias = hcp_make_rsrc_n(p.bias, p.bias ? (unsigned)(MODE == 4 ? p.cv.fold_c : p.N) * 4u : 0u);
+#pragma unroll
+        for (int j = 0; j < TNF; ++j) bias_v[j] = hcp_buf_load16f(rbias, (unsigned)geglu_col(p, BN, nc0 + fcol0 + j * 16 + 4 * fg) * 4u);
     };
     auto load_residual = [&]() {
         const hcp_rsrc rres = hcp_make_rsrc_n(p.residual, p.residual ? (unsigned)(((size_t)(p.M - 1) * p.ldr + p.N) * 2) : 0u);
@@ -424,6 +452,27 @@
         }
     }
 
+    if constexpr (MODE == 4) {
+        const int q = n0 / p.cv.fold_c;
+        const size_t qoff = (size_t)((q >> 1) * 2 * p.cv.Ws + (q & 1)) * p.cv.fold_c;
+#pragma unroll
+        for (int i = 0; i < TMF; ++i) {
+            const int m = m0 + frow0 + i * 16 + fr;
+            if (m >= p.M) continue;
+            hcp_bf16* const drow = (hcp_bf16*)p.D + (size_t)(2 * m - m % p.cv.Ws) * p.ldd + qoff;
+#pragma unroll
+            for (int j = 0; j < TNF; ++j) {
+                const int n = n0 + fcol0 + j * 16 + 4 * fg;
+                if (j >= nfin || n >= p.N) continue;
+                const hcp_f32x4 v = acc[i][j] * p.alpha + bias_v[j];
+                hcp_bf16x4 o;
+#pragma unroll
+                for (int e = 0; e < 4; ++e) o[e] = (short)hcp_f2bf(v[e]);
+                *(hcp_bf16x4*)(drow + (nc0 + fcol0 + j * 16 + 4 * fg)) = o;
+            }
+        }
+        return;
+    }
     if (p.nsplit > 1) {
 #pragma unroll
         for (int i = 0; i < TMF; ++i) {
@@ -553,6 +602,11 @@
     if (lora) return launch_pp<BM, BN, 0, true>(p, ring, stream);
     if (mode == 0) return launch_pp<BM, BN, 0, false>(p, ring, stream);
     if (mode == 1) return launch_pp<BM, BN, 1, false>(p, ring, stream);
+    if constexpr (BN == 160) {
+        if (mode == 4) return launch_pp<BM, BN, 4, false>(p, ring, stream);
+        if (mode == 5) return launch_pp<BM, BN, 5, false>(p, ring, stream);
+    }
+    if (mode != 2) return -2;
     return launch_pp<BM, BN, 2, false>(p, ring, stream);
 }
 
diff --git a/hcp_diffusion_amd/csrc/gemm_tuned_fold.inc b/hcp_diffusion_amd/csrc/gemm_tuned_fold.inc
--- /dev/null
+++ b/hcp_diffusion_amd/csrc/gemm_tuned_fold.inc
@@ -0,0 +1 @@
+
diff --git a/hcp_diffusion_amd/csrc/pack.hip b/hcp_diffusion_amd/csrc/pack.hip
--- a/hcp_diffusion_amd/csrc/pack.hip
+++ b/hcp_diffusion_amd/csrc/pack.hip
@@ -49,6 +49,49 @@
     }
 }
 
+HCP_DEVICE float fold_sum(const float* w, int klo_y, int khi_y, int klo_x, int khi_x, int cin) {
+    float sacc = 0.f;
+    bool first = true;
+    for (int ky = klo_y; ky <= khi_y; ++ky)
+        for (int kx = klo_x; kx <= khi_x; ++kx) {
+            const float v = w[(size_t)(ky * 3 + kx) * cin];
+            sacc = first ? v : sacc + v;
+            first = false;
+        }
+    return sacc;
+}
+HCP_KERNEL(256) conv_fold_pack_kernel(const float* W, hcp_bf16* Wf, hcp_bf16* Wdf, int Cout, int Cin) {
+    const long n = (long)16 * Cout * Cin;
+    const int Cp = (Cout + 63) / 64 * 64;
+    const long nd = (long)16 * Cp * Cin;
+    for (long idx = (long)blockIdx.x * 256 + threadIdx.x; idx < n + nd; idx += (long)gridDim.x * 256) {
+        if (idx < n) {
+            const int ci = (int)(idx % Cin); long r = idx / Cin;
+            const int tx = (int)(r & 1), ty = (int)((r >> 1) & 1); r >>= 2;
+            const int co = (int)(r % Cout), q = (int)(r / Cout), py = q >> 1, px = q & 1;
+            const int ylo = py == 0 ? (ty == 0 ? 0 : 1) : (ty == 0 ? 0 : 2), yhi = py == 0 ? (ty == 0 ? 0 : 2) : (ty == 0 ? 1 : 2);
+            const int xlo = px == 0 ? (tx == 0 ? 0 : 1) : (tx == 0 ? 0 : 2), xhi = px == 0 ? (tx == 0 ? 0 : 2) : (tx == 0 ? 1 : 2);
+            Wf[idx] = hcp_f2bf(fold_sum(W + (size_t)co * 9 * Cin + ci, ylo, yhi, xlo, xhi, Cin));
+        } else {
+            const long j = idx - n;
+            const int co = (int)(j % Cp); long r = j / Cp;
+            if (co >= Cout) { Wdf[j] = 0; continue; }
+            const int ax = (int)(r & 3), ay = (int)((r >> 2) & 3); const int ci = (int)(r >> 4);
+            const int ylo = ay == 0 ? 2 : (ay == 1 ? 1 : 0), yhi = ay == 0 ? 2 : (ay == 1 ? 2 : (ay == 2 ? 1 : 0));
+            const int xlo = ax == 0 ? 2 : (ax == 1 ? 1 : 0), xhi = ax == 0 ? 2 : (ax == 1 ? 2 : (ax == 2 ? 1 : 0));
+            Wdf[j] = hcp_f2bf(fold_sum(W + (size_t)co * 9 * Cin + ci, ylo, yhi, xlo, xhi, Cin));
+        }
+    }
+}
+
+}
+
+HCP_API int hcp_conv_fold_pack(const float* W, void* Wf, void* Wdf, int Cout, int Cin, hipStream_t stream) {
+    HCP_REQUIRE(W && Wf && Wdf && Cout > 0 && Cin > 0, "hcp_conv_fold_pack: bad arguments");
+    const long n = (long)16 * Cin * (Cout + (Cout + 63) / 64 * 64);
+    int g = (int)((n + 255) / 256); if (g > 8192) g = 8192;
+    HCP_LAUNCH(conv_fold_pack_kernel, dim3(g), dim3(256), 0, stream, W, (hcp_bf16*)Wf, (hcp_bf16*)Wdf, Cout, Cin);
+    HCP_LAUNCH_CHECK("conv_fold_pack");
 }
 
 HCP_API int hcp_pack_piece_bytes(void) { return (int)sizeof(PackPiece); }
diff --git a/hcp_diffusion_amd/csrc/runtime.hip b/hcp_diffusion_amd/csrc/runtime.hip
--- a/hcp_diffusion_amd/csrc/runtime.hip
+++ b/hcp_diffusion_amd/csrc/runtime.hip
@@ -14,7 +14,7 @@
 
 HCP_API int hcp_is_emulated(void) { return HCP_IS_EMULATED; }
 
-HCP_API int hcp_abi_version(void) { return 4; }
+HCP_API int hcp_abi_version(void) { return 5; }
 
 namespace {
 HCP_KERNEL(256) atomics_selfcheck_kernel(float* line, float* bucket, int nb, int stride) {
diff --git a/hcp_diffusion_amd/kernels.py b/hcp_diffusion_amd/kernels.py
--- a/hcp_diffusion_amd/kernels.py
+++ b/hcp_diffusion_amd/kernels.py
@@ -194,7 +194,7 @@
 
 
 def conv3x3(x1, wp, cout, *, x2=None, stride=1, upsample=False, mode=0, out_hw=None, bias=None, rowbias=None,
-            residual=None, out_f32=False, a2=None, b2=None, pad=1, out=None):
+            residual=None, out_f32=False, a2=None, b2=None, pad=1, out=None, fold=None):
     assert x1.dtype == BF16 and x1.dim() == 4 and x1.is_contiguous()
     B, Hs, Ws, C1 = x1.shape
     C2 = 0
@@ -215,6 +215,12 @@
                 Cout=cout, stride=stride, upsample=1 if upsample else 0, pad=pad, Ho=Ho, Wo=Wo, ldd=cout, ldr=cout if residual is not None else 0,
                 bias=bias is not None, rowbias=rowbias is not None, rows_per_group=Ho * Wo if rowbias is not None else 0,
                 residual=residual is not None, out_f32=bool(out_f32))
+    if fold is not None:
+        assert C2 == 0 and stride == 1 and pad == 1 and rowbias is None and residual is None and a2 is None and not out_f32 and out is None
+        assert (mode == 0 and upsample) or (mode == 1 and bias is None and Hs % 2 == 0 and Ws % 2 == 0 and (Ho, Wo) == (Hs, Ws))
+        y = _conv3x3_fold(x1, fold, cout, mode, bias)
+        if y is not None:
+            return y
     if out is None:
         out = torch.empty((B, Ho, Wo, cout), dtype=torch.float32 if out_f32 else BF16, device=x1.device)
     assert out.dtype == (torch.float32 if out_f32 else BF16) and out.is_contiguous() and tuple(out.shape) == (B, Ho, Wo, cout)
@@ -232,7 +238,42 @@
                                 cout, _p(out), cout, _p(bias), _p(rowbias), rowbias.stride(0) if rowbias is not None else 0,
                                 _p(residual), cout, 1 if out_f32 else 0, _p(a2), _p(b2), _p(ws), ws.numel(), _stream(x1)),
          "hcp_conv3x3_bf16")
-    return out
+    return upsample2x_bwd(out) if (fold is not None and mode == 1) else out
+
+
+def conv_fold_pack(w, wf, wdf):
+    cout, _, _, cin = w.shape
+    assert w.dtype == torch.float32 and w.is_contiguous() and tuple(w.shape) == (cout, 3, 3, cin)
+    assert wf.dtype == BF16 and wf.is_contiguous() and tuple(wf.shape) == (2, 2, cout, 2, 2, cin)
+    assert wdf.dtype == BF16 and wdf.is_contiguous() and tuple(wdf.shape) == (cin, 4, 4, fold_cout_pad(cout))
+    _chk(lib().hcp_conv_fold_pack(_p(w), _p(wf), _p(wdf), cout, cin, _stream(w)), "hcp_conv_fold_pack")
+
+
+def fold_cout_pad(cout):
+    return (cout + 63) // 64 * 64
+
+
+def conv_fold_eligible(cin, cout):
+    return cin % 64 == 0 and cout % 160 == 0
+
+
+def _conv3x3_fold(x, wfold, cout, mode, bias):
+    B, Hx, Wx, Cx = x.shape
+    if mode == 0:
+        Hs, Ws, cin, co = Hx, Wx, Cx, cout
+        assert wfold.dtype == BF16 and wfold.is_contiguous() and tuple(wfold.shape) == (2, 2, co, 2, 2, cin)
+        y = torch.empty((B, 2 * Hs, 2 * Ws, co), dtype=BF16, device=x.device)
+    else:
+        Hs, Ws, cin, co = Hx // 2, Wx // 2, cout, Cx
+        assert wfold.dtype == BF16 and wfold.is_contiguous() and tuple(wfold.shape) == (cin, 4, 4, fold_cout_pad(co))
+        y = torch.empty((B, Hs, Ws, cin), dtype=BF16, device=x.device)
+    assert conv_fold_eligible(cin, co)
+    ws = _workspace(x)
+    rc = lib().hcp_conv3x3_up_fold_bf16(_p(x), B, Hs, Ws, cin, co, mode, _p(wfold), _p(y), _p(bias), _p(ws), ws.numel(), _stream(x))
+    if rc == 1:
+        return None
+    _chk(rc, "hcp_conv3x3_up_fold_bf16")
+    return y
 
 
 def wgrad_linear(dy, x, dw):
diff --git a/hcp_diffusion_amd/layers.py b/hcp_diffusion_amd/layers.py
--- a/hcp_diffusion_amd/layers.py
+++ b/hcp_diffusion_amd/layers.py
@@ -95,6 +95,19 @@
             self._pk = pk
         return self._pk
 
+    def folded(self):
+        pk = self.packed()
+        if getattr(pk, "fold_key", None) != pk.key:
+            w = self.weight.detach().permute(0, 2, 3, 1)
+            if w.dtype != torch.float32 or not w.is_contiguous():
+                w = w.float().contiguous()
+            if getattr(pk, "wf", None) is None:
+                pk.wf = torch.empty((2, 2, pk.cout, 2, 2, pk.cin), dtype=BF16, device=w.device)
+                pk.wdf = torch.empty((pk.cin, 4, 4, ops.K.fold_cout_pad(pk.cout)), dtype=BF16, device=w.device)
+            ops.K.conv_fold_pack(w, pk.wf, pk.wdf)
+            pk.fold_key = pk.key
+        return pk.wf, pk.wdf
+
     def forward(self, x, residual=None, x2=None, rowbias=None, upsample=False):
         if self.kernel_size == (1, 1):
             assert x2 is None and rowbias is None and not upsample
diff --git a/hcp_diffusion_amd/ops.py b/hcp_diffusion_amd/ops.py
--- a/hcp_diffusion_amd/ops.py
+++ b/hcp_diffusion_amd/ops.py
@@ -321,7 +321,11 @@
             y = K.conv3x3(x1, pk.w, pk.cout, x2=x2, stride=stride, upsample=upsample, bias=pk.bias, rowbias=rowbias, residual=residual,
                           a2=T, b2=lp.bu)
         else:
-            y = K.conv3x3(x1, pk.w, pk.cout, x2=x2, stride=stride, upsample=upsample, bias=pk.bias, rowbias=rowbias, residual=residual)
+            fold = (upsample and stride == 1 and x2 is None and rowbias is None and residual is None and not host.weight.requires_grad
+                    and K.conv_fold_eligible(pk.cin, pk.cout))
+            ctx.fold = fold
+            y = K.conv3x3(x1, pk.w, pk.cout, x2=x2, stride=stride, upsample=upsample, bias=pk.bias, rowbias=rowbias, residual=residual,
+                          fold=host.folded()[0] if fold else None)
         ctx.host, ctx.stride, ctx.upsample, ctx.lora = host, stride, upsample, lora
         ctx.in_shape = x1.shape
         ctx.c2 = x2.shape[-1] if x2 is not None else 0
@@ -355,7 +359,9 @@
                 dl1 = K.conv3x3(U, lp.wdl[:C1], C1, mode=1, stride=ctx.stride, out_hw=hw)
             if ctx.c2 and ctx.needs_input_grad[1]:
                 dl2 = K.conv3x3(U, lp.wdl[C1:], ctx.c2, mode=1, stride=ctx.stride, out_hw=hw)
-        if ctx.needs_input_grad[0]:
+        if ctx.needs_input_grad[0] and getattr(ctx, "fold", False):
+            dx1 = K.conv3x3(dy, pk.wd[:C1], C1, mode=1, stride=ctx.stride, out_hw=hw, fold=ctx.host.folded()[1])
+        elif ctx.needs_input_grad[0]:
             dx1 = K.conv3x3(dy, pk.wd[:C1], C1, mode=1, stride=ctx.stride, out_hw=hw, residual=dl1)
             if ctx.upsample:
                 dx1 = K.upsample2x_bwd(dx1)
diff --git a/include/hcp_mi355x.h b/include/hcp_mi355x.h
--- a/include/hcp_mi355x.h
+++ b/include/hcp_mi355x.h
@@ -10,7 +10,7 @@
 
 const char* hcp_last_error(void);
 int hcp_is_emulated(void);
-#define HCP_ABI_VERSION 4
+#define HCP_ABI_VERSION 5
 int hcp_abi_version(void);
 int hcp_selfcheck_atomics(float* line, float* bucket, int nb, int stride, int workgroups, hcpStream_t stream);
 
@@ -29,6 +29,9 @@
                      int stride, int upsample, int pad, const void* Wp, int Cout, void* D, int ldd, const float* bias,
                      const float* rowbias, int rowbias_ld, const void* residual, int ldr, int out_f32, const void* A2,
                      const void* B2, void* workspace, size_t workspace_bytes, hcpStream_t stream);
+int hcp_conv_fold_pack(const float* W, void* Wf, void* Wdf, int Cout, int Cin, hcpStream_t stream);
+int hcp_conv3x3_up_fold_bf16(const void* X, int B, int Hs, int Ws, int Cin, int Cout, int mode, const void* Wfold, void* D,
+                             const float* bias, void* workspace, size_t workspace_bytes, hcpStream_t stream);
 
 int hcp_attention_fwd(const void* Q, const void* K, const void* V, void* O, float* lse, int B, int H, int Nq, int Nk, int D,
                       long q_bs, int q_rs, long k_bs, int k_rs, long v_bs, int v_rs, long o_bs, int o_rs, float scale,
diff --git a/include/hcp_mi355x_tools.h b/include/hcp_mi355x_tools.h
--- a/include/hcp_mi355x_tools.h
+++ b/include/hcp_mi355x_tools.h
@@ -10,6 +10,7 @@
 int hcp_debug_set_gn_target(int workgroups);
 int hcp_debug_set_gemm_epilogue(int mode);
 int hcp_debug_set_conv_patch(int on);
+int hcp_debug_set_conv_fold(int on);
 int hcp_debug_set_gemm_loaders(int mode);
 int hcp_debug_set_gemm_glds(int on);
 int hcp_debug_set_attention_config(int cfg);
```
